# aosokin/os2d

Hardware: AMD Instinct MI355X
Metric: query-image-pairs/s (1280-px input, ResNet50, N-class) (higher is better)
Workload: dtype fftx3 (as fft; the per-bin complex GEMM on the fp16 MFMA with spectra split into fp16 hi+lo, 3 MFMAs per product, fp32 accumulate)

## Files before the change

### include/os2d_hip.h

```cpp
#ifndef OS2D_HIP_H
#define OS2D_HIP_H

#include <stddef.h>

#ifdef __cplusplus
extern "C" {
#endif

#define OS2D_ABI_VERSION 9

#define OS2D_PRECISION_F32 0
#define OS2D_PRECISION_F16X3 1
#define OS2D_PRECISION_F16X2 2

#define OS2D_PRECISION_FFT 3

#define OS2D_PRECISION_FFT32 5

#define OS2D_PRECISION_FFTX3 4

int os2d_abi_version(void);

const char* os2d_last_error(void);

size_t os2d_packed_conv_floats(int layer );
size_t os2d_packed_bias_floats(int layer );
int os2d_pack_conv(int layer, int P, const float* w, const float* b, const float* bn_weight, const float* bn_bias,
                   const float* bn_running_mean, const float* bn_running_var, float bn_eps, float* packed_w,
                   float* packed_b, void* stream);

int os2d_class_prepare(const float* src, int C, int h, int w, int normalize, float* q15, float* qp, void* stream);
size_t os2d_class_prepare_workspace_floats(int B, int C);
int os2d_class_prepare_batch(const float* const* srcs, const int* sizes, int B, int C, int normalize, float* q15,
                             float* qp, float* workspace, void* stream);

int os2d_head_workspace_bytes(int A, int B, int C, int H, int W, int P, size_t* bytes);
int os2d_head_workspace_bytes_ex(int A, int B, int C, int H, int W, int P, int precision, size_t* bytes);
int os2d_head_forward(const float* fm, const float* qp, const float* w1, const float* b1, const float* w2,
                      const float* b2, const float* w3, const float* b3, int A, int B, int C, int H, int W, int P,
                      int inverse, int stride, int rec_field, float* loc, float* cls, float* corners,
                      void* workspace, size_t workspace_bytes, void* stream);

size_t os2d_packed_conv_bytes(int layer, int precision);
int os2d_rnorm_exp(void);
int os2d_pack_conv_f16x3(int layer , int P, const float* w, const float* b, const float* bn_weight,
                         const float* bn_bias, const float* bn_running_mean, const float* bn_running_var, float bn_eps,
                         const int* weight_exp, const int* in_exp, const int* out_exp, void* packed_w, float* packed_b,
                         void* stream);

size_t os2d_class_split_bytes(int B, int C);
int os2d_class_split(const float* qp, void* qs, int B, int C, void* stream);

#define OS2D_STATUS_F16_RANGE 1
int os2d_head_forward_ex(const float* fm, const float* qp, const void* w1, const float* b1, const void* w2,
                         const float* b2, const void* w3, const float* b3, int A, int B, int C, int H, int W, int P,
                         int inverse, int stride, int rec_field, float* loc, float* cls, float* corners,
                         void* workspace, size_t workspace_bytes, void* stream, int precision, const void* qs,
                         void** stage_events, int* chunk_classes, int* status, const float* wspec, const float* twQ,
                         const float* twP);
int os2d_head_forward_ex2(const float* fm, const float* qp, const void* w1, const float* b1, const void* w2,
                          const float* b2, const void* w3, const float* b3, int A, int B, int C, int H, int W, int P,
                          int inverse, int stride, int rec_field, float* loc, float* cls, float* corners,
                          void* workspace, size_t workspace_bytes, void* stream, int precision, const void* qs,
                          void** stage_events, int* chunk_classes, int* status, const float* wspec, const float* twQ,
                          const float* twP, const void* wspec2);
void os2d_debug_set_dump(void* stream, int slot, void* dst, size_t bytes);
int os2d_prof_event_create(void** ev);
int os2d_prof_event_destroy(void* ev);
int os2d_prof_event_elapsed_ms(void* begin, void* end, float* ms);

int os2d_fm_sumsq(const float* fm, float* sumsq, int A, int C, int H, int W, void* stream);
size_t os2d_plane_floats(int H, int W);
int os2d_corr(const float* fm, const float* qp, const float* sumsq, float* corr, float* rnorm, int A, int B, int C,
              int H, int W, void* stream);
size_t os2d_corr_f16x3_workspace_bytes(int A, int C, int H, int W);
int os2d_corr_f16x3(const float* fm, const void* qs, float* corr, void* rshb, int A, int B, int C, int H, int W,
                    void* workspace, size_t workspace_bytes, void* stream);
size_t os2d_corr_f16x3_packed_workspace_bytes(int A, int B, int C, int H, int W);
int os2d_corr_f16x3_packed(const float* fm, const void* qs, float* corr, float* inv_norm, int A, int B, int C, int H, int W,
                           int form, void* workspace, size_t workspace_bytes, void* stream);
int os2d_corr_normalize(const float* corr, float* rnorm, int NB, int H, int W, void* stream);
int os2d_transform_conv(int layer, const float* in, const float* packed_w, const float* packed_b, float* out,
                        int NB, int P, int H, int W, void* stream);
size_t os2d_shb_bytes(int channels, int H, int W);
int os2d_corr_normalize_f16x3(const float* corr, void* rshb, int NB, int H, int W, void* stream);
int os2d_transform_conv_f16x3(int layer, const void* in, const void* packed_w, const float* packed_b, void* out, int NB,
                              int P, int H, int W, int terms, int* status, void* stream);
int os2d_alignment_grids(const float* params, int NB, int H, int W, int P, int inverse, float* theta, float* grids,
                         void* stream);
int os2d_sample_decode(const float* corr, const float* params, int NB, int H, int W, int P, int inverse, int stride,
                       int rec_field, float* loc, float* cls, float* corners, void* stream);

int os2d_decode_boxes(const float* loc, int NB, int H, int W, int stride, int rec_field, float img_w, float img_h,
                      float* boxes, void* stream);

int os2d_nms_workspace_bytes(int NC, int N, size_t* bytes);
int os2d_nms(const float* boxes, const int* counts, int NC, int N, float iou_threshold, unsigned char* keep,
             int* num_keep, void* workspace, size_t workspace_bytes, void* stream);

int os2d_detect_level_supported(int H, int W);
int os2d_detect_level(const float* loc, const float* cls, int B, int H, int W, int stride, int rec_field, float img_w,
                      float img_h, float scale_x, float scale_y, float score_threshold, float iou_threshold,
                      float* out_boxes, float* out_scores, int* out_index, int* out_count, void* stream);

#define OS2D_BOX_OP_SCALE 1
#define OS2D_BOX_OP_HFLIP 2
#define OS2D_BOX_OP_VFLIP 3
#define OS2D_BOX_OP_SHIFT 4
#define OS2D_BOX_MAX_OPS 6
#define OS2D_BOX_MAX_DEFAULT_OPS 12
int os2d_detect_level_ops(const float* loc, const float* cls, int B, int H, int W, int stride, int rec_field, float img_w,
                          float img_h, int op_count, const int* op_kinds, const float* op_args, float score_threshold,
                          float iou_threshold, float* out_boxes, float* out_scores, int* out_index, int* out_count,
                          void* stream);

size_t os2d_spectral_weight_bytes(int C, int Cout, int nbins);
int os2d_fft_sizes(int H, int W, int* P, int* Q, int* nbins);
int os2d_fft_tiles(int H, int W, int* tiles_y, int* tiles_x, int* tile_h, int* tile_w);
int os2d_fft_forward(const float* corr, const float* inv_norm, float* X, const float* twQ, const float* twP, int NB, int C,
                     int H, int W, void* stream);
int os2d_fft_inverse(const float* Y, const float* packed_b, void* out, const float* twQ, const float* twP, int NB, int Cout,
                     int H, int W, int* status, void* stream);
#define OS2D_SPECTRA_ROWS 0
#define OS2D_SPECTRA_QUADS 1
int os2d_fft_inverse_ex(const float* Y, const float* packed_b, void* out, const float* twQ, const float* twP, int NB, int Cout,
                        int H, int W, int* status, int layout, void* stream);
int os2d_spectral_gemm(const float* wspec, const float* X, float* Y, int NB, int C, int Cout, int nbins, void* stream);
size_t os2d_spectral_weight16_bytes(int C, int nbins);
int os2d_spectral_weights_build(const double* wfold, const double* twP64, const double* twQ64, int C, int Cout, int P, int Q,
                                int nbins, int split, void* out, void* workspace, void* stream);
float os2d_spectral_xscale(int H, int W);
int os2d_spectral_gemm_f16(const void* w16, const float* X, float* Y, int NB, int C, int Cout, int nbins, float xscale,
                           void* stream);

int os2d_dft_sizes(int H, int W, int* P, int* Q, int* nbins, int* tiles);
int os2d_dft_channel_stride(int C);
size_t os2d_dft_matrices_bytes(int P, int Q);
int os2d_dft_matrices_build(const double* twP64, const double* twQ64, int P, int Q, void* out, void* stream);
int os2d_dft_forward(const float* corr, const float* inv_norm, float* X, const void* matrices, int NB, int C, int H, int W,
                     void* stream);
int os2d_dft_inverse(const float* Y, const float* packed_b, void* out, const void* matrices, int NB, int Cout, int H, int W,
                     int* status, void* stream);
int os2d_dft_inverse_planes(const float* Y, const float* packed_b, float* out, const void* matrices, int NB, int Cout, int H, int W,
                            int* status, void* stream);
int os2d_spectral_weights_build_dft(const double* wfold, const double* twP64, const double* twQ64, int C, int Cout, int P, int Q,
                                    int nbins, void* out, void* workspace, void* stream);
int os2d_spectral_gemm_f16_quads(const void* w16, const float* X, float* Y, int NB, int C, int Cout, int nbins, float xscale,
                                 void* stream);
float os2d_dft_xscale(int H, int W);

#define OS2D_PYRAMID_MAX_LEVELS 16
int os2d_detect_pyramid_supported(int L, int N, int nms_max_batch);
int os2d_detect_pyramid_workspace_bytes(int B, int N, int passes, size_t* bytes);
int os2d_detect_pyramid(const float* const* loc, const float* const* cls, const float* const* corners, int B, int L,
                        const int* hw, int stride, int rec_field, const float* img_wh, const float* scale_xy,
                        float score_threshold, float iou_threshold, int nms_max_batch, int passes, float* out_boxes,
                        float* out_scores, int* out_index, float* out_default, float* out_corners, int* out_count,
                        int* unfinished, void* workspace, size_t workspace_bytes, void* stream);
int os2d_detect_pyramid_merged(const float* const* loc, const float* const* cls, const float* const* corners, int B, int L,
                               const int* hw, int stride, int rec_field, const float* img_wh, const float* scale_xy,
                               float score_threshold, float iou_threshold, int nms_max_batch, int passes, int G, int V,
                               const int* slot_rows, float* out_boxes, float* out_scores, int* out_index, float* out_default,
                               float* out_corners, int* out_count, int* unfinished, void* workspace, size_t workspace_bytes,
                               void* stream);

int os2d_detect_pyramid_ops(const float* const* loc, const float* const* cls, const float* const* corners, int B, int L,
                            const int* hw, int stride, int rec_field, const float* img_wh, const int* op_counts,
                            const int* op_kinds, const float* op_args, const int* default_op_counts,
                            const int* default_op_kinds, const float* default_op_args, float score_threshold, float iou_threshold,
                            int nms_max_batch, int passes, int G, int V, const int* slot_rows, float* out_boxes,
                            float* out_scores, int* out_index, float* out_default, float* out_corners, int* out_count,
                            int* unfinished, void* workspace, size_t workspace_bytes, void* stream);

#ifdef __cplusplus
}
#endif
#endif
```

### os2d_amd/_lib.py

```python
import ctypes

from . import build
from ._native import NativeLibrary, Os2dLibraryError

ABI_VERSION = 9

_c_float_p = ctypes.c_void_p
_vp = ctypes.c_void_p
_i = ctypes.c_int
_f = ctypes.c_float
_sz = ctypes.c_size_t

SIGNATURES = {
    "os2d_abi_version": (_i, []),
    "os2d_last_error": (ctypes.c_char_p, []),
    "os2d_packed_conv_floats": (_sz, [_i]),
    "os2d_packed_bias_floats": (_sz, [_i]),
    "os2d_pack_conv": (_i, [_i, _i, _vp, _vp, _vp, _vp, _vp, _vp, _f, _vp, _vp, _vp]),
    "os2d_class_prepare": (_i, [_vp, _i, _i, _i, _i, _vp, _vp, _vp]),
    "os2d_head_workspace_bytes": (_i, [_i, _i, _i, _i, _i, _i, ctypes.POINTER(_sz)]),
    "os2d_head_forward": (_i, [_vp] * 8 + [_i] * 9 + [_vp, _vp, _vp, _vp, _sz, _vp]),
    "os2d_packed_conv_bytes": (_sz, [_i, _i]),
    "os2d_pack_conv_f16x3": (_i, [_i, _i, _vp, _vp, _vp, _vp, _vp, _vp, _f, _vp, _vp, _vp, _vp, _vp, _vp]),
    "os2d_rnorm_exp": (_i, []),
    "os2d_class_prepare_batch": (_i, [_vp, _vp, _i, _i, _i, _vp, _vp, _vp, _vp]),
    "os2d_class_prepare_workspace_floats": (_sz, [_i, _i]),
    "os2d_shb_bytes": (_sz, [_i, _i, _i]),
    "os2d_corr_normalize_f16x3": (_i, [_vp, _vp, _i, _i, _i, _vp]),
    "os2d_transform_conv_f16x3": (_i, [_i, _vp, _vp, _vp, _vp, _i, _i, _i, _i, _i, _vp, _vp]),
    "os2d_alignment_grids": (_i, [_vp, _i, _i, _i, _i, _i, _vp, _vp, _vp]),
    "os2d_spectral_weight_bytes": (_sz, [_i, _i, _i]),
    "os2d_spectral_gemm": (_i, [_vp, _vp, _vp, _i, _i, _i, _i, _vp]),
    "os2d_spectral_weight16_bytes": (_sz, [_i, _i]),
    "os2d_spectral_xscale": (_f, [_i, _i]),
    "os2d_spectral_weights_build": (_i, [_vp, _vp, _vp, _i, _i, _i, _i, _i, _i, _vp, _vp, _vp]),
    "os2d_spectral_gemm_f16": (_i, [_vp, _vp, _vp, _i, _i, _i, _i, _f, _vp]),
    "os2d_debug_set_dump": (None, [_vp, _i, _vp, _sz]),
    "os2d_fft_sizes": (_i, [_i, _i, ctypes.POINTER(_i), ctypes.POINTER(_i), ctypes.POINTER(_i)]),
    "os2d_fft_tiles": (_i, [_i, _i, ctypes.POINTER(_i), ctypes.POINTER(_i), ctypes.POINTER(_i), ctypes.POINTER(_i)]),
    "os2d_fft_forward": (_i, [_vp, _vp, _vp, _vp, _vp, _i, _i, _i, _i, _vp]),
    "os2d_fft_inverse": (_i, [_vp, _vp, _vp, _vp, _vp, _i, _i, _i, _i, _vp, _vp]),
    "os2d_fft_inverse_ex": (_i, [_vp, _vp, _vp, _vp, _vp, _i, _i, _i, _i, _vp, _i, _vp]),
    "os2d_dft_sizes": (_i, [_i, _i, ctypes.POINTER(_i), ctypes.POINTER(_i), ctypes.POINTER(_i), ctypes.POINTER(_i)]),
    "os2d_dft_channel_stride": (_i, [_i]),
    "os2d_dft_matrices_bytes": (_sz, [_i, _i]),
    "os2d_dft_matrices_build": (_i, [_vp, _vp, _i, _i, _vp, _vp]),
    "os2d_dft_forward": (_i, [_vp, _vp, _vp, _vp, _i, _i, _i, _i, _vp]),
    "os2d_dft_inverse": (_i, [_vp, _vp, _vp, _vp, _i, _i, _i, _i, _vp, _vp]),
    "os2d_spectral_weights_build_dft": (_i, [_vp, _vp, _vp, _i, _i, _i, _i, _i, _vp, _vp, _vp]),
    "os2d_spectral_gemm_f16_quads": (_i, [_vp, _vp, _vp, _i, _i, _i, _i, _f, _vp]),
    "os2d_dft_xscale": (_f, [_i, _i]),
    "os2d_class_split": (_i, [_vp, _vp, _i, _i, _vp]),
    "os2d_class_split_bytes": (_sz, [_i, _i]),
    "os2d_head_forward_ex": (_i, [_vp] * 8 + [_i] * 9 + [_vp, _vp, _vp, _vp, _sz, _vp, _i, _vp,
                                  ctypes.POINTER(_vp), ctypes.POINTER(_i), _vp, _vp, _vp, _vp]),
    "os2d_head_forward_ex2": (_i, [_vp] * 8 + [_i] * 9 + [_vp, _vp, _vp, _vp, _sz, _vp, _i, _vp,
                                   ctypes.POINTER(_vp), ctypes.POINTER(_i), _vp, _vp, _vp, _vp, _vp]),
    "os2d_dft_inverse_planes": (_i, [_vp, _vp, _vp, _vp, _i, _i, _i, _i, _vp, _vp]),
    "os2d_head_workspace_bytes_ex": (_i, [_i, _i, _i, _i, _i, _i, _i, ctypes.POINTER(_sz)]),
    "os2d_prof_event_create": (_i, [ctypes.POINTER(_vp)]),
    "os2d_prof_event_destroy": (_i, [_vp]),
    "os2d_prof_event_elapsed_ms": (_i, [_vp, _vp, ctypes.POINTER(_f)]),
    "os2d_fm_sumsq": (_i, [_vp, _vp, _i, _i, _i, _i, _vp]),
    "os2d_plane_floats": (_sz, [_i, _i]),
    "os2d_corr": (_i, [_vp, _vp, _vp, _vp, _vp, _i, _i, _i, _i, _i, _vp]),
    "os2d_corr_normalize": (_i, [_vp, _vp, _i, _i, _i, _vp]),
    "os2d_corr_f16x3_workspace_bytes": (_sz, [_i, _i, _i, _i]),
    "os2d_corr_f16x3": (_i, [_vp, _vp, _vp, _vp, _i, _i, _i, _i, _i, _vp, _sz, _vp]),
    "os2d_corr_f16x3_packed_workspace_bytes": (_sz, [_i, _i, _i, _i, _i]),
    "os2d_corr_f16x3_packed": (_i, [_vp, _vp, _vp, _vp, _i, _i, _i, _i, _i, _i, _vp, _sz, _vp]),
    "os2d_transform_conv": (_i, [_i, _vp, _vp, _vp, _vp, _i, _i, _i, _i, _vp]),
    "os2d_sample_decode": (_i, [_vp, _vp, _i, _i, _i, _i, _i, _i, _i, _vp, _vp, _vp, _vp]),
    "os2d_decode_boxes": (_i, [_vp, _i, _i, _i, _i, _i, _f, _f, _vp, _vp]),
    "os2d_nms_workspace_bytes": (_i, [_i, _i, ctypes.POINTER(_sz)]),
    "os2d_nms": (_i, [_vp, _vp, _i, _i, _f, _vp, _vp, _vp, _sz, _vp]),
    "os2d_detect_level_supported": (_i, [_i, _i]),
    "os2d_detect_level": (_i, [_vp, _vp] + [_i] * 5 + [_f] * 6 + [_vp] * 5),
    "os2d_detect_level_ops": (_i, [_vp, _vp] + [_i] * 5 + [_f, _f, _i, _vp, _vp, _f, _f] + [_vp] * 5),
    "os2d_detect_pyramid_supported": (_i, [_i, _i, _i]),
    "os2d_detect_pyramid_workspace_bytes": (_i, [_i, _i, _i, ctypes.POINTER(_sz)]),
    "os2d_detect_pyramid": (_i, [_vp, _vp, _vp, _i, _i, _vp, _i, _i, _vp, _vp, _f, _f, _i, _i, _vp, _vp, _vp, _vp, _vp, _vp,
                                 _vp, _vp, _sz, _vp]),
    "os2d_detect_pyramid_merged": (_i, [_vp, _vp, _vp, _i, _i, _vp, _i, _i, _vp, _vp, _f, _f, _i, _i, _i, _i, _vp, _vp, _vp, _vp,
                                        _vp, _vp, _vp, _vp, _vp, _sz, _vp]),
    "os2d_detect_pyramid_ops": (_i, [_vp, _vp, _vp, _i, _i, _vp, _i, _i, _vp, _vp, _vp, _vp, _vp, _vp, _vp, _f, _f, _i, _i, _i, _i, _vp, _vp, _vp,
                                     _vp, _vp, _vp, _vp, _vp, _vp, _sz, _vp]),
}


LIBRARY = NativeLibrary(build.HIP, SIGNATURES, ABI_VERSION, "os2d_abi_version", "os2d_last_error", "the OS2D head")
lib_path, load, check = LIBRARY.lib_path, LIBRARY.load, LIBRARY.check


def ptr(t):
    if t is None:
        return None
    import torch
    if not (isinstance(t, torch.Tensor) and t.is_cuda and t.dtype in (torch.float32, torch.float64, torch.uint8, torch.int32, torch.int64)
            and t.is_contiguous()):
        raise ValueError("expected a contiguous device tensor, got {}".format(
            (type(t).__name__, getattr(t, "device", None), getattr(t, "dtype", None))))
    return ctypes.c_void_p(t.data_ptr())


def host_ptr(t):
    if t is None:
        return None
    if not t.is_pinned():
        raise ValueError("expected a pinned host tensor")
    return ctypes.c_void_p(t.data_ptr())


def current_stream(device):
    import torch
    return ctypes.c_void_p(torch.cuda.current_stream(device).cuda_stream)
```

### os2d_amd/csrc/abi.hip

```cpp
#include <stdio.h>

#include "../../include/os2d_hip.h"
#include "os2d_common.h"
#include "detect_common.h"
#include <atomic>
#include <mutex>
#include <random>
#include <vector>

namespace {
struct ConvShape {
  int cout, cin, ks, mt;
};
bool conv_shape(int layer, int P, ConvShape* s) {
  switch (layer) {
    case 1: *s = {128, OS2D_K, 7, 128}; return true;
    case 2: *s = {64, 128, 5, 64}; return true;
    case 3: *s = {P, 64, 5, 32}; return true;
    default: return false;
  }
}
size_t align_up(size_t x, size_t a) { return (x + a - 1) / a * a; }

int os2d_conv1_steps_padded() { return 25; }

struct Carve {
  size_t flags, sumsq, fs, corr, rpad, h1, h2, params, invn, sumfx, xspec, yspec, total;
};
Carve carve(int A, int Bc, int C, int H, int W, int P, int fft_bins = 0, int fft_tiles = 1, int xspec_channels = OS2D_K) {
  const size_t HW = (size_t)H * W, PL = os2d_plane(H, W), NB = (size_t)A * Bc;
  Carve c;
  size_t off = 0;
  auto take = [&](size_t floats) {
    size_t o = off;
    off = align_up(off + floats * sizeof(float), 256);
    return o;
  };
  c.flags = take((size_t)A + 1);
  c.sumsq = take((size_t)A * HW);
  c.fs = take((size_t)A * os2d_corr_groups(C) * 2 * HW * 4);
  c.corr = take(NB * OS2D_K * HW);
  c.rpad = take(fft_bins > 0 ? 0 : NB * (OS2D_G * 2 * 4) * PL);
  c.h1 = take(NB * 128 * PL);
  c.h2 = take(NB * 64 * PL);
  c.params = take(NB * P * HW);
  c.invn = c.sumfx = c.xspec = c.yspec = 0;
  if (fft_bins > 0) {
    c.invn = take(NB * HW);
    c.sumfx = take(NB * HW * 2);
    c.xspec = take(NB * fft_tiles * xspec_channels * (size_t)fft_bins * 2);
    c.yspec = take(NB * fft_tiles * 128 * (size_t)fft_bins * 2);
  }
  c.total = off;
  return c;
}

#ifdef OS2D_DIAG_DUMP
struct DumpEntry {
  void* stream;
  int slot;
  void* dst;
  size_t bytes;
};
std::vector<DumpEntry> g_dumps;
std::mutex g_dumps_mutex;
bool dumps_active() {
  std::lock_guard<std::mutex> lock(g_dumps_mutex);
  return !g_dumps.empty();
}
void dump_slot(void* stream, int slot, const void* src, size_t bytes) {
  std::lock_guard<std::mutex> lock(g_dumps_mutex);
  for (const DumpEntry& e : g_dumps)
    if (e.stream == stream && e.slot == slot && e.dst)
      (void)hipMemcpyAsync(e.dst, src, bytes < e.bytes ? bytes : e.bytes, hipMemcpyDeviceToDevice, static_cast<hipStream_t>(stream));
}
#else
inline bool dumps_active() { return false; }
inline void dump_slot(void*, int, const void*, size_t) {}
#endif

bool head_args_ok(int A, int B, int C, int H, int W, int P) {
  if (A < 1 || B < 1 || C < 1 || H < 1 || W < 1 || (P != 6 && P != 4)) {
    os2d_set_error("bad head shape A=%d B=%d C=%d H=%d W=%d P=%d (need A,B,C,H,W>=1, P in {6,4})", A, B, C, H,
                   W, P);
    return false;
  }
  if (W > OS2D_MAX_W) {
    os2d_set_error("feature map width %d > %d: beyond what the transform planner of the 7x7 layer tiles (images wider than %d px "
                   "at stride 16 are not supported)", W, OS2D_MAX_W, OS2D_MAX_W * 16);
    return false;
  }
  if (H > OS2D_MAX_H) {
    os2d_set_error("feature map height %d > %d: beyond what the transform planner of the 7x7 layer tiles (images taller than %d px "
                   "at stride 16 are not supported)", H, OS2D_MAX_H, OS2D_MAX_H * 16);
    return false;
  }
  return true;
}
int next_epoch() {
  static std::atomic<unsigned> counter{[] {
    std::random_device rd;
    return (unsigned)rd() | 0x100u;
  }()};
  unsigned e;
  do e = counter.fetch_add(1u, std::memory_order_relaxed) + 1u;
  while (e < 2u);
  return (int)e;
}
bool is_freq(int precision) {
  return precision == OS2D_PRECISION_FFT || precision == OS2D_PRECISION_FFTX3 || precision == OS2D_PRECISION_FFT32;
}
int freq_plan(int precision, int H, int W, int* P, int* Q, int* bins, int* tiles) {
  return precision == OS2D_PRECISION_FFTX3 ? os2d_dft_plan(H, W, P, Q, bins, tiles) : os2d_fft_plan(H, W, P, Q, bins, tiles);
}
bool direct7_width_ok(int W) {
  if (W > OS2D_MAX_W_DIRECT7) {
    os2d_set_error("feature map width %d > %d: the direct 7x7 kernels keep 3 halo rows of their input in LDS - wider maps need a "
                   "frequency-domain precision (fftx3 / fft / fft32), which tiles any width up to %d", W, OS2D_MAX_W_DIRECT7, OS2D_MAX_W);
    return false;
  }
  return true;
}
}

void os2d_debug_set_dump(void* stream, int slot, void* dst, size_t bytes) {
#ifdef OS2D_DIAG_DUMP
  std::lock_guard<std::mutex> lock(g_dumps_mutex);
  for (size_t i = 0; i < g_dumps.size(); ++i)
    if (g_dumps[i].stream == stream && g_dumps[i].slot == slot) {
      if (dst) {
        g_dumps[i].dst = dst;
        g_dumps[i].bytes = bytes;
      } else {
        g_dumps.erase(g_dumps.begin() + i);
      }
      return;
    }
  if (dst) g_dumps.push_back(DumpEntry{stream, slot, dst, bytes});
#else
  (void)stream, (void)slot, (void)dst, (void)bytes;
  os2d_set_error("os2d_debug_set_dump: this library was built without -DOS2D_DIAG_DUMP (diagnostic builds only)");
#endif
}

extern "C" {

int os2d_abi_version(void) { return OS2D_ABI_VERSION; }
const char* os2d_last_error(void) { return os2d_error_text; }

size_t os2d_packed_conv_floats(int layer) {
  ConvShape s;
  if (!conv_shape(layer, 6, &s)) return 0;
  return (size_t)((s.cin + 1) / 2) * s.ks * s.ks * 2 * s.mt;
}
size_t os2d_packed_bias_floats(int layer) {
  ConvShape s;
  if (!conv_shape(layer, 6, &s)) return 0;
  return (size_t)3 * s.mt;
}

int os2d_pack_conv(int layer, int P, const float* w, const float* b, const float* bn_weight, const float* bn_bias,
                   const float* bn_running_mean, const float* bn_running_var, float bn_eps, float* packed_w,
                   float* packed_b, void* stream) {
  ConvShape s;
  if (!conv_shape(layer, P, &s) || (layer == 3 && P != 6 && P != 4)) {
    os2d_set_error("os2d_pack_conv: bad layer %d / P %d", layer, P);
    return -1;
  }
  if (!w || !b || !packed_w || !packed_b) {
    os2d_set_error("os2d_pack_conv: null pointer");
    return -1;
  }
  const bool has_bn = bn_weight || bn_bias || bn_running_mean || bn_running_var;
  if (has_bn && !(bn_weight && bn_bias && bn_running_mean && bn_running_var)) {
    os2d_set_error("os2d_pack_conv: BatchNorm needs all four of weight/bias/running_mean/running_var");
    return -1;
  }
  return os2d_launch_pack_conv(w, b, bn_weight, bn_bias, bn_running_mean, bn_running_var, bn_eps, s.cout, s.cin, s.ks,
                               s.mt, packed_w, packed_b, os2d_stream(stream));
}

int os2d_class_prepare(const float* src, int C, int h, int w, int normalize, float* q15, float* qp, void* stream) {
  if (!src || !q15 || !qp || C < 1 || h < 1 || w < 1) {
    os2d_set_error("os2d_class_prepare: bad arguments (C=%d h=%d w=%d)", C, h, w);
    return -1;
  }
  return os2d_launch_class_prepare(src, C, h, w, normalize, q15, qp, os2d_stream(stream));
}

size_t os2d_class_prepare_workspace_floats(int B, int C) {
  if (B < 1 || C < 1) return 0;
  return (size_t)os2d_class_prepare_partial_floats(B, C);
}

int os2d_class_prepare_batch(const float* const* srcs, const int* sizes, int B, int C, int normalize, float* q15,
                             float* qp, float* workspace, void* stream) {
  if (!srcs || !sizes || !q15 || !qp || !workspace || B < 1 || C < 1 || B > 65535) {
    os2d_set_error("os2d_class_prepare_batch: bad arguments (B=%d C=%d; at most 65535 classes per call)", B, C);
    return -1;
  }
  return os2d_launch_class_prepare_batch(srcs, sizes, B, C, normalize, q15, qp, workspace, os2d_stream(stream));
}

size_t os2d_plane_floats(int H, int W) { return (size_t)os2d_plane(H, W); }

size_t os2d_shb_bytes(int channels, int H, int W) {
  if (channels < 1 || H < 1 || W < 1) return 0;
  return (size_t)((channels + 7) / 8) * 2 * os2d_plane(H, W) * 16;
}

int os2d_head_workspace_bytes(int A, int B, int C, int H, int W, int P, size_t* bytes) {
  if (!bytes) {
    os2d_set_error("os2d_head_workspace_bytes: null output");
    return -1;
  }
  if (!head_args_ok(A, B, C, H, W, P)) return -1;
  *bytes = carve(A, B, C, H, W, P).total;
  return 0;
}

int os2d_head_workspace_bytes_ex(int A, int B, int C, int H, int W, int P, int precision, size_t* bytes) {
  if (!bytes) {
    os2d_set_error("os2d_head_workspace_bytes_ex: null output");
    return -1;
  }
  if (!head_args_ok(A, B, C, H, W, P)) return -1;
  int bins = 0, tiles[6] = {1, 1, 0, 0, 0, 0};
  if (is_freq(precision) && !freq_plan(precision, H, W, nullptr, nullptr, &bins, tiles)) {
    os2d_set_error("os2d_head_workspace_bytes_ex: no transform plan for a %dx%d map", H, W);
    return -3;
  }
  *bytes = carve(A, B, C, H, W, P, bins, tiles[0] * tiles[1], precision == OS2D_PRECISION_FFTX3 ? OS2D_XSPEC_CPAD : OS2D_K).total;
  return 0;
}

int os2d_fm_sumsq(const float* fm, float* sumsq, int A, int C, int H, int W, void* stream) {
  if (!fm || !sumsq || A < 1 || C < 1 || H < 1 || W < 1) {
    os2d_set_error("os2d_fm_sumsq: bad arguments");
    return -1;
  }
  return os2d_launch_fm_sumsq(fm, sumsq, A, C, H * W, os2d_stream(stream));
}

int os2d_corr(const float* fm, const float* qp, const float* sumsq, float* corr, float* rnorm, int A, int B, int C,
              int H, int W, void* stream) {
  if (!fm || !qp || !sumsq || !corr || !rnorm) {
    os2d_set_error("os2d_corr: null pointer");
    return -1;
  }
  if (!head_args_ok(A, B, C, H, W, 6)) return -1;
  int rc = os2d_launch_border_zero(rnorm, A * B * OS2D_KP, H, W, os2d_stream(stream));
  if (rc) return rc;
  return os2d_launch_corr(fm, qp, sumsq, corr, rnorm, nullptr, A, B, C, H, W, 0, os2d_stream(stream));
}

size_t os2d_corr_f16x3_workspace_bytes(int A, int C, int H, int W) {
  if (A < 1 || C < 1 || H < 1 || W < 1) return 0;
  return align_up((size_t)A * H * W * sizeof(float), 256) + (size_t)A * os2d_corr_groups(C) * 2 * H * W * 16;
}

int os2d_corr_f16x3(const float* fm, const void* qs, float* corr, void* rshb, int A, int B, int C, int H, int W,
                    void* workspace, size_t workspace_bytes, void* stream) {
  if (!fm || !qs || !corr || !rshb || !workspace) {
    os2d_set_error("os2d_corr_f16x3: null pointer");
    return -1;
  }
  if (!head_args_ok(A, B, C, H, W, 6)) return -1;
  if (workspace_bytes < os2d_corr_f16x3_workspace_bytes(A, C, H, W) || (reinterpret_cast<uintptr_t>(workspace) & 255)) {
    os2d_set_error("os2d_corr_f16x3: workspace too small or not 256-byte aligned");
    return -2;
  }
  float* sumsq = static_cast<float*>(workspace);
  void* fs = static_cast<char*>(workspace) + align_up((size_t)A * H * W * sizeof(float), 256);
  int rc = os2d_launch_fm_sumsq(fm, sumsq, A, C, H * W, os2d_stream(stream));
  if (!rc) rc = os2d_launch_split_fm(fm, sumsq, fs, A, C, H * W, nullptr, 0, Os2dRangeFlag{nullptr, 0}, os2d_stream(stream));
  if (!rc) rc = os2d_launch_border_zero_shb(rshb, A * B, H, W, os2d_stream(stream));
  if (!rc) rc = os2d_launch_corr_f16x3(fs, qs, corr, rshb, nullptr, nullptr, 0, A, B, C, H, W, os2d_stream(stream));
  return rc;
}

size_t os2d_corr_f16x3_packed_workspace_bytes(int A, int B, int C, int H, int W) {
  if (A < 1 || B < 1 || C < 1 || H < 1 || W < 1) return 0;
  return align_up(os2d_corr_f16x3_workspace_bytes(A, C, H, W), 256) + (size_t)A * B * H * W * sizeof(unsigned long long);
}

int os2d_corr_f16x3_packed(const float* fm, const void* qs, float* corr, float* inv_norm, int A, int B, int C, int H, int W,
                           int form, void* workspace, size_t workspace_bytes, void* stream) {
  if (!fm || !qs || !corr || !inv_norm || !workspace) {
    os2d_set_error("os2d_corr_f16x3_packed: null pointer");
    return -1;
  }
  if (!head_args_ok(A, B, C, H, W, 6)) return -1;
  if (workspace_bytes < os2d_corr_f16x3_packed_workspace_bytes(A, B, C, H, W) || (reinterpret_cast<uintptr_t>(workspace) & 255)) {
    os2d_set_error("os2d_corr_f16x3_packed: workspace too small or not 256-byte aligned");
    return -2;
  }
  float* sumsq = static_cast<float*>(workspace);
  void* fs = static_cast<char*>(workspace) + align_up((size_t)A * H * W * sizeof(float), 256);
  void* sumfx = static_cast<char*>(workspace) + align_up(os2d_corr_f16x3_workspace_bytes(A, C, H, W), 256);
  int rc = os2d_launch_fm_sumsq(fm, sumsq, A, C, H * W, os2d_stream(stream));
  if (!rc) rc = os2d_launch_split_fm(fm, sumsq, fs, A, C, H * W, nullptr, 0, Os2dRangeFlag{nullptr, 0}, os2d_stream(stream));
  if (form < -1 || form > 7 || (form >= 0 && (form & 3) > 1)) {
    os2d_set_error("os2d_corr_f16x3_packed: form %d (0 padded | 1 packed | -1 the head's choice; + 4: no half tiles at the tail)", form);
    return -1;
  }
  const bool packed = form < 0 ? os2d_corr_f16x3_use_packed(A, B, H, W) != 0 : (form & 1) != 0;
  if (!rc && packed) rc = os2d_launch_corr_sums_clear(sumfx, A, B, H, W, os2d_stream(stream));
  if (!rc) rc = os2d_launch_corr_f16x3(fs, qs, corr, nullptr, inv_norm, packed ? sumfx : nullptr, (form >= 0 && (form & 4)) ? 2 : 0, A, B, C, H, W, os2d_stream(stream));
  return rc;
}

int os2d_corr_normalize(const float* corr, float* rnorm, int NB, int H, int W, void* stream) {
  if (!corr || !rnorm || NB < 1 || H < 1 || W < 1) {
    os2d_set_error("os2d_corr_normalize: bad arguments");
    return -1;
  }
  return os2d_launch_corr_normalize(corr, rnorm, NB, H, W, os2d_stream(stream));
}

int os2d_transform_conv(int layer, const float* in, const float* packed_w, const float* packed_b, float* out, int NB,
                        int P, int H, int W, void* stream) {
  if (!in || !packed_w || !packed_b || !out || NB < 1 || H < 1 || W < 1 || (layer == 3 && P != 6 && P != 4)) {
    os2d_set_error("os2d_transform_conv: bad arguments (layer=%d NB=%d P=%d)", layer, NB, P);
    return -1;
  }
  return os2d_launch_conv(layer, in, packed_w, packed_b, out, NB, P, H, W, os2d_stream(stream));
}

int os2d_sample_decode(const float* corr, const float* params, int NB, int H, int W, int P, int inverse, int stride,
                       int rec_field, float* loc, float* cls, float* corners, void* stream) {
  if (!corr || !params || !loc || !cls || !corners || NB < 1 || H < 1 || W < 1 || (P != 6 && P != 4)) {
    os2d_set_error("os2d_sample_decode: bad arguments");
    return -1;
  }
  return os2d_launch_sample_decode(corr, params, NB, H, W, P, inverse, stride, rec_field, NB, NB, 0, loc, cls,
                                   corners, nullptr, 0, nullptr, os2d_stream(stream));
}

int os2d_decode_boxes(const float* loc, int NB, int H, int W, int stride, int rec_field, float img_w, float img_h,
                      float* boxes, void* stream) {
  if (!loc || !boxes || NB < 1 || H < 1 || W < 1) {
    os2d_set_error("os2d_decode_boxes: bad arguments");
    return -1;
  }
  return os2d_launch_decode_boxes(loc, NB, H, W, stride, rec_field, img_w, img_h, boxes, os2d_stream(stream));
}

int os2d_detect_level_supported(int H, int W) { return os2d_detect_level_lds_bytes(H, W) != 0 ? 1 : 0; }

int os2d_detect_level(const float* loc, const float* cls, int B, int H, int W, int stride, int rec_field, float img_w,
                      float img_h, float scale_x, float scale_y, float score_threshold, float iou_threshold,
                      float* out_boxes, float* out_scores, int* out_index, int* out_count, void* stream) {
  if (!loc || !cls || !out_boxes || !out_scores || !out_index || !out_count || B < 1 || H < 1 || W < 1 || stride < 1 ||
      rec_field < 1) {
    os2d_set_error("os2d_detect_level: bad arguments");
    return -1;
  }
  return os2d_launch_detect_level(loc, cls, B, H, W, stride, rec_field, img_w, img_h, os2d_box_ops_scale<OS2D_BOX_MAX_OPS>(scale_x, scale_y),
                                  score_threshold, iou_threshold, out_boxes, out_scores, out_index, out_count, os2d_stream(stream));
}

int os2d_detect_level_ops(const float* loc, const float* cls, int B, int H, int W, int stride, int rec_field, float img_w,
                          float img_h, int op_count, const int* op_kinds, const float* op_args, float score_threshold,
                          float iou_threshold, float* out_boxes, float* out_scores, int* out_index, int* out_count,
                          void* stream) {
  if (!loc || !cls || !out_boxes || !out_scores || !out_index || !out_count || B < 1 || H < 1 || W < 1 || stride < 1 ||
      rec_field < 1) {
    os2d_set_error("os2d_detect_level_ops: bad arguments");
    return -1;
  }
  Os2dBoxOps ops;
  if (!os2d_box_ops_from(op_kinds, op_args, op_count, &ops)) {
    os2d_set_error("os2d_detect_level_ops: bad transform chain (at most %d ops of kind 1..4)", OS2D_BOX_MAX_OPS);
    return -1;
  }
  return os2d_launch_detect_level(loc, cls, B, H, W, stride, rec_field, img_w, img_h, ops, score_threshold, iou_threshold,
                                  out_boxes, out_scores, out_index, out_count, os2d_stream(stream));
}

int os2d_nms_workspace_bytes(int NC, int N, size_t* bytes) {
  if (!bytes || NC < 1 || N < 1) {
    os2d_set_error("os2d_nms_workspace_bytes: bad arguments");
    return -1;
  }
  *bytes = (size_t)NC * N * 4 * sizeof(float);
  return 0;
}

int os2d_nms(const float* boxes, const int* counts, int NC, int N, float iou_threshold, unsigned char* keep,
             int* num_keep, void* workspace, size_t workspace_bytes, void* stream) {
  if (!boxes || !counts || !keep || !num_keep || !workspace || NC < 1 || N < 1) {
    os2d_set_error("os2d_nms: bad arguments");
    return -1;
  }
  if ((reinterpret_cast<uintptr_t>(boxes) & 15) || (reinterpret_cast<uintptr_t>(workspace) & 15)) {
    os2d_set_error("os2d_nms: boxes and workspace must be 16-byte aligned");
    return -1;
  }
  if (workspace_bytes < (size_t)NC * N * 4 * sizeof(float)) {
    os2d_set_error("os2d_nms: workspace too small");
    return -2;
  }
  return os2d_launch_nms(boxes, counts, NC, N, iou_threshold, keep, num_keep, workspace, os2d_stream(stream));
}

int os2d_head_forward_ex2(const float* fm, const float* qp, const void* w1, const float* b1, const void* w2,
                          const float* b2, const void* w3, const float* b3, int A, int B, int C, int H, int W, int P,
                          int inverse, int stride, int rec_field, float* loc, float* cls, float* corners,
                          void* workspace, size_t workspace_bytes, void* stream, int precision, const void* qs,
                          void** stage_events, int* chunk_classes, int* status, const float* wspec, const float* twQ,
                          const float* twP, const void* wspec2) {
  if (!fm || !qp || !w1 || !b1 || !w2 || !b2 || !w3 || !b3 || !loc || !cls || !corners || !workspace) {
    os2d_set_error("os2d_head_forward: null pointer");
    return -1;
  }
  if (precision != OS2D_PRECISION_F32 && precision != OS2D_PRECISION_F16X3 && precision != OS2D_PRECISION_F16X2 &&
      precision != OS2D_PRECISION_FFT && precision != OS2D_PRECISION_FFTX3 && precision != OS2D_PRECISION_FFT32) {
    os2d_set_error("os2d_head_forward: unknown precision %d", precision);
    return -1;
  }
  int fft_bins = 0, tiles[6] = {1, 1, 0, 0, 0, 0};
  const bool dft = precision == OS2D_PRECISION_FFTX3;
  if (is_freq(precision)) {
    if (!wspec || !twQ || (!dft && !twP)) {
      os2d_set_error("os2d_head_forward: the frequency-domain modes need the weight spectra and the transform tables "
                     "(fft / fft32: twQ, twP; fftx3: the matrices of os2d_dft_matrices_build as twQ)");
      return -1;
    }
    if (!freq_plan(precision, H, W, nullptr, nullptr, &fft_bins, tiles)) {
      os2d_set_error("os2d_head_forward: no transform plan for a %dx%d map", H, W);
      return -3;
    }
  } else if (!direct7_width_ok(W)) {
    return -1;
  }
  const int fft_T = tiles[0] * tiles[1], xch = dft ? OS2D_XSPEC_CPAD : OS2D_K;
  static const bool conv2_freq_env = [] {
    const char* e = getenv("OS2D_CONV2_FREQ");
    return !(e && e[0] == '0');
  }();
  const bool conv2_freq = dft && wspec2 && conv2_freq_env;
  const bool fp32_ops = precision == OS2D_PRECISION_F32 || precision == OS2D_PRECISION_FFT32;
  if (!fp32_ops && !qs) {
    os2d_set_error("os2d_head_forward: precision f16x3 / f16x2 needs the split class operand (os2d_class_split)");
    return -1;
  }
  if (!head_args_ok(A, B, C, H, W, P)) return -1;
  if (stride < 1 || rec_field < 1) {
    os2d_set_error("os2d_head_forward: bad stride/rec_field %d/%d", stride, rec_field);
    return -1;
  }
  if (reinterpret_cast<uintptr_t>(workspace) & 255) {
    os2d_set_error("os2d_head_forward: workspace must be 256-byte aligned");
    return -1;
  }
  const size_t one = carve(A, 1, C, H, W, P, fft_bins, fft_T, xch).total;
  if (workspace_bytes < one) {
    os2d_set_error("os2d_head_forward: workspace too small (%zu B, need >= %zu B for one class)", workspace_bytes, one);
    return -2;
  }
  int Bc = B;
  while (Bc > 1 && carve(A, Bc, C, H, W, P, fft_bins, fft_T, xch).total > workspace_bytes) {
    const size_t two = carve(A, 2, C, H, W, P, fft_bins, fft_T, xch).total;
    const size_t per = two - one;
    int guess = per ? (int)((workspace_bytes - one) / per) + 1 : 1;
    if (guess >= Bc) guess = Bc - 1;
    if (guess < 1) guess = 1;
    Bc = guess;
  }
  hipStream_t st = os2d_stream(stream);
  char* ws = static_cast<char*>(workspace);
  const Carve c = carve(A, Bc, C, H, W, P, fft_bins, fft_T, xch);
  float* invn = fft_bins ? reinterpret_cast<float*>(ws + c.invn) : nullptr;
  void* sumfx = (fft_bins && !fp32_ops && os2d_corr_f16x3_use_packed(A, Bc, H, W)) ? ws + c.sumfx : nullptr;
  float* xspec = fft_bins ? reinterpret_cast<float*>(ws + c.xspec) : nullptr;
  float* yspec = fft_bins ? reinterpret_cast<float*>(ws + c.yspec) : nullptr;
  float* sumsq = reinterpret_cast<float*>(ws + c.sumsq);
  void* fsplit = ws + c.fs;
  float* corr = reinterpret_cast<float*>(ws + c.corr);
  float* rpad = reinterpret_cast<float*>(ws + c.rpad);
  float* h1 = reinterpret_cast<float*>(ws + c.h1);
  float* h2 = reinterpret_cast<float*>(ws + c.h2);
  float* params = reinterpret_cast<float*>(ws + c.params);
  int* flags = reinterpret_cast<int*>(ws + c.flags);
  const int epoch = next_epoch();
  const Os2dRangeFlag per_image = {fp32_ops ? nullptr : flags, epoch}, whole_call = {fp32_ops ? nullptr : flags + A, epoch};

  if (chunk_classes) *chunk_classes = Bc;
  auto mark = [&](int b0, int idx) {
    if (stage_events && b0 == 0 && stage_events[idx]) (void)hipEventRecord(reinterpret_cast<hipEvent_t>(stage_events[idx]), st);
  };
  int rc = os2d_launch_fm_sumsq(fm, sumsq, A, C, H * W, st);
  if (rc) return rc;
  if (!fp32_ops && (rc = os2d_launch_split_fm(fm, sumsq, fsplit, A, C, H * W, sumfx, sumfx ? (size_t)A * Bc * H * W : 0, per_image, st))) return rc;
  for (int b0 = 0; b0 < B; b0 += Bc) {
    const int bc = (B - b0 < Bc) ? (B - b0) : Bc;
    const int NB = A * bc;
    const bool f16 = !fp32_ops;
    const int terms1 = precision == OS2D_PRECISION_F16X2 ? 2 : 3;
    mark(b0, 0);
    if (f16) {
      if (!fft_bins && (rc = os2d_launch_border_zero_shb(rpad, NB, H, W, st))) return rc;
    } else if (!fft_bins) {
      if ((rc = os2d_launch_border_zero(rpad, NB * OS2D_KP, H, W, st))) return rc;
    }
    if (f16) {
      const char* qsb = static_cast<const char*>(qs) + (size_t)b0 * os2d_corr_groups(C) * 2 * 256 * 16;
      if ((rc = os2d_launch_corr_f16x3(fsplit, qsb, corr, fft_bins ? nullptr : rpad, invn, sumfx, 1, A, bc, C, H, W, st))) return rc;
    } else {
      if ((rc = os2d_launch_corr(fm, qp + (size_t)b0 * C * OS2D_QROWS, sumsq, corr, fft_bins ? nullptr : rpad, invn, A, bc, C, H, W,
                                 0, st)))
        return rc;
    }
    mark(b0, 1);
    mark(b0, 2);
    if (fft_bins) {
      bool inv_borders = false;
      if (f16) {
        static const bool borders_in_inverse = [] {
          const char* e = getenv("OS2D_BORDERS_IN_INVERSE");
          return !(e && e[0] == '0');
        }();
        inv_borders = dft && borders_in_inverse;
        const int planes = (inv_borders || conv2_freq) ? 0 : NB * 16 * 2;
        if ((planes || sumfx) &&
            (rc = os2d_launch_border_zero_shb_planes_norms(h1, planes, H, W, sumfx, invn, (size_t)NB * H * W, st)))
          return rc;
      } else if ((rc = os2d_launch_border_zero(h1, NB * 128, H, W, st))) {
        return rc;
      }
      mark(b0, 10);
      const int layout = precision == OS2D_PRECISION_FFTX3 ? OS2D_SPECTRA_QUADS : OS2D_SPECTRA_ROWS;
      if (dft) {
        const void* mats = twQ;
        if ((rc = os2d_launch_dft_forward(corr, invn, xspec, mats, NB, OS2D_K, xch, H, W, st))) return rc;
        mark(b0, 11);
        if ((rc = os2d_launch_spectral_gemm_f16(wspec, xspec, yspec, NB * fft_T, OS2D_K, 128, fft_bins,
                                                os2d_spectral_xscale_for(tiles[4], tiles[5]), 1, xch, st)))
          return rc;
        mark(b0, 12);
        if ((rc = os2d_launch_dft_inverse(yspec, b1, 128, h1, mats, NB, 128, H, W, whole_call,
                                          conv2_freq ? OS2D_DFT_OUT_PLANES : inv_borders ? OS2D_DFT_OUT_SHB_BORDERS : OS2D_DFT_OUT_SHB, st)))
          return rc;
      } else {
        if ((rc = os2d_launch_fft_forward(corr, invn, xspec, twQ, twP, NB, OS2D_K, H, W, st))) return rc;
        mark(b0, 11);
        if ((rc = os2d_launch_spectral_gemm(wspec, xspec, yspec, NB * fft_T, OS2D_K, 128, fft_bins, st))) return rc;
        mark(b0, 12);
        if ((rc = os2d_launch_fft_inverse(yspec, b1, 128, h1, twQ, twP, NB, 128, H, W, whole_call, layout, f16 ? 0 : 1, st))) return rc;
      }
    } else if (f16) {
      if ((rc = os2d_launch_conv_f16x3(1, rpad, w1, b1, whole_call, h1, NB, P, H, W, terms1, st))) return rc;
    } else {
      if ((rc = os2d_launch_conv(1, rpad, static_cast<const float*>(w1), b1, h1, NB, P, H, W, st))) return rc;
    }
    mark(b0, 3);
    mark(b0, 4);
    if (dumps_active() && b0 == 0) {
      const size_t PLb = os2d_plane(H, W);
      dump_slot(stream, 0, corr, (size_t)NB * OS2D_K * H * W * 4);
      if (fft_bins) {
        dump_slot(stream, 1, invn, (size_t)NB * H * W * 4);
        dump_slot(stream, 2, xspec, (size_t)NB * fft_T * OS2D_K * fft_bins * 8);
        dump_slot(stream, 3, yspec, (size_t)NB * fft_T * 128 * fft_bins * 8);
      }
      dump_slot(stream, 4, h1, (size_t)NB * 128 * (conv2_freq ? (size_t)H * W : PLb) * 4);
    }
    if (conv2_freq) {
      if ((rc = os2d_launch_dft_forward(h1, nullptr, xspec, twQ, NB, 128, 128, H, W, st))) return rc;
      if ((rc = os2d_launch_spectral_gemm_f16(wspec2, xspec, yspec, NB * fft_T, 128, 64, fft_bins,
                                              os2d_spectral_xscale_for(tiles[4], tiles[5]), 1, 128, st)))
        return rc;
      if ((rc = os2d_launch_dft_inverse(yspec, b2, 64, h2, twQ, NB, 64, H, W, whole_call, OS2D_DFT_OUT_SHB_BORDERS, st))) return rc;
    } else if (f16) {
      if ((rc = os2d_launch_conv_f16x3(2, h1, w2, b2, whole_call, h2, NB, P, H, W, 3, st))) return rc;
    } else {
      if ((rc = os2d_launch_conv(2, h1, static_cast<const float*>(w2), b2, h2, NB, P, H, W, st))) return rc;
    }
    mark(b0, 5);
    mark(b0, 6);
    if (dumps_active() && b0 == 0) dump_slot(stream, 5, h2, (size_t)NB * 64 * os2d_plane(H, W) * 4);
    static const bool fused_tail_env = [] {
      const char* e = getenv("OS2D_FUSED_TAIL");
      return !(e && e[0] == '0');
    }();
    const bool fused_tail = f16 && fused_tail_env && !dumps_active();
    if (fused_tail) {
      if ((rc = os2d_launch_conv3_sample_decode(h2, w3, b3, corr, NB, H, W, P, inverse, stride, rec_field, bc, B, b0, loc, cls, corners,
                                                flags, epoch, status, st)))
        return rc;
      mark(b0, 7);
      mark(b0, 8);
      mark(b0, 9);
      continue;
    }
    if (f16) {
      if ((rc = os2d_launch_conv_f16x3(3, h2, w3, b3, whole_call, params, NB, P, H, W, 3, st))) return rc;
    } else {
      if ((rc = os2d_launch_conv(3, h2, static_cast<const float*>(w3), b3, params, NB, P, H, W, st))) return rc;
    }
    mark(b0, 7);
    mark(b0, 8);
    if (dumps_active() && b0 == 0) dump_slot(stream, 6, params, (size_t)NB * P * H * W * 4);
    if ((rc = os2d_launch_sample_decode(corr, params, NB, H, W, P, inverse, stride, rec_field, bc, B, b0, loc, cls,
                                        corners, fp32_ops ? nullptr : flags, epoch, status, st)))
      return rc;
    mark(b0, 9);
  }
  return 0;
}

int os2d_head_forward_ex(const float* fm, const float* qp, const void* w1, const float* b1, const void* w2,
                         const float* b2, const void* w3, const float* b3, int A, int B, int C, int H, int W, int P,
                         int inverse, int stride, int rec_field, float* loc, float* cls, float* corners,
                         void* workspace, size_t workspace_bytes, void* stream, int precision, const void* qs,
                         void** stage_events, int* chunk_classes, int* status, const float* wspec, const float* twQ,
                         const float* twP) {
  return os2d_head_forward_ex2(fm, qp, w1, b1, w2, b2, w3, b3, A, B, C, H, W, P, inverse, stride, rec_field, loc, cls, corners, workspace,
                               workspace_bytes, stream, precision, qs, stage_events, chunk_classes, status, wspec, twQ, twP, nullptr);
}

int os2d_head_forward(const float* fm, const float* qp, const float* w1, const float* b1, const float* w2,
                      const float* b2, const float* w3, const float* b3, int A, int B, int C, int H, int W, int P,
                      int inverse, int stride, int rec_field, float* loc, float* cls, float* corners, void* workspace,
                      size_t workspace_bytes, void* stream) {
  return os2d_head_forward_ex(fm, qp, w1, b1, w2, b2, w3, b3, A, B, C, H, W, P, inverse, stride, rec_field, loc, cls,
                              corners, workspace, workspace_bytes, stream, OS2D_PRECISION_F32, nullptr, nullptr, nullptr,
                              nullptr, nullptr, nullptr, nullptr);
}

size_t os2d_class_split_bytes(int B, int C) {
  if (B < 1 || C < 1) return 0;
  return (size_t)B * os2d_corr_groups(C) * 2 * 256 * 16;
}

int os2d_class_split(const float* qp, void* qs, int B, int C, void* stream) {
  if (!qp || !qs || B < 1 || C < 1) {
    os2d_set_error("os2d_class_split: bad arguments");
    return -1;
  }
  return os2d_launch_split_qp(qp, qs, B, C, os2d_stream(stream));
}

size_t os2d_packed_conv_bytes(int layer, int precision) {
  if (precision == OS2D_PRECISION_F32) return os2d_packed_conv_floats(layer) * sizeof(float);
  if (precision != OS2D_PRECISION_F16X3 && precision != OS2D_PRECISION_F16X2) return 0;
  if (layer == 1) return (size_t)OS2D_G * os2d_conv1_steps_padded() * 4 * 128 * 16;
  if (layer == 2) return (size_t)16 * 14 * 4 * 64 * 16;
  if (layer == 3) return (size_t)8 * 14 * 4 * 32 * 16;
  return 0;
}

int os2d_pack_conv_f16x3(int layer, int P, const float* w, const float* b, const float* bn_weight, const float* bn_bias,
                         const float* bn_running_mean, const float* bn_running_var, float bn_eps, const int* weight_exp,
                         const int* in_exp, const int* out_exp, void* packed_w, float* packed_b, void* stream) {
  const bool has_bn = bn_weight || bn_bias || bn_running_mean || bn_running_var;
  if (layer < 1 || layer > 3 || !w || !b || !packed_w || !packed_b || !weight_exp || !in_exp ||
      (layer != 3 && !out_exp) || (has_bn && !(bn_weight && bn_bias && bn_running_mean && bn_running_var)) ||
      (layer == 3 && P != 6 && P != 4)) {
    os2d_set_error("os2d_pack_conv_f16x3: bad arguments (layer %d, P %d)", layer, P);
    return -1;
  }
  if (layer == 1)
    return os2d_launch_pack_conv_f16(w, b, bn_weight, bn_bias, bn_running_mean, bn_running_var, bn_eps, 128, OS2D_K, 7,
                                     128, os2d_conv1_steps_padded(), weight_exp, in_exp, out_exp, packed_w, packed_b,
                                     os2d_stream(stream));
  if (layer == 2)
    return os2d_launch_pack_conv_f16(w, b, bn_weight, bn_bias, bn_running_mean, bn_running_var, bn_eps, 64, 128, 5, 64,
                                     14, weight_exp, in_exp, out_exp, packed_w, packed_b, os2d_stream(stream));
  return os2d_launch_pack_conv_f16(w, b, bn_weight, bn_bias, bn_running_mean, bn_running_var, bn_eps, P, 64, 5, 32, 14,
                                   weight_exp, in_exp, nullptr, packed_w, packed_b, os2d_stream(stream));
}

int os2d_rnorm_exp(void) { return OS2D_RNORM_EXP; }

int os2d_corr_normalize_f16x3(const float* corr, void* rshb, int NB, int H, int W, void* stream) {
  if (!corr || !rshb || NB < 1 || H < 1 || W < 1) {
    os2d_set_error("os2d_corr_normalize_f16x3: bad arguments");
    return -1;
  }
  return os2d_launch_corr_normalize_shb(corr, rshb, NB, H, W, os2d_stream(stream));
}

int os2d_transform_conv_f16x3(int layer, const void* in, const void* packed_w, const float* packed_b, void* out, int NB,
                              int P, int H, int W, int terms, int* status, void* stream) {
  if (!in || !packed_w || !packed_b || !out || NB < 1 || H < 1 || W < 1 || layer < 1 || layer > 3 ||
      (layer == 3 && P != 6 && P != 4) || (terms != 3 && !(terms == 2 && layer == 1))) {
    os2d_set_error("os2d_transform_conv_f16x3: bad arguments (layer=%d NB=%d P=%d terms=%d)", layer, NB, P, terms);
    return -1;
  }
  if (W > (layer == 1 ? OS2D_MAX_W_DIRECT7 : OS2D_MAX_W)) {
    os2d_set_error("os2d_transform_conv_f16x3: feature map width %d > %d", W, layer == 1 ? OS2D_MAX_W_DIRECT7 : OS2D_MAX_W);
    return -1;
  }
  return os2d_launch_conv_f16x3(layer, in, packed_w, packed_b, Os2dRangeFlag{status, OS2D_STATUS_F16_RANGE}, out, NB, P, H, W, terms, os2d_stream(stream));
}

int os2d_fft_sizes(int H, int W, int* P, int* Q, int* nbins) {
  if (!P || !Q || !nbins) {
    os2d_set_error("os2d_fft_sizes: null output");
    return -1;
  }
  if (!os2d_fft_plan(H, W, P, Q, nbins, nullptr)) {
    os2d_set_error("os2d_fft_sizes: no transform plan for a %dx%d map", H, W);
    return -3;
  }
  return 0;
}

int os2d_fft_tiles(int H, int W, int* tiles_y, int* tiles_x, int* tile_h, int* tile_w) {
  int t[6];
  if (!tiles_y || !tiles_x || !tile_h || !tile_w) {
    os2d_set_error("os2d_fft_tiles: null output");
    return -1;
  }
  if (!os2d_fft_plan(H, W, nullptr, nullptr, nullptr, t)) {
    os2d_set_error("os2d_fft_tiles: no transform plan for a %dx%d map", H, W);
    return -3;
  }
  *tiles_y = t[0];
  *tiles_x = t[1];
  *tile_h = t[2];
  *tile_w = t[3];
  return 0;
}

int os2d_fft_forward(const float* corr, const float* inv_norm, float* X, const float* twQ, const float* twP, int NB, int C,
                     int H, int W, void* stream) {
  if (!corr || !inv_norm || !X || !twQ || !twP || NB < 1 || C < 1 || H < 1 || W < 1) {
    os2d_set_error("os2d_fft_forward: bad arguments");
    return -1;
  }
  return os2d_launch_fft_forward(corr, inv_norm, X, twQ, twP, NB, C, H, W, os2d_stream(stream));
}

int os2d_fft_inverse_ex(const float* Y, const float* packed_b, void* out, const float* twQ, const float* twP, int NB, int Cout,
                        int H, int W, int* status, int layout, void* stream) {
  if (!Y || !packed_b || !out || !twQ || !twP || NB < 1 || Cout != 128 || H < 1 || W < 1 ||
      (layout != OS2D_SPECTRA_ROWS && layout != OS2D_SPECTRA_QUADS)) {
    os2d_set_error("os2d_fft_inverse: bad arguments (Cout must be 128: the 7x7 layer)");
    return -1;
  }
  int rc = os2d_launch_border_zero_shb_planes(out, NB * (Cout / 8) * 2, H, W, os2d_stream(stream));
  if (rc) return rc;
  return os2d_launch_fft_inverse(Y, packed_b, 128, out, twQ, twP, NB, Cout, H, W, Os2dRangeFlag{status, OS2D_STATUS_F16_RANGE}, layout, 0, os2d_stream(stream));
}

int os2d_fft_inverse(const float* Y, const float* packed_b, void* out, const float* twQ, const float* twP, int NB, int Cout,
                     int H, int W, int* status, void* stream) {
  return os2d_fft_inverse_ex(Y, packed_b, out, twQ, twP, NB, Cout, H, W, status, OS2D_SPECTRA_ROWS, stream);
}

size_t os2d_spectral_weight_bytes(int C, int Cout, int nbins) {
  if (C < 1 || Cout < 1 || Cout > 128 || nbins < 8 || (nbins & 7)) return 0;
  return os2d_spectral_weight_floats(C, Cout, nbins) * sizeof(float);
}

int os2d_spectral_gemm(const float* wspec, const float* X, float* Y, int NB, int C, int Cout, int nbins, void* stream) {
  if (!wspec || !X || !Y || NB < 1 || C < 1 || Cout < 1 || Cout > 128 || nbins < 8 || (nbins & 7)) {
    os2d_set_error("os2d_spectral_gemm: bad arguments (NB=%d C=%d Cout=%d nbins=%d; nbins must be a multiple of 8)", NB, C,
                   Cout, nbins);
    return -1;
  }
  if ((reinterpret_cast<uintptr_t>(wspec) | reinterpret_cast<uintptr_t>(X) | reinterpret_cast<uintptr_t>(Y)) & 15) {
    os2d_set_error("os2d_spectral_gemm: buffers must be 16-byte aligned");
    return -1;
  }
  return os2d_launch_spectral_gemm(wspec, X, Y, NB, C, Cout, nbins, os2d_stream(stream));
}

int os2d_spectral_weights_build(const double* wfold, const double* twP64, const double* twQ64, int C, int Cout, int P, int Q,
                                int nbins, int split, void* out, void* workspace, void* stream) {
  if (!wfold || !twP64 || !twQ64 || !out || (split && !workspace) || C < 1 || Cout < 1 || Cout > 128 || nbins < 8 || (nbins & 7)) {
    os2d_set_error("os2d_spectral_weights_build: bad arguments (C=%d Cout=%d nbins=%d)", C, Cout, nbins);
    return -1;
  }
  if ((reinterpret_cast<uintptr_t>(out) & 15) || (reinterpret_cast<uintptr_t>(workspace) & 7)) {
    os2d_set_error("os2d_spectral_weights_build: out must be 16-byte, workspace 8-byte aligned");
    return -1;
  }
  return os2d_launch_spectra_pack(wfold, twP64, twQ64, C, Cout, P, Q, nbins, split, 0, out, workspace, os2d_stream(stream));
}

size_t os2d_spectral_weight16_bytes(int C, int nbins) {
  if (C < 1 || nbins < 8 || (nbins & 7)) return 0;
  return os2d_spectral_weight16_size(C, nbins);
}

float os2d_spectral_xscale(int H, int W) {
  int t[6];
  if (H < 1 || W < 1 || !os2d_fft_plan(H, W, nullptr, nullptr, nullptr, t)) return 0.f;
  return os2d_spectral_xscale_for(t[4], t[5]);
}

int os2d_spectral_gemm_f16(const void* w16, const float* X, float* Y, int NB, int C, int Cout, int nbins, float xscale,
                           void* stream) {
  if (!w16 || !X || !Y || NB < 1 || C < 1 || Cout < 1 || Cout > 128 || nbins < 8 || (nbins & 7) || !(xscale > 0.f)) {
    os2d_set_error("os2d_spectral_gemm_f16: bad arguments (NB=%d C=%d Cout=%d nbins=%d; nbins must be a multiple of 8)", NB, C,
                   Cout, nbins);
    return -1;
  }
  if ((reinterpret_cast<uintptr_t>(w16) | reinterpret_cast<uintptr_t>(X) | reinterpret_cast<uintptr_t>(Y)) & 15) {
    os2d_set_error("os2d_spectral_gemm_f16: buffers must be 16-byte aligned");
    return -1;
  }
  return os2d_launch_spectral_gemm_f16(w16, X, Y, NB, C, Cout, nbins, xscale, 0, 0, os2d_stream(stream));
}

int os2d_dft_sizes(int H, int W, int* P, int* Q, int* nbins, int* tiles) {
  if (!P || !Q || !nbins) {
    os2d_set_error("os2d_dft_sizes: null output");
    return -1;
  }
  if (!os2d_dft_plan(H, W, P, Q, nbins, tiles)) {
    os2d_set_error("os2d_dft_sizes: no transform plan for a %dx%d map", H, W);
    return -3;
  }
  return 0;
}

int os2d_dft_channel_stride(int C) { return C == OS2D_K ? OS2D_XSPEC_CPAD : (C + 7) / 8 * 8; }

size_t os2d_dft_matrices_bytes(int P, int Q) {
  if (P < 4 || (P & 3) || Q < 2 || (Q & 1)) return 0;
  return os2d_dft_matrices_size(P, Q);
}

int os2d_dft_matrices_build(const double* twP64, const double* twQ64, int P, int Q, void* out, void* stream) {
  if (!twP64 || !twQ64 || !out || (reinterpret_cast<uintptr_t>(out) & 15)) {
    os2d_set_error("os2d_dft_matrices_build: bad arguments (out must be 16-byte aligned)");
    return -1;
  }
  return os2d_launch_dft_matrices(twP64, twQ64, P, Q, out, os2d_stream(stream));
}

int os2d_dft_forward(const float* corr, const float* inv_norm, float* X, const void* matrices, int NB, int C, int H, int W,
                     void* stream) {
  if (!corr || !X || !matrices || NB < 1 || C < 1 || H < 1 || W < 1) {
    os2d_set_error("os2d_dft_forward: bad arguments");
    return -1;
  }
  return os2d_launch_dft_forward(corr, inv_norm, X, matrices, NB, C, os2d_dft_channel_stride(C), H, W, os2d_stream(stream));
}

int os2d_dft_inverse(const float* Y, const float* packed_b, void* out, const void* matrices, int NB, int Cout, int H, int W,
                     int* status, void* stream) {
  if (!Y || !packed_b || !out || !matrices || NB < 1 || (Cout != 128 && Cout != 64) || H < 1 || W < 1) {
    os2d_set_error("os2d_dft_inverse: bad arguments (Cout must be 128 or 64: the 7x7 layer / the 5x5 layer 128 -> 64)");
    return -1;
  }
  return os2d_launch_dft_inverse(Y, packed_b, Cout, out, matrices, NB, Cout, H, W, Os2dRangeFlag{status, OS2D_STATUS_F16_RANGE},
                                 OS2D_DFT_OUT_SHB_BORDERS, os2d_stream(stream));
}

int os2d_dft_inverse_planes(const float* Y, const float* packed_b, float* out, const void* matrices, int NB, int Cout, int H, int W,
                            int* status, void* stream) {
  if (!Y || !packed_b || !out || !matrices || NB < 1 || (Cout != 128 && Cout != 64) || H < 1 || W < 1) {
    os2d_set_error("os2d_dft_inverse_planes: bad arguments (Cout must be 128 or 64)");
    return -1;
  }
  return os2d_launch_dft_inverse(Y, packed_b, Cout, out, matrices, NB, Cout, H, W, Os2dRangeFlag{status, OS2D_STATUS_F16_RANGE},
                                 OS2D_DFT_OUT_PLANES, os2d_stream(stream));
}

int os2d_spectral_weights_build_dft(const double* wfold, const double* twP64, const double* twQ64, int C, int Cout, int P, int Q,
                                    int nbins, void* out, void* workspace, void* stream) {
  if (!wfold || !twP64 || !twQ64 || !out || !workspace || C < 1 || Cout < 1 || Cout > 128 || nbins < 8 || (nbins & 7) || (P & 3)) {
    os2d_set_error("os2d_spectral_weights_build_dft: bad arguments (C=%d Cout=%d P=%d nbins=%d)", C, Cout, P, nbins);
    return -1;
  }
  if ((reinterpret_cast<uintptr_t>(out) & 15) || (reinterpret_cast<uintptr_t>(workspace) & 7)) {
    os2d_set_error("os2d_spectral_weights_build_dft: out must be 16-byte, workspace 8-byte aligned");
    return -1;
  }
  return os2d_launch_spectra_pack(wfold, twP64, twQ64, C, Cout, P, Q, nbins, 1, 1, out, workspace, os2d_stream(stream));
}

int os2d_spectral_gemm_f16_quads(const void* w16, const float* X, float* Y, int NB, int C, int Cout, int nbins, float xscale,
                                 void* stream) {
  if (!w16 || !X || !Y || NB < 1 || C < 1 || Cout < 1 || Cout > 128 || nbins < 8 || (nbins & 7) || !(xscale > 0.f)) {
    os2d_set_error("os2d_spectral_gemm_f16_quads: bad arguments (NB=%d C=%d Cout=%d nbins=%d)", NB, C, Cout, nbins);
    return -1;
  }
  if ((reinterpret_cast<uintptr_t>(w16) | reinterpret_cast<uintptr_t>(X) | reinterpret_cast<uintptr_t>(Y)) & 15) {
    os2d_set_error("os2d_spectral_gemm_f16_quads: buffers must be 16-byte aligned");
    return -1;
  }
  return os2d_launch_spectral_gemm_f16(w16, X, Y, NB, C, Cout, nbins, xscale, 1, os2d_dft_channel_stride(C), os2d_stream(stream));
}

float os2d_dft_xscale(int H, int W) {
  int t[6];
  if (H < 1 || W < 1 || !os2d_dft_plan(H, W, nullptr, nullptr, nullptr, t)) return 0.f;
  return os2d_spectral_xscale_for(t[4], t[5]);
}

int os2d_alignment_grids(const float* params, int NB, int H, int W, int P, int inverse, float* theta, float* grids,
                         void* stream) {
  if (!params || (!theta && !grids) || NB < 1 || H < 1 || W < 1 || (P != 6 && P != 4)) {
    os2d_set_error("os2d_alignment_grids: bad arguments");
    return -1;
  }
  return os2d_launch_alignment_grids(params, NB, H, W, P, inverse, theta, grids, os2d_stream(stream));
}

int os2d_prof_event_create(void** ev) {
  hipEvent_t e;
  hipError_t rc = hipEventCreate(&e);
  if (rc != hipSuccess || !ev) {
    os2d_set_error("hipEventCreate: %s", hipGetErrorString(rc));
    return -4;
  }
  *ev = e;
  return 0;
}
int os2d_prof_event_destroy(void* ev) { return hipEventDestroy(reinterpret_cast<hipEvent_t>(ev)) == hipSuccess ? 0 : -4; }
int os2d_prof_event_elapsed_ms(void* a, void* b, float* ms) {
  hipError_t rc = hipEventElapsedTime(ms, reinterpret_cast<hipEvent_t>(a), reinterpret_cast<hipEvent_t>(b));
  if (rc != hipSuccess) {
    os2d_set_error("hipEventElapsedTime: %s", hipGetErrorString(rc));
    return -4;
  }
  return 0;
}

}
```

### os2d_amd/csrc/dft_mfma.h

```cpp
#pragma once

#ifndef DFT_DEV
#error "the includer defines DFT_DEV, DFT_TID, DFT_BID, DFT_GRID, DFT_LDS, DFT_BARRIER, DFT_MFMA, DFT_SHFL_XOR, DFT_SHFL_XOR_U32, DFT_BALLOT, DFT_FLAG, DFT_FLAG_SET, DFT_RAISE, DFT_UNIFORM"
#endif

#ifndef DFT_HD
#define DFT_HD static inline
#endif
#ifndef DFT_MEMBER
#define DFT_MEMBER inline
#endif
#ifndef DFT_LANDED
#define DFT_LANDED(X)
#endif
#ifndef DFT_FWD_PREFETCH_AFTER
#define DFT_FWD_PREFETCH_AFTER 2
#endif
#ifndef DFT_INV_PREFETCH_AFTER
#define DFT_INV_PREFETCH_AFTER 2
#endif
#ifndef DFT_PIPE_REGA
#define DFT_PIPE_REGA 1
#endif
#ifndef DFT_PIPE_LDS
#define DFT_PIPE_LDS 1
#endif
#ifndef DFT_SCHED_FENCE
#define DFT_SCHED_FENCE()
#endif
#ifndef DFT_STREAM_STORE
#define DFT_STREAM_STORE(P, V) (*(P) = (V))
#endif
#ifndef DFT_STAMP
#define DFT_STAMP(K)
#define DFT_STAMP_BEGIN()
#define DFT_STAMP_END(BASE)
#endif

#include "tile_common.h"

namespace os2d_dft {

typedef float f32x4u __attribute__((ext_vector_type(4), aligned(4)));

constexpr int DFT_THR = 512, DFT_WAVES = 8;
constexpr int DFT_G = 4;
constexpr int DFT_MAXP = 64;
constexpr int DFT_MAXV = 48;
constexpr int DFT_MAXWK = 96;
constexpr int DFT_KREG = 8;
constexpr int DFT_OUT_SHB = 0, DFT_OUT_SHB_BORDERS = 1, DFT_OUT_PLANES = 2;

struct DftPlan {
  int H, W;
  int P, Q, V, NBINS;
  int T, TY, TX, TH, TW;
  int oy, ox;
  int LH, LW;
  int RH;
  int Pp;
  int Wk;
  int N1;
  int M2;
  int Mx;
  int N2;
  int MA;
  int MB;
  int KB;
  int NBo;
  int G;
  int eT;
  int fast;
  unsigned inv_cg, inv_t, inv_tx, inv_c4, inv_v, inv_pq, inv_og, inv_kg, inv_pp;
  int lds_const, lds_union, lds_total;
};

DFT_HD int dft_round_up(int x, int m) { return (x + m - 1) / m * m; }
DFT_HD unsigned dft_magic(unsigned d) { return d > 1 ? (unsigned)(((1ull << 32) + d - 1) / d) : 0u; }

DFT_HD int dft_units_fqt(int P, int Q) { return (dft_round_up(Q, 16) / 8) * 2 * dft_round_up(Q + 2, 32); }
constexpr int DFT_R2_P = 64, DFT_R2_MATU = 8 * 2 * 64, DFT_R2_TWU = 16;
constexpr int DFT_R2_LDS_TW = 512;
DFT_HD bool dft_radix2(int P) { return P == DFT_R2_P; }
DFT_HD int dft_units_fp2(int P, int Q) {
  return dft_radix2(P) ? DFT_R2_MATU + DFT_R2_TWU : (2 * dft_round_up(P, 8) / 8) * 2 * dft_round_up(2 * P, 32);
}
DFT_HD int dft_units_e2(int P, int Q) { return (2 * dft_round_up(P, 8) / 8) * 2 * dft_round_up(2 * P, 32); }
DFT_HD int dft_units_gq(int P, int Q) { return (dft_round_up(Q + 2, 16) / 8) * 2 * dft_round_up(Q, 32); }
DFT_HD size_t dft_matrices_units(int P, int Q) {
  return (size_t)dft_units_fqt(P, Q) + dft_units_fp2(P, Q) + dft_units_e2(P, Q) + dft_units_gq(P, Q);
}

static inline bool dft_plan_transform(int LH, int LW, int RH, int ncols, int minP, int minQ, int G, DftPlan* pl) {
  pl->G = G;
  pl->P = dft_round_up(minP, 4);
  if (pl->P == 60) pl->P = DFT_R2_P;
  pl->Q = dft_round_up(minQ, 2);
  pl->V = pl->Q / 2 + 1;
  pl->NBINS = dft_round_up(pl->P * pl->V, 8);
  pl->LH = LH;
  pl->LW = LW;
  pl->RH = RH;
  pl->Pp = dft_round_up(pl->P, 8);
  pl->Wk = dft_round_up(LW, 16);
  pl->N1 = dft_round_up(2 * pl->V, 32);
  pl->M2 = dft_round_up(2 * pl->P, 32);
  pl->Mx = dft_round_up(G * pl->Pp, 32);
  pl->N2 = dft_round_up(G * pl->V, 32);
  pl->MA = dft_round_up(2 * RH, 32);
  pl->MB = G * (pl->MA / 2);
  pl->KB = dft_round_up(2 * pl->V, 16);
  pl->NBo = dft_round_up(ncols, 32);
  int e = 0;
  while ((1 << e) < pl->P) ++e;
  pl->eT = e + 1;
  if (pl->P > DFT_MAXP || pl->V > DFT_MAXV || pl->Wk > DFT_MAXWK || LH > pl->P || LW > pl->Q || RH > pl->P) return false;
  const int fqt = (pl->Wk / 8) * 2 * pl->N1 * 16, gq = (pl->KB / 8) * 2 * pl->NBo * 16;
  const int x = (pl->Wk / 8) * 2 * (pl->Mx + 1) * 16, r2 = (2 * pl->Pp / 8) * 2 * (pl->N2 + 1) * 16;
  const int xs = pl->V * (pl->P * 8 * G + 16);
  const int y2 = r2, tt = (pl->KB / 8) * 2 * (pl->MB + 1) * 16;
  int u = x;
  if (r2 > u) u = r2;
  if (xs > u) u = xs;
  if (y2 > u) u = y2;
  if (tt > u) u = tt;
  if (G == 8) {
    if (dft_radix2(pl->P)) return false;
    const int fp2 = (2 * pl->Pp / 8) * 2 * pl->M2 * 16;
    const int ca = fqt + fp2, cb = gq + fp2;
    pl->lds_const = ca > cb ? ca : cb;
    pl->lds_union = dft_round_up(u, 256);
    pl->lds_total = pl->lds_const + pl->lds_union + 1024;
    const int t1 = (pl->Mx / 32) * (pl->N1 / 32), t2 = (pl->M2 / 32) * (pl->N2 / 32), tA = (pl->MA / 32) * (pl->N2 / 32),
              tB = (pl->MB / 32) * (pl->NBo / 32);
    const int npos = pl->Pp * (pl->Wk / 4), nitem = G * pl->V * (pl->Pp / 8);
    return pl->lds_total <= 160 * 1024 && t1 <= 24 && t2 <= 24 && tA <= 24 && tB <= 24 && npos <= 2 * DFT_THR && nitem <= 3 * DFT_THR;
  }
  pl->lds_const = fqt > gq ? fqt : gq;
  pl->lds_union = dft_round_up(u, 256);
  pl->lds_total = pl->lds_const + pl->lds_union + 1024;
  return pl->lds_total <= 160 * 1024;
}

static inline void dft_set_tiles(DftPlan* pl, int H, int W, int TY, int TX, int TH, int TW) {
  pl->H = H;
  pl->W = W;
  pl->TY = TY;
  pl->TX = TX;
  pl->T = TY * TX;
  pl->TH = TH;
  pl->TW = TW;
  pl->oy = TY > 1 ? 3 : 0;
  pl->ox = TX > 1 ? 3 : 0;
  pl->fast = (pl->T == 1 && (W & 3) == 0) ? 1 : 0;
  pl->inv_t = dft_magic((unsigned)pl->T);
  pl->inv_tx = dft_magic((unsigned)TX);
  pl->inv_c4 = dft_magic((unsigned)(pl->Wk / 4));
  pl->inv_v = dft_magic((unsigned)pl->V);
  pl->inv_pq = dft_magic((unsigned)(pl->P / 4 * pl->G * 2));
  pl->inv_kg = dft_magic((unsigned)(pl->Pp / 8));
  pl->inv_pp = dft_magic((unsigned)pl->Pp);
}

struct DftSize {
  int P, Q;
};
static const DftSize DFT_CANONICAL[6] = {{36, 46}, {44, 54}, {48, 62}, {52, 68}, {56, 70}, {64, 84}};

static inline bool dft_make_plan_policy(int H, int W, int canonical, DftPlan* out, int G = DFT_G) {
  bool found = false;
  long best = 0;
  for (int TY = 1; TY <= 48; ++TY)
    for (int TX = 1; TX <= 48; ++TX) {
      const int TH = (H + TY - 1) / TY, TW = (W + TX - 1) / TX;
      if ((TY > 1 && (TY - 1) * TH >= H) || (TX > 1 && (TX - 1) * TW >= W)) continue;
      const int LH = TY > 1 ? TH + 6 : H, LW = TX > 1 ? TW + 6 : W;
      const int minP = TY > 1 ? TH + 6 : H + 3, minQ = TX > 1 ? TW + 6 : W + 3;
      if (minP > DFT_MAXP || minQ > 2 * (DFT_MAXV - 1)) continue;
      for (int k = 0; k < (canonical ? 6 : 1); ++k) {
        if (canonical && (DFT_CANONICAL[k].P < minP || DFT_CANONICAL[k].Q < minQ)) continue;
        DftPlan c = {};
        if (!dft_plan_transform(LH, LW, TY > 1 ? TH + 3 : H, TX > 1 ? TW + 3 : W, canonical ? DFT_CANONICAL[k].P : minP,
                                canonical ? DFT_CANONICAL[k].Q : minQ, G, &c))
          continue;
        dft_set_tiles(&c, H, W, TY, TX, TH, TW);
        const long cost = (long)c.T * c.NBINS;
        if (!found || cost < best) {
          found = true;
          best = cost;
          *out = c;
        }
      }
    }
  return found;
}

#ifndef OS2D_HOST_EMU
static inline int dft_size_policy() {
  static const int policy = [] {
    const char* e = getenv("OS2D_DFT_SIZES");
    return (e && (e[0] == 'e' || e[0] == '0')) ? 0 : 1;
  }();
  return policy;
}
#else
static inline int dft_size_policy() { return emu_dft_policy; }
#endif
static inline bool dft_make_plan(int H, int W, DftPlan* out) { return dft_make_plan_policy(H, W, dft_size_policy(), out); }
static inline bool dft_plan_g8(const DftPlan& base, DftPlan* out) {
  DftPlan c = {};
  if (!dft_plan_transform(base.LH, base.LW, base.RH, base.TX > 1 ? base.TW + 3 : base.W, base.P, base.Q, 8, &c)) return false;
  dft_set_tiles(&c, base.H, base.W, base.TY, base.TX, base.TH, base.TW);
  *out = c;
  return true;
}

constexpr int DFT_PBLK = 64;
DFT_HD size_t dft_spectra_pair0(int pr, int NBT, int NQ, int cstride, size_t* qstride) {
  const int pb = pr / DFT_PBLK, pl = pr - pb * DFT_PBLK;
  const int nbl = NBT - pb * DFT_PBLK < DFT_PBLK ? NBT - pb * DFT_PBLK : DFT_PBLK;
  *qstride = (size_t)nbl * cstride * 8;
  return ((size_t)pb * DFT_PBLK * NQ + pl) * cstride * 8;
}

DFT_DEV int dft_div(int x, unsigned magic) { return magic ? (int)(((unsigned long long)(unsigned)x * magic) >> 32) : x; }

DFT_DEV void dft_split4(float a, float b, float c, float d, u32x2* hi, u32x2* lo) {
  const f32x4 x = {a, b, c, d};
  const half4 h = __builtin_convertvector(x, half4);
  *hi = __builtin_bit_cast(u32x2, h);
#ifdef DFT_SPLIT_LO_PAIR
  u32x2 l;
  l[0] = DFT_SPLIT_LO_PAIR(a, b, (*hi)[0]);
  l[1] = DFT_SPLIT_LO_PAIR(c, d, (*hi)[1]);
  *lo = l;
#else
  const half4 l = __builtin_convertvector(x - __builtin_convertvector(h, f32x4), half4);
  *lo = __builtin_bit_cast(u32x2, l);
#endif
}

DFT_DEV half8 dft_frag(const u32x4* p) { return __builtin_bit_cast(half8, *p); }

DFT_DEV f32x16 dft_mma3(half8 ah, half8 al, half8 bh, half8 bl, f32x16 acc) {
  acc = DFT_MFMA(ah, bl, acc);
  acc = DFT_MFMA(al, bh, acc);
  acc = DFT_MFMA(ah, bh, acc);
  return acc;
}

template <int NT, int KS>
DFT_DEV void dft_product_rega(f32x16* acc, const half8* ah, const half8* al, int ksn, const u32x4* B, int bstride, int nt0,
                              int ntstep, int l31, int hw) {
  constexpr int KR = KS ? KS : DFT_KREG;
  half8 bh[2][NT], bl[2][NT];
#define DFT_REGA_READ(KSTEP, SET)                                                                                          \
  _Pragma("unroll") for (int j = 0; j < NT; ++j) {                                                                         \
    bh[SET][j] = dft_frag(B + (size_t)((2 * (KSTEP) + hw) * 2 + 0) * bstride + (nt0 + ntstep * j) * 32 + l31);             \
    bl[SET][j] = dft_frag(B + (size_t)((2 * (KSTEP) + hw) * 2 + 1) * bstride + (nt0 + ntstep * j) * 32 + l31);             \
  }
  if (DFT_PIPE_REGA) DFT_REGA_READ(0, 0)
#pragma unroll
  for (int ks = 0; ks < KR; ++ks) {
    if (KS || ks < ksn) {
      if (DFT_PIPE_REGA) {
        if (ks + 1 < KR && (KS || ks + 1 < ksn)) DFT_REGA_READ(ks + 1, (ks + 1) & 1)
        DFT_SCHED_FENCE();
      } else {
        DFT_REGA_READ(ks, ks & 1)
      }
#pragma unroll
      for (int j = 0; j < NT; ++j) acc[j] = dft_mma3(ah[ks], al[ks], bh[ks & 1][j], bl[ks & 1][j], acc[j]);
      if (DFT_PIPE_REGA) DFT_SCHED_FENCE();
    }
  }
#undef DFT_REGA_READ
}

template <int KS>
DFT_DEV void dft_product_rega_any(f32x16* acc, int ntiles, const half8* ah, const half8* al, int ksn, const u32x4* B, int bstride,
                                  int nt0, int ntstep, int l31, int hw) {
  if (ntiles == 3) dft_product_rega<3, KS>(acc, ah, al, ksn, B, bstride, nt0, ntstep, l31, hw);
  else if (ntiles == 2) dft_product_rega<2, KS>(acc, ah, al, ksn, B, bstride, nt0, ntstep, l31, hw);
  else if (ntiles == 1) dft_product_rega<1, KS>(acc, ah, al, ksn, B, bstride, nt0, ntstep, l31, hw);
}

template <int NT, bool SHARE, int NW, int PIPE_MODE>
DFT_DEV void dft_product_lds(f32x16* acc, int ks0, int ks1, const u32x4* A, int astride, const u32x4* B, int bstride, int t0, int mtn,
                             int l31, int hw) {
  constexpr int NA = SHARE ? 1 : NT;
  int tm[NT], tn[NT];
#pragma unroll
  for (int j = 0; j < NT; ++j) {
    const int t = t0 + NW * j;
    tn[j] = t / mtn;
    tm[j] = t - tn[j] * mtn;
  }
  half8 ah[2][NA], al[2][NA], bh[2][NT], bl[2][NT];
#define DFT_LDS_READ(KSTEP, SET)                                                                                           \
  {                                                                                                                        \
    const int kc_ = (KSTEP) < ks1 ? (KSTEP) : ks1 - 1;                                                                     \
    _Pragma("unroll") for (int j = 0; j < NA; ++j) {                                                                       \
      ah[SET][j] = dft_frag(A + (size_t)((2 * kc_ + hw) * 2 + 0) * astride + tm[j] * 32 + l31);                            \
      al[SET][j] = dft_frag(A + (size_t)((2 * kc_ + hw) * 2 + 1) * astride + tm[j] * 32 + l31);                            \
    }                                                                                                                      \
    _Pragma("unroll") for (int j = 0; j < NT; ++j) {                                                                       \
      bh[SET][j] = dft_frag(B + (size_t)((2 * kc_ + hw) * 2 + 0) * bstride + tn[j] * 32 + l31);                            \
      bl[SET][j] = dft_frag(B + (size_t)((2 * kc_ + hw) * 2 + 1) * bstride + tn[j] * 32 + l31);                            \
    }                                                                                                                      \
  }
#define DFT_LDS_MMA(SET)                                                                                                   \
  DFT_SCHED_FENCE();                                                                                                       \
  _Pragma("unroll") for (int j = 0; j < NT; ++j)                                                                           \
    acc[j] = dft_mma3(ah[SET][SHARE ? 0 : j], al[SET][SHARE ? 0 : j], bh[SET][j], bl[SET][j], acc[j]);                    \
  DFT_SCHED_FENCE();
  if (ks0 >= ks1) return;
  constexpr bool PIPE = PIPE_MODE == 2 || (PIPE_MODE == 1 && SHARE);
  if (!PIPE) {
    for (int ks = ks0; ks < ks1; ++ks) {
      DFT_LDS_READ(ks, 0)
      _Pragma("unroll") for (int j = 0; j < NT; ++j)
        acc[j] = dft_mma3(ah[0][SHARE ? 0 : j], al[0][SHARE ? 0 : j], bh[0][j], bl[0][j], acc[j]);
    }
    return;
  }
  DFT_LDS_READ(ks0, 0)
  int ks = ks0;
  for (; ks + 1 < ks1; ks += 2) {
    DFT_LDS_READ(ks + 1, 1)
    DFT_LDS_MMA(0)
    DFT_LDS_READ(ks + 2, 0)
    DFT_LDS_MMA(1)
  }
  if (ks < ks1) {
    DFT_LDS_MMA(0)
  }
#undef DFT_LDS_READ
#undef DFT_LDS_MMA
}

template <int NW, int PIPE_MODE>
DFT_DEV void dft_product_lds_any(f32x16* acc, int ntiles, int ks0, int ks1, const u32x4* A, int astride, const u32x4* B, int bstride,
                                 int t0, int mtn, int l31, int hw) {
  const bool share = mtn == NW;
  if (ntiles == 3) {
    if (share) dft_product_lds<3, true, NW, PIPE_MODE>(acc, ks0, ks1, A, astride, B, bstride, t0, mtn, l31, hw);
    else dft_product_lds<3, false, NW, PIPE_MODE>(acc, ks0, ks1, A, astride, B, bstride, t0, mtn, l31, hw);
  } else if (ntiles == 2) {
    if (share) dft_product_lds<2, true, NW, PIPE_MODE>(acc, ks0, ks1, A, astride, B, bstride, t0, mtn, l31, hw);
    else dft_product_lds<2, false, NW, PIPE_MODE>(acc, ks0, ks1, A, astride, B, bstride, t0, mtn, l31, hw);
  } else if (ntiles == 1) {
    dft_product_lds<1, true, NW, PIPE_MODE>(acc, ks0, ks1, A, astride, B, bstride, t0, mtn, l31, hw);
  }
}

DFT_DEV void dft_matrix_unit(int which, int unit, int P, int Q, const double* twP, const double* twQ, u32x4* out) {
  const int V = Q / 2 + 1;
  const bool r2 = which == 1 && dft_radix2(P);
  if (r2 && unit >= DFT_R2_MATU) {
    const int u = 2 * (unit - DFT_R2_MATU);
    u32x4 o;
    for (int t = 0; t < 4; ++t) o[t] = __builtin_bit_cast(unsigned, (float)twP[2 * u + t]);
    *out = o;
    return;
  }
  const int tws = r2 ? 2 : 1;
  if (r2) P /= 2;
  const int Pp = dft_round_up(P, 8);
  int cols, kidx, hl, col;
  double vals[8];
  if (which == 0) cols = dft_round_up(2 * V, 32);
  else if (which == 1 || which == 2) cols = dft_round_up(2 * P, 32);
  else cols = dft_round_up(Q, 32);
  col = unit % cols;
  hl = (unit / cols) & 1;
  kidx = unit / (2 * cols);
  for (int t = 0; t < 8; ++t) {
    const int k = kidx * 8 + t;
    double x = 0.0;
    if (which == 0) {
      const int v = col >> 1, ri = col & 1;
      if (k < Q && v < V) x = twQ[2 * (int)(((long long)v * k) % Q) + ri] * 16384.0;
    } else if (which == 1) {
      const int ri = k / Pp, h = k - ri * Pp, u = col >> 1, ro = col & 1;
      if (h < P && u < P && ri < 2) {
        const int a = (int)(((long long)u * h) % P) * tws;
        const double c = twP[2 * a], s = -twP[2 * a + 1];
        x = (ro == 0 ? (ri == 0 ? c : s) : (ri == 0 ? -s : c)) * 16384.0;
      }
    } else if (which == 2) {
      const int ri = k / Pp, u = k - ri * Pp, h = col >> 1, ro = col & 1;
      if (u < P && h < P && ri < 2) {
        const int a = (int)(((long long)u * h) % P);
        const double c = twP[2 * a], s = -twP[2 * a + 1];
        x = (ro == 0 ? (ri == 0 ? c : -s) : (ri == 0 ? s : c)) * 16384.0;
      }
    } else {
      const int v = k >> 1, ri = k & 1;
      if (v < V && col < Q) {
        const double a = (v == 0 || 2 * v == Q) ? 1.0 : 2.0;
        x = a * twQ[2 * (int)(((long long)v * col) % Q) + ri] * 8192.0;
      }
    }
    vals[t] = x;
  }
  unsigned w[4];
  for (int t = 0; t < 4; ++t) {
    unsigned short b[2];
    for (int e = 0; e < 2; ++e) {
      const double x = vals[2 * t + e];
      const _Float16 h = (_Float16)x;
      const _Float16 r = hl == 0 ? h : (_Float16)(x - (double)h);
      b[e] = __builtin_bit_cast(unsigned short, r);
    }
    w[t] = (unsigned)b[0] | ((unsigned)b[1] << 16);
  }
  u32x4 o;
  o[0] = w[0];
  o[1] = w[1];
  o[2] = w[2];
  o[3] = w[3];
  *out = o;
}

template <bool TILED, bool FAST, int G, int NW, int KS2 = 0>
DFT_DEV void dft_forward_body(const float* corr,
                              const float* invn,
                              float* X,
                              const u32x4* FqT, const u32x4* Fp2, const DftPlan& pl, int C, int Cpad, int NBT, int iters) {
  constexpr int THR = NW * 64;
  constexpr bool ALDS = G == 8;
  constexpr bool R2 = !ALDS && KS2 == 8;
  unsigned char* smem = DFT_LDS;
  const int tid = DFT_TID, lane = tid & 63, l31 = lane & 31, hw = lane >> 5;
  const int wv = DFT_UNIFORM(tid >> 6);
  const int P = pl.P, V = pl.V, Pp = pl.Pp, Wk = pl.Wk, N1 = pl.N1, Mx = pl.Mx, N2 = pl.N2, LH = pl.LH, LW = pl.LW, W = pl.W, H = pl.H;
  const int MxS = Mx + 1, N2S = N2 + 1;
  const int CG = (C + G - 1) / G, HW = H * W;
  const bool unit_norm = invn == nullptr;
  u32x4* ldsF = reinterpret_cast<u32x4*>(smem);
  u32x4* ldsU = reinterpret_cast<u32x4*>(smem + pl.lds_const);
  unsigned char* ldsUb = smem + pl.lds_const;
  const int nF = (Wk / 8) * 2 * N1;
  for (int i = tid; i < nF; i += THR) ldsF[i] = FqT[i];
  const unsigned char* ldsTw = smem + pl.lds_const + pl.lds_union + DFT_R2_LDS_TW;
  if (R2 && tid < DFT_R2_TWU) reinterpret_cast<u32x4*>(smem + pl.lds_const + pl.lds_union + DFT_R2_LDS_TW)[tid] = Fp2[DFT_R2_MATU + tid];
  u32x4* ldsP = ldsF + nF;
  if (ALDS)
    for (int i = tid; i < (2 * Pp / 8) * 2 * pl.M2; i += THR) ldsP[i] = Fp2[i];

  const int mt1n = Mx / 32, nt1n = N1 / 32, nt2n = N2 / 32, mt2n = pl.M2 / 32;
  const int ks1n = Wk / 16, ks2n = 2 * Pp / 16;
  const int mt2 = wv & 3;
  constexpr int KR2 = R2 ? 4 : KS2 ? KS2 : DFT_KREG;
  half8 fp2h[KR2], fp2l[KR2];
  if (R2) {
#pragma unroll
    for (int ks = 0; ks < KR2; ++ks) {
      fp2h[ks] = dft_frag(Fp2 + ((size_t)((2 * ks + hw) * 2 + 0)) * 64 + (mt2 & 1) * 32 + l31);
      fp2l[ks] = dft_frag(Fp2 + ((size_t)((2 * ks + hw) * 2 + 1)) * 64 + (mt2 & 1) * 32 + l31);
    }
  } else if (!ALDS) {
#pragma unroll
    for (int ks = 0; ks < KR2; ++ks) {
      const int kc = ks < ks2n ? ks : 0, mc = mt2 < mt2n ? mt2 : 0;
      fp2h[ks] = dft_frag(Fp2 + ((size_t)((2 * kc + hw) * 2 + 0)) * pl.M2 + mc * 32 + l31);
      fp2l[ks] = dft_frag(Fp2 + ((size_t)((2 * kc + hw) * 2 + 1)) * pl.M2 + mc * 32 + l31);
    }
  }
  if (!ALDS) {
#pragma unroll
    for (int ks = 0; ks < KR2; ++ks) {
      DFT_LANDED(fp2h[ks]);
      DFT_LANDED(fp2l[ks]);
    }
  }

  constexpr int NSLOT = ALDS ? 2 : 3 * 512 / THR;
  const int npos = Pp * (Wk / 4);
  f32x4 pc[NSLOT][G], pn[NSLOT];
#define DFT_FWD_ITER(IT)                                                                                     \
  const int pr_ = dft_div((IT), pl.inv_cg), cg_ = (IT)-pr_ * CG;                                             \
  const int nb_ = TILED ? dft_div(pr_, pl.inv_t) : pr_, tile_ = TILED ? pr_ - nb_ * pl.T : 0;               \
  const int ty_ = TILED ? dft_div(tile_, pl.inv_tx) : 0, tx_ = TILED ? tile_ - ty_ * pl.TX : 0;             \
  const int Y0 = TILED ? ty_ * pl.TH - pl.oy : 0, X0 = TILED ? tx_ * pl.TW - pl.ox : 0;                     \
  const int c0_ = cg_ * G;
#define DFT_FWD_POS(TID, S)                                                                                  \
  const int i_ = (TID) + (S)*THR;                                                                        \
  const int r_ = dft_div(i_, pl.inv_c4), c4_ = i_ - r_ * (Wk / 4);                                          \
  const int y_ = Y0 + r_, x_ = X0 + 4 * c4_;
#define DFT_FWD_PREFETCH(IT, TID) DFT_FWD_PREFETCH_SLOTS(IT, TID, 0, NSLOT)
#define DFT_FWD_PREFETCH_SLOTS(IT, TID, S0, S1)                                                              \
  {                                                                                                          \
    DFT_FWD_ITER(IT)                                                                                         \
     \
    const float* nrm_ = invn ? invn + (size_t)nb_ * HW : corr + ((size_t)nb_ * C + (c0_ < C ? c0_ : C - 1)) * HW; \
    _Pragma("unroll") for (int s = (S0); s < (S1); ++s) {                                                    \
      DFT_FWD_POS(TID, s)                                                                                    \
      if (FAST) {                                                                                            \
        const bool ok = i_ < npos && r_ < LH && 4 * c4_ < LW;                                                \
        const int off = ok ? y_ * W + x_ : 0;                                                                \
        pn[s] = *reinterpret_cast<const f32x4*>(nrm_ + off);                                                \
        _Pragma("unroll") for (int g = 0; g < G; ++g) {                                                  \
          const int c = c0_ + g < C ? c0_ + g : C - 1;                                                       \
          pc[s][g] = *reinterpret_cast<const f32x4*>(corr + ((size_t)nb_ * C + c) * HW + off);              \
        }                                                                                                    \
      } else {                                                                                               \
                                                                           \
        const bool rok = i_ < npos && r_ < LH && y_ >= 0 && y_ < H;                                          \
        const int off0 = y_ * W + x_;                                                                        \
        const bool vec = rok && off0 >= 0 && off0 + 3 < HW;                                                  \
        const int offv = vec ? off0 : 0;                                                                     \
        pn[s] = *reinterpret_cast<const f32x4u*>(nrm_ + offv);                                               \
        _Pragma("unroll") for (int g = 0; g < G; ++g) {                                                      \
          const int c = c0_ + g < C ? c0_ + g : C - 1;                                                       \
          pc[s][g] = *reinterpret_cast<const f32x4u*>(corr + ((size_t)nb_ * C + c) * HW + offv);             \
        }                                                                                                    \
        if (rok && !vec) {                                                                                   \
          _Pragma("unroll") for (int e = 0; e < 4; ++e) {                                                    \
            const bool ok = 4 * c4_ + e < LW && x_ + e >= 0 && x_ + e < W;                                   \
            const int off = ok ? y_ * W + x_ + e : 0;                                                        \
            pn[s][e] = nrm_[off];                                                                            \
            _Pragma("unroll") for (int g = 0; g < G; ++g) {                                                  \
              const int c = c0_ + g < C ? c0_ + g : C - 1;                                                   \
              pc[s][g][e] = corr[((size_t)nb_ * C + c) * HW + off];                                          \
            }                                                                                                \
          }                                                                                                  \
        }                                                                                                    \
      }                                                                                                      \
    }                                                                                                        \
  }
  const int first = (DFT_GRID & 7) == 0 ? (DFT_BID & 7) * (DFT_GRID >> 3) + (DFT_BID >> 3) : DFT_BID;
  if (first < iters) DFT_FWD_PREFETCH(first, tid)
  DFT_BARRIER();

  DFT_STAMP_BEGIN()
  for (int it = first; it < iters; it += DFT_GRID) {
    int tl = tid;
#ifndef OS2D_HOST_EMU
    asm volatile("" : "+v"(tl));
#endif
    const int lane = tl & 63, l31 = lane & 31, hw = lane >> 5;
    DFT_FWD_ITER(it)
    {
#pragma unroll
      for (int s = 0; s < NSLOT; ++s) {
        DFT_FWD_POS(tl, s)
        if (i_ < npos) {
          float nsc[4];
#pragma unroll
          for (int e = 0; e < 4; ++e) {
            const bool ok = FAST ? (r_ < LH && 4 * c4_ < LW) : (r_ < LH && y_ >= 0 && y_ < H && 4 * c4_ + e < LW && x_ + e >= 0 && x_ + e < W);
            nsc[e] = ok ? (unit_norm ? 32768.0f : pn[s][e] * 32768.0f) : 0.f;
          }
#pragma unroll
          for (int g = 0; g < G; ++g) {
            u32x2 hi = {0u, 0u}, lo = {0u, 0u};
            if (c0_ + g < C)
              dft_split4(fmaxf(pc[s][g][0], 0.f) * nsc[0], fmaxf(pc[s][g][1], 0.f) * nsc[1], fmaxf(pc[s][g][2], 0.f) * nsc[2],
                         fmaxf(pc[s][g][3], 0.f) * nsc[3], &hi, &lo);
            const int m = g * Pp + (R2 ? (r_ & 1) * 32 + (r_ >> 1) : r_);
            unsigned char* dst = ldsUb + ((size_t)((c4_ >> 1) * 2) * MxS + m) * 16 + (c4_ & 1) * 8;
            *reinterpret_cast<u32x2*>(dst) = hi;
            *reinterpret_cast<u32x2*>(dst + (size_t)MxS * 16) = lo;
          }
        }
      }
      for (int i = tid; i < (Mx - G * Pp) * (Wk / 8) * 2; i += THR) {
        const int m = G * Pp + i % (Mx - G * Pp), kh = i / (Mx - G * Pp);
        ldsU[(size_t)kh * MxS + m] = u32x4{0u, 0u, 0u, 0u};
      }
    }
    DFT_BARRIER();
    DFT_STAMP(0)

    f32x16 acc[3];
    int tm[3], tn[3];
    int nt1w = 0;
#pragma unroll
    for (int j = 0; j < 3; ++j) {
      const int t = wv + NW * j;
      const bool mine = t < mt1n * nt1n;
      tn[j] = mine ? t / mt1n : 0;
      tm[j] = mine ? t - tn[j] * mt1n : -1;
      nt1w += mine ? 1 : 0;
#pragma unroll
      for (int r = 0; r < 16; ++r) acc[j][r] = 0.f;
    }
    dft_product_lds_any<NW, DFT_PIPE_LDS ? 2 : 0>(acc, nt1w, 0, ks1n, ldsU, MxS, ldsF, N1, wv, mt1n, l31, hw);
    DFT_BARRIER();
    DFT_STAMP(1)

#pragma unroll
    for (int j = 0; j < 3; ++j) {
      if (tm[j] < 0) continue;
      const int n = tn[j] * 32 + l31, v = n >> 1, ri = n & 1;
#pragma unroll
      for (int q = 0; q < 4; ++q) {
        const int mb = tm[j] * 32 + 8 * q;
        const int img = dft_div(mb, pl.inv_pp), h0 = mb - img * Pp + 4 * hw;
        if (v < V && img < G) {
          u32x2 hi, lo;
          const float sc = 1.0f / 2097152.0f;
          dft_split4(acc[j][4 * q] * sc, acc[j][4 * q + 1] * sc, acc[j][4 * q + 2] * sc, acc[j][4 * q + 3] * sc, &hi, &lo);
          const int kg = R2 ? (h0 >> 5) * 8 + ri * 4 + ((h0 & 31) >> 3) : ri * (Pp / 8) + (h0 >> 3);
          unsigned char* dst = ldsUb + ((size_t)(kg * 2) * N2S + img * V + v) * 16 + (h0 & 4) * 2;
          *reinterpret_cast<u32x2*>(dst) = hi;
          *reinterpret_cast<u32x2*>(dst + (size_t)N2S * 16) = lo;
        }
      }
    }
    DFT_BARRIER();
    DFT_STAMP(2)

    f32x16 xc[3];
    int un[3], um[3];
    int nt2w = 0;
#pragma unroll
    for (int j = 0; j < 3; ++j) {
      const int t = wv + NW * j;
      const int nt = ALDS ? t / mt2n : (wv >> 2) + (NW / 4) * j;
      const bool mine = ALDS ? t < mt2n * nt2n : (nt < nt2n && mt2 < mt2n);
      un[j] = mine ? nt : -1;
      um[j] = ALDS ? t - nt * mt2n : mt2;
      nt2w += mine ? 1 : 0;
#pragma unroll
      for (int r = 0; r < 16; ++r) xc[j][r] = 0.f;
    }
    const int itn = it + DFT_GRID < iters ? it + DFT_GRID : it;
    {
      if (ALDS) {
        dft_product_lds_any<NW, DFT_PIPE_LDS ? 2 : 0>(xc, nt2w, 0, ks2n, ldsP, pl.M2, ldsU, N2S, wv, mt2n, l31, hw);
        DFT_FWD_PREFETCH_SLOTS(itn, tl, 0, NSLOT)
      } else if (!R2 && (DFT_FWD_PREFETCH_AFTER == 1 || (DFT_FWD_PREFETCH_AFTER == 2 && KS2 > 0 && KS2 <= 6))) {
        dft_product_rega_any<KS2>(xc, nt2w, fp2h, fp2l, ks2n, ldsU, N2S, wv >> 2, NW / 4, l31, hw);
        DFT_FWD_PREFETCH_SLOTS(itn, tl, 0, NSLOT)
      } else if (R2) {
        DFT_FWD_PREFETCH_SLOTS(itn, tl, 0, NSLOT)
        dft_product_rega_any<4>(xc, nt2w, fp2h, fp2l, 4, ldsU + (size_t)(mt2 >> 1) * 16 * N2S, N2S, wv >> 2, NW / 4, l31, hw);
      } else {
        DFT_FWD_PREFETCH_SLOTS(itn, tl, 0, NSLOT)
        dft_product_rega_any<KS2>(xc, nt2w, fp2h, fp2l, ks2n, ldsU, N2S, wv >> 2, NW / 4, l31, hw);
      }
    }
    DFT_BARRIER();
    DFT_STAMP(3)

    const int XS = P * 8 * G + 16;
#pragma unroll
    for (int j = 0; j < 3; ++j) {
      if (un[j] < 0) continue;
      const int n2 = un[j] * 32 + l31;
      const int img = dft_div(n2, pl.inv_v), v = n2 - img * V;
#pragma unroll
      for (int q = 0; q < 4; ++q) {
        const int u0 = (um[j] * 32 + 8 * q + 4 * hw) >> 1;
        if (img < G && u0 < P) {
          const float sc = 1.0f / 4194304.0f;
          f32x4 o;
          o[0] = xc[j][4 * q] * sc;
          o[1] = xc[j][4 * q + 1] * sc;
          o[2] = xc[j][4 * q + 2] * sc;
          o[3] = xc[j][4 * q + 3] * sc;
          *reinterpret_cast<f32x4*>(ldsUb + (size_t)v * XS + (u0 >> 2) * (G * 32) + img * 32 + (u0 & 3) * 8) = o;
        }
      }
    }
    DFT_BARRIER();
    DFT_STAMP(4)

    {
      const int per_v = (P / 4) * (G * 2), npieces = V * per_v;
      size_t qstride;
      float* dstbase = X + dft_spectra_pair0(pr_, NBT, pl.NBINS / 4, Cpad, &qstride) + (size_t)c0_ * 8;
      if (R2) {
        constexpr int per_h = (DFT_R2_P / 8) * (G * 2);
        for (int i = tl; i < V * per_h; i += THR) {
          const int v = i / per_h, rem = i - v * per_h;
          const int uq = rem / (2 * G), jj = rem - uq * (2 * G);
          const unsigned char* src = ldsUb + (size_t)v * XS + uq * (G * 32) + jj * 16;
          const f32x4 e = *reinterpret_cast<const f32x4*>(src);
          const f32x4 o = *reinterpret_cast<const f32x4*>(src + (DFT_R2_P / 8) * (G * 32));
          const f32x4 w = *reinterpret_cast<const f32x4*>(ldsTw + (4 * uq + 2 * (jj & 1)) * 8);
          f32x4 t;
          t[0] = w[0] * o[0] - w[1] * o[1];
          t[1] = w[0] * o[1] + w[1] * o[0];
          t[2] = w[2] * o[2] - w[3] * o[3];
          t[3] = w[2] * o[3] + w[3] * o[2];
          float* dst = dstbase + (size_t)(v * (P / 4) + uq) * qstride + jj * 4;
          DFT_STREAM_STORE(reinterpret_cast<f32x4*>(dst), e + t);
          DFT_STREAM_STORE(reinterpret_cast<f32x4*>(dst + (size_t)(DFT_R2_P / 8) * qstride), e - t);
        }
      } else
      for (int i = tl; i < npieces; i += THR) {
        const int v = dft_div(i, pl.inv_pq), rem = i - v * per_v;
        const int uq = rem / (2 * G), jj = rem - uq * (2 * G);
        const f32x4 val = *reinterpret_cast<const f32x4*>(ldsUb + (size_t)v * XS + uq * (G * 32) + jj * 16);
        DFT_STREAM_STORE(reinterpret_cast<f32x4*>(dstbase + (size_t)(v * (P / 4) + uq) * qstride + jj * 4), val);
      }
      const int qpad0 = (P * V) / 4, qpad1 = pl.NBINS / 4;
      for (int i = tl; i < (qpad1 - qpad0) * 2 * G; i += THR)
        *reinterpret_cast<f32x4*>(dstbase + (size_t)(qpad0 + i / (2 * G)) * qstride + (i % (2 * G)) * 4) = f32x4{0.f, 0.f, 0.f, 0.f};
    }
    DFT_BARRIER();
    DFT_STAMP(5)
  }
  DFT_STAMP_END(0)
#undef DFT_FWD_ITER
#undef DFT_FWD_POS
#undef DFT_FWD_PREFETCH
#undef DFT_FWD_PREFETCH_SLOTS
}

template <bool TILED, int KSA = 0, int G = DFT_G>
DFT_DEV void dft_inverse_body(const float* Y,
                              const float* bp,
                              int MTP, unsigned char* out,
                              const u32x4* E2, const u32x4* Gq, const DftPlan& pl, int Cout, int NBT, int PLANE, int Ws,
                              int BASE, int iters, DFT_FLAG bad_flag, int zero_borders) {
  unsigned char* smem = DFT_LDS;
  const int tid = DFT_TID, lane = tid & 63, l31 = lane & 31, hw = lane >> 5;
  const int wv = DFT_UNIFORM(tid >> 6);
  const int P = pl.P, V = pl.V, Pp = pl.Pp, N2 = pl.N2, MB = pl.MB, KB = pl.KB, NBo = pl.NBo, H = pl.H, W = pl.W;
  const int N2S = N2 + 1, MBS = MB + 1;
  const int OG = Cout / G;
  constexpr bool ALDS = G == 8;
  constexpr int LG = G == 8 ? 3 : 2;
  u32x4* ldsG = reinterpret_cast<u32x4*>(smem);
  u32x4* ldsU = reinterpret_cast<u32x4*>(smem + pl.lds_const);
  unsigned char* ldsUb = smem + pl.lds_const;
  float* smaxw = reinterpret_cast<float*>(smem + pl.lds_const + pl.lds_union);
  const int nG = (KB / 8) * 2 * NBo, NQ = dft_round_up(pl.Q, 32);
  for (int i = tid; i < nG; i += DFT_THR) {
    const int kh = i / NBo, n = i - kh * NBo;
    ldsG[i] = Gq[(size_t)kh * NQ + n];
  }
  const int MAfull = dft_round_up(2 * P, 32);
  u32x4* ldsE = ldsG + nG;
  if (ALDS)
    for (int i = tid; i < (2 * Pp / 8) * 2 * MAfull; i += DFT_THR) ldsE[i] = E2[i];

  const int mtAn = pl.MA / 32, ntAn = N2 / 32, ksAn = 2 * Pp / 16;
  const int mtBn = MB / 32, ntBn = NBo / 32, ksBn = KB / 16;
  const int mtA = wv & 3;
  constexpr int KRA = KSA ? KSA : DFT_KREG;
  half8 e2h[KRA], e2l[KRA];
  if (!ALDS) {
#pragma unroll
    for (int ks = 0; ks < KRA; ++ks) {
      const int kc = ks < ksAn ? ks : 0, mc = mtA < mtAn ? mtA : 0;
      e2h[ks] = dft_frag(E2 + ((size_t)((2 * kc + hw) * 2 + 0)) * MAfull + mc * 32 + l31);
      e2l[ks] = dft_frag(E2 + ((size_t)((2 * kc + hw) * 2 + 1)) * MAfull + mc * 32 + l31);
    }
#pragma unroll
    for (int ks = 0; ks < KRA; ++ks) {
      DFT_LANDED(e2h[ks]);
      DFT_LANDED(e2l[ks]);
    }
  }

  constexpr int NITEM = 3;
  const int uoct = Pp / 8, nitem = G * V * uoct;
  f32x4 py[NITEM][4];
#define DFT_INV_PREFETCH(IT, TID) DFT_INV_PREFETCH_ITEMS(IT, TID, 0, NITEM)
#define DFT_INV_PREFETCH_ITEMS(IT, TID, S0, S1)                                             \
  {                                                                                         \
    const int pr_ = dft_div((IT), pl.inv_og), og_ = (IT)-pr_ * OG;                          \
    size_t qstride;                                                                         \
    const float* src_ = Y + dft_spectra_pair0(pr_, NBT, pl.NBINS / 4, Cout, &qstride) + (size_t)og_ * G * 8; \
    _Pragma("unroll") for (int s = (S0); s < (S1); ++s) {                                   \
      const int e_ = (TID) + s * DFT_THR;                                                   \
      const int ec_ = e_ < nitem ? e_ : 0;                                                  \
      const int pimg_ = ec_ & (G - 1), prest_ = ec_ >> LG;                                  \
      const int pv_ = dft_div(prest_, pl.inv_kg), puo_ = prest_ - pv_ * (Pp / 8);           \
      const int q0_ = pv_ * (P / 4) + 2 * puo_;                                             \
      const bool ptwo_ = 8 * puo_ + 4 < P;                                                  \
      const float* p0_ = src_ + (size_t)q0_ * qstride + pimg_ * 8;                          \
      const float* p1_ = src_ + (size_t)(ptwo_ ? q0_ + 1 : q0_) * qstride + pimg_ * 8;      \
      py[s][0] = *reinterpret_cast<const f32x4*>(p0_);                                     \
      py[s][1] = *reinterpret_cast<const f32x4*>(p0_ + 4);                                 \
      py[s][2] = *reinterpret_cast<const f32x4*>(p1_);                                     \
      py[s][3] = *reinterpret_cast<const f32x4*>(p1_ + 4);                                 \
    }                                                                                       \
  }
#define DFT_INV_ITEM(E)                                                                     \
  const int img_ = (E) & (G - 1), rest_ = (E) >> LG;                                        \
  const int v_ = dft_div(rest_, pl.inv_kg), uo_ = rest_ - v_ * uoct;                        \
  const bool two_ = 8 * uo_ + 4 < P;
#define DFT_INV_MAXIMA(TID)                                                                 \
  {                                                                                         \
    float m = 0.f;                                                                          \
    _Pragma("unroll") for (int s = 0; s < NITEM; ++s)                                       \
      if ((TID) + s * DFT_THR < nitem) {                                                    \
        DFT_INV_ITEM((TID) + s * DFT_THR)                                                   \
        (void)img_;                                                                         \
        (void)v_;                                                                           \
        (void)uo_;                                                                          \
        _Pragma("unroll") for (int k = 0; k < 4; ++k)                                       \
          if (k < 2 || two_) {                                                              \
            _Pragma("unroll") for (int e = 0; e < 4; ++e) m = fmaxf(m, fabsf(py[s][k][e])); \
          }                                                                                 \
      }                                                                                     \
    if (G == 4) m = fmaxf(m, DFT_SHFL_XOR(m, 4));                                           \
    m = fmaxf(m, DFT_SHFL_XOR(m, 8));                                                       \
    m = fmaxf(m, DFT_SHFL_XOR(m, 16));                                                      \
    m = fmaxf(m, DFT_SHFL_XOR(m, 32));                                                      \
    if (lane < G) smaxw[wv * G + lane] = m;                                                 \
  }
  bool bad = false;
  const int first = (DFT_GRID & 7) == 0 ? (DFT_BID & 7) * (DFT_GRID >> 3) + (DFT_BID >> 3) : DFT_BID;
  if (first < iters) {
    DFT_INV_PREFETCH(first, tid)
    DFT_INV_MAXIMA(tid)
  }
  DFT_BARRIER();

  DFT_STAMP_BEGIN()
  for (int it = first; it < iters; it += DFT_GRID) {
    int tl = tid;
#ifndef OS2D_HOST_EMU
    asm volatile("" : "+v"(tl));
#endif
    const int lane = tl & 63, l31 = lane & 31, hw = lane >> 5;
    const int pr = dft_div(it, pl.inv_og), og = it - pr * OG;
    const int nb = TILED ? dft_div(pr, pl.inv_t) : pr, tile = TILED ? pr - nb * pl.T : 0;
    const int ty = TILED ? dft_div(tile, pl.inv_tx) : 0, tx = TILED ? tile - ty * pl.TX : 0;
    const int y0 = TILED ? ty * pl.TH : 0, x0 = TILED ? tx * pl.TW : 0, oy = TILED ? pl.oy : 0, ox = TILED ? pl.ox : 0;
    const int TH_ = TILED ? pl.TH : H, TW_ = TILED ? pl.TW : W;
    const int o0 = og * G;

    DFT_STAMP(0)
    float simg = 1.f, cinv[4] = {0.f, 0.f, 0.f, 0.f};
    {
#pragma unroll
      for (int g = 0; g < G; ++g) {
        float m = 0.f;
#pragma unroll
        for (int w = 0; w < DFT_WAVES; ++w) m = fmaxf(m, smaxw[w * G + g]);
        int E = (int)((__builtin_bit_cast(unsigned, m) >> 23) & 0xffu) - 127;
        if (!(m > 0.f) || E < -100) E = -100;
        if (E > 100) E = 100;
        const float s = __builtin_bit_cast(float, (unsigned)(13 - E + 127) << 23);
        const float sinv = __builtin_bit_cast(float, (unsigned)(E - 13 + 127) << 23);
        if (g == (tl & (G - 1))) simg = s;
        const float ci = sinv * __builtin_bit_cast(float, (unsigned)(pl.eT - 13 + 127) << 23) / (float)(P * pl.Q);
        if (G == 4 || (g >> 2) == hw) cinv[g & 3] = ci;
      }
    }
#pragma unroll
    for (int s = 0; s < NITEM; ++s) {
      const int e = tl + s * DFT_THR;
      if (e < nitem) {
        DFT_INV_ITEM(e)
        const int img = img_, v = v_, uo = uo_;
        const bool two = two_;
        float re[8], im[8];
#pragma unroll
        for (int k = 0; k < 4; ++k) {
          const bool ok = k < 2 || two;
          re[2 * k] = ok ? py[s][k][0] * simg : 0.f;
          im[2 * k] = ok ? py[s][k][1] * simg : 0.f;
          re[2 * k + 1] = ok ? py[s][k][2] * simg : 0.f;
          im[2 * k + 1] = ok ? py[s][k][3] * simg : 0.f;
        }
        u32x2 h0, l0, h1, l1;
        u32x4 t;
        const size_t n = (size_t)img * V + v;
        dft_split4(re[0], re[1], re[2], re[3], &h0, &l0);
        dft_split4(re[4], re[5], re[6], re[7], &h1, &l1);
        t[0] = h0[0], t[1] = h0[1], t[2] = h1[0], t[3] = h1[1];
        ldsU[(size_t)((uo)*2 + 0) * N2S + n] = t;
        t[0] = l0[0], t[1] = l0[1], t[2] = l1[0], t[3] = l1[1];
        ldsU[(size_t)((uo)*2 + 1) * N2S + n] = t;
        dft_split4(im[0], im[1], im[2], im[3], &h0, &l0);
        dft_split4(im[4], im[5], im[6], im[7], &h1, &l1);
        t[0] = h0[0], t[1] = h0[1], t[2] = h1[0], t[3] = h1[1];
        ldsU[(size_t)((uoct + uo) * 2 + 0) * N2S + n] = t;
        t[0] = l0[0], t[1] = l0[1], t[2] = l1[0], t[3] = l1[1];
        ldsU[(size_t)((uoct + uo) * 2 + 1) * N2S + n] = t;
      }
    }
    DFT_BARRIER();
    DFT_STAMP(1)

    f32x16 ta[3];
    int an[3], am[3];
    int ntaw = 0;
#pragma unroll
    for (int j = 0; j < 3; ++j) {
      const int t = wv + DFT_WAVES * j;
      const int nt = ALDS ? t / mtAn : (wv >> 2) + 2 * j;
      const bool mine = ALDS ? t < mtAn * ntAn : (nt < ntAn && mtA < mtAn);
      an[j] = mine ? nt : -1;
      am[j] = ALDS ? t - nt * mtAn : mtA;
      ntaw += mine ? 1 : 0;
#pragma unroll
      for (int r = 0; r < 16; ++r) ta[j][r] = 0.f;
    }
    const int itn = it + DFT_GRID < iters ? it + DFT_GRID : it;
    {
      if (ALDS) {
        dft_product_lds_any<DFT_WAVES, DFT_PIPE_LDS ? 1 : 0>(ta, ntaw, 0, ksAn, ldsE, MAfull, ldsU, N2S, wv, mtAn, l31, hw);
        DFT_INV_PREFETCH_ITEMS(itn, tl, 0, NITEM)
      } else if (DFT_INV_PREFETCH_AFTER == 1 || (DFT_INV_PREFETCH_AFTER == 2 && KSA > 0 && KSA <= 6)) {
        dft_product_rega_any<KSA>(ta, ntaw, e2h, e2l, ksAn, ldsU, N2S, wv >> 2, 2, l31, hw);
        DFT_INV_PREFETCH_ITEMS(itn, tl, 0, NITEM)
      } else {
        DFT_INV_PREFETCH_ITEMS(itn, tl, 0, NITEM)
        dft_product_rega_any<KSA>(ta, ntaw, e2h, e2l, ksAn, ldsU, N2S, wv >> 2, 2, l31, hw);
      }
    }
    DFT_BARRIER();
    DFT_STAMP(2)

    {
      const float sc = __builtin_bit_cast(float, (unsigned)(127 - 14 - pl.eT) << 23);
#pragma unroll
      for (int j = 0; j < 3; ++j) {
        if (an[j] < 0) continue;
        const int n = an[j] * 32 + l31;
        const int img = dft_div(n, pl.inv_v), v = n - img * V;
        if (img >= G) continue;
#pragma unroll
        for (int q = 0; q < 4; ++q) {
          const int h0 = (am[j] * 32 + 8 * q + 4 * hw) >> 1;
          u32x2 hi, lo;
          dft_split4(ta[j][4 * q] * sc, ta[j][4 * q + 1] * sc, ta[j][4 * q + 2] * sc, ta[j][4 * q + 3] * sc, &hi, &lo);
          unsigned char* d0 = ldsUb + ((size_t)((v >> 2) * 2) * MBS + (size_t)h0 * G + img) * 16 + (v & 3) * 4;
          *reinterpret_cast<unsigned*>(d0) = hi[0];
          *reinterpret_cast<unsigned*>(d0 + (size_t)MBS * 16) = lo[0];
          *reinterpret_cast<unsigned*>(d0 + G * 16) = hi[1];
          *reinterpret_cast<unsigned*>(d0 + G * 16 + (size_t)MBS * 16) = lo[1];
        }
      }
      for (int v = V; v < KB / 2; ++v)
        for (int m = tl; m < MB; m += DFT_THR) {
          unsigned char* d0 = ldsUb + ((size_t)((v >> 2) * 2) * MBS + m) * 16 + (v & 3) * 4;
          *reinterpret_cast<unsigned*>(d0) = 0u;
          *reinterpret_cast<unsigned*>(d0 + (size_t)MBS * 16) = 0u;
        }
    }
    DFT_BARRIER();
    DFT_STAMP(3)

    f32x16 yc[3];
    int bm[3], bn[3];
    int ntbw = 0;
#pragma unroll
    for (int j = 0; j < 3; ++j) {
      const int t = wv + DFT_WAVES * j;
      const bool mine = t < mtBn * ntBn;
      bn[j] = mine ? t / mtBn : 0;
      bm[j] = mine ? t - bn[j] * mtBn : -1;
      ntbw += mine ? 1 : 0;
#pragma unroll
      for (int r = 0; r < 16; ++r) yc[j][r] = 0.f;
    }
    dft_product_lds_any<DFT_WAVES, DFT_PIPE_LDS ? 1 : 0>(yc, ntbw, 0, ksBn, ldsU, MBS, ldsG, NBo, wv, mtBn, l31, hw);
    DFT_INV_MAXIMA(tl)
    DFT_STAMP(4)

    {
      const bool planes = zero_borders == DFT_OUT_PLANES;
      float bias[4], osc[4];
#pragma unroll
      for (int g = 0; g < 4; ++g) {
        bias[g] = bp[o0 + (G == 8 ? 4 * hw : 0) + g];
        osc[g] = bp[2 * MTP + o0 + (G == 8 ? 4 * hw : 0) + g];
      }
      const int grp = o0 >> 3, slot = o0 & 7;
      unsigned char* hi_unit = out + (((size_t)nb * ((Cout + 7) >> 3) + grp) * 2 + 0) * (size_t)PLANE * 16 + slot * 2;
      unsigned char* lo_unit = out + (((size_t)nb * ((Cout + 7) >> 3) + grp) * 2 + 1) * (size_t)PLANE * 16 + slot * 2;
      if (zero_borders == DFT_OUT_SHB_BORDERS && (!TILED || tile == 0)) {
        const int rows = H * (Ws - W), tail0 = BASE + H * Ws, npad = BASE + rows + (PLANE - tail0);
        for (int k = tl; k < npad; k += DFT_THR) {
          int cell;
          if (k < BASE) cell = k;
          else if (k < BASE + rows) {
            const int jj = k - BASE, hr = jj / (Ws - W);
            cell = BASE + hr * Ws + W + (jj - hr * (Ws - W));
          } else cell = tail0 + (k - BASE - rows);
          if (G == 8) {
            *reinterpret_cast<u32x4*>(hi_unit + (size_t)cell * 16) = u32x4{0u, 0u, 0u, 0u};
            *reinterpret_cast<u32x4*>(lo_unit + (size_t)cell * 16) = u32x4{0u, 0u, 0u, 0u};
          } else {
            *reinterpret_cast<u32x2*>(hi_unit + (size_t)cell * 16) = u32x2{0u, 0u};
            *reinterpret_cast<u32x2*>(lo_unit + (size_t)cell * 16) = u32x2{0u, 0u};
          }
        }
      }
#pragma unroll
      for (int j = 0; j < 3; ++j) {
        if (bm[j] < 0) continue;
        const int wwin = bn[j] * 32 + l31, tw = wwin - ox;
#pragma unroll
        for (int q = 0; q < 4; ++q) {
          const int hwin = G == 8 ? bm[j] * 4 + q : (bm[j] * 32 + 8 * q + 4 * hw) >> 2, th = hwin - oy;
          const int h = y0 + th, w = x0 + tw;
          const bool inside = th >= 0 && th < TH_ && tw >= 0 && tw < TW_ && h < H && w < W;
          if (G == 8 || inside) {
            float t[4];
#pragma unroll
            for (int g = 0; g < 4; ++g) {
              const float pre = yc[j][4 * q + g] * cinv[g] + bias[g];
              t[g] = fmaxf(pre, 0.f) * osc[g];
              if (inside && (!(fabsf(t[g]) <= 65504.f) || pre != pre)) bad = true;
            }
            if (planes) {
              if (inside) {
                float* dst = reinterpret_cast<float*>(out) + ((size_t)nb * Cout + o0 + (G == 8 ? 4 * hw : 0)) * ((size_t)H * W) + (size_t)h * W + w;
#pragma unroll
                for (int g = 0; g < 4; ++g) dst[(size_t)g * H * W] = t[g] * (1.0f / 32768.0f);
              }
              continue;
            }
            u32x2 hi, lo;
            dft_split4(t[0], t[1], t[2], t[3], &hi, &lo);
            const size_t off = ((size_t)BASE + (size_t)h * Ws + w) * 16;
            if (G == 8) {
              const u32x2 send = hw ? hi : lo, keep = hw ? lo : hi;
              u32x2 recv;
              recv[0] = DFT_SHFL_XOR_U32(send[0], 32);
              recv[1] = DFT_SHFL_XOR_U32(send[1], 32);
              const u32x4 unit = hw ? u32x4{recv[0], recv[1], keep[0], keep[1]} : u32x4{keep[0], keep[1], recv[0], recv[1]};
              if (inside) *reinterpret_cast<u32x4*>((hw ? lo_unit : hi_unit) + off) = unit;
            } else {
              *reinterpret_cast<u32x2*>(hi_unit + off) = hi;
              *reinterpret_cast<u32x2*>(lo_unit + off) = lo;
            }
          }
        }
      }
    }
    DFT_BARRIER();
    DFT_STAMP(5)
  }
  DFT_STAMP_END(8)
  if (DFT_FLAG_SET(bad_flag) && DFT_BALLOT(bad) != 0ull) {
    if ((tid & 63) == 0) DFT_RAISE(bad_flag);
  }
#undef DFT_INV_MAXIMA
#undef DFT_INV_ITEM
#undef DFT_INV_PREFETCH
#undef DFT_INV_PREFETCH_ITEMS
}

}
```

### os2d_amd/csrc/dft_mfma.hip

```cpp
#include "tile_common.h"
#include <map>
#include <mutex>
#include <utility>

extern __shared__ __attribute__((aligned(16))) unsigned char os2d_dft_smem[];

#define DFT_DEV __device__ __forceinline__
#define DFT_HD __host__ __device__ static inline
#define DFT_MEMBER __device__ __forceinline__
#define DFT_TID ((int)threadIdx.x)
#define DFT_BID ((int)blockIdx.x)
#define DFT_GRID ((int)gridDim.x)
#define DFT_LDS os2d_dft_smem
#define DFT_BARRIER() asm volatile("s_waitcnt lgkmcnt(0)\n\ts_barrier" ::: "memory")
#define DFT_MFMA(a, b, c) __builtin_amdgcn_mfma_f32_32x32x16_f16(a, b, c, 0, 0, 0)
#define DFT_SHFL_XOR(v, m) __shfl_xor(v, m, 64)
#define DFT_SHFL_XOR_U32(v, m) ((unsigned)__shfl_xor((int)(v), m, 64))
#define DFT_BALLOT(p) __builtin_amdgcn_ballot_w64(p)
#define DFT_UNIFORM(x) __builtin_amdgcn_readfirstlane(x)
#define DFT_SCHED_FENCE() __builtin_amdgcn_sched_barrier(0)
#define DFT_LANDED(X) asm volatile("" : "+v"(X))
#define DFT_SPLIT_LO_PAIR(a, b, hi) os2d_split_lo_pair(a, b, hi)
#define DFT_STREAM_STORE(P, V) os2d_stream_store(P, V)
#define DFT_FLAG Os2dRangeFlag
#define DFT_FLAG_SET(f) ((f).word != nullptr)
#define DFT_RAISE(f) os2d_raise(f)
#ifdef OS2D_DIAG_DFT_STAMPS
__device__ unsigned long long os2d_dft_stamps[16];
#define DFT_STAMP_BEGIN() unsigned long long st_acc_[6] = {0, 0, 0, 0, 0, 0}, st_n_ = 0, st_last_ = wall_clock64();
#define DFT_STAMP(K)                                   \
  {                                                    \
    const unsigned long long t_ = wall_clock64();      \
    st_acc_[K] += t_ - st_last_;                       \
    st_last_ = t_;                                     \
    if ((K) == 5) ++st_n_;                             \
  }
#define DFT_STAMP_END(BASE)                                                                   \
  if (threadIdx.x == 0) {                                                                     \
    for (int k_ = 0; k_ < 6; ++k_) atomicAdd(&os2d_dft_stamps[(BASE) + k_], st_acc_[k_]);     \
    atomicAdd(&os2d_dft_stamps[(BASE) + 6], st_n_);                                           \
  }
#endif
#include "dft_mfma.h"

namespace {

using namespace os2d_dft;

template <bool TILED, bool FAST, int G, int NW, int KS>
__global__ __launch_bounds__(NW * 64, 8 / NW) void dft_forward_kernel(const float* __restrict__ corr, const float* __restrict__ invn,
                                                                      float* __restrict__ X, const u32x4* __restrict__ FqT,
                                                                      const u32x4* __restrict__ Fp2, DftPlan pl, int C, int Cpad, int NBT,
                                                                      int iters) {
  dft_forward_body<TILED, FAST, G, NW, KS>(corr, invn, X, FqT, Fp2, pl, C, Cpad, NBT, iters);
}

template <bool TILED, int KS, int G>
__global__ __launch_bounds__(DFT_THR, 1) void dft_inverse_kernel(const float* __restrict__ Y, const float* __restrict__ bp, int MTP,
                                                                 unsigned char* __restrict__ out, const u32x4* __restrict__ E2,
                                                                 const u32x4* __restrict__ Gq, DftPlan pl, int Cout, int NBT, int PLANE,
                                                                 int Ws, int BASE, int iters, Os2dRangeFlag status, int zero_borders) {
  dft_inverse_body<TILED, KS, G>(Y, bp, MTP, out, E2, Gq, pl, Cout, NBT, PLANE, Ws, BASE, iters, status, zero_borders);
}

typedef void (*dft_forward_fn)(const float*, const float*, float*, const u32x4*, const u32x4*, DftPlan, int, int, int, int);
typedef void (*dft_inverse_fn)(const float*, const float*, int, unsigned char*, const u32x4*, const u32x4*, DftPlan, int, int, int, int, int,
                               int, Os2dRangeFlag, int);
template <int G, int NW, int KS>
dft_forward_fn dft_forward_variant(const DftPlan& pl) {
  return pl.T > 1 ? dft_forward_kernel<true, false, G, NW, KS> : (pl.fast ? dft_forward_kernel<false, true, G, NW, KS> : dft_forward_kernel<false, false, G, NW, KS>);
}
template <int G, int NW>
dft_forward_fn dft_forward_pick(const DftPlan& pl) {
  if constexpr (G == 8) {
    return dft_forward_variant<G, NW, 0>(pl);
  } else {
    switch (2 * pl.Pp / 16) {
      case 5: return dft_forward_variant<G, NW, 5>(pl);
      case 6: return dft_forward_variant<G, NW, 6>(pl);
      case 7: return dft_forward_variant<G, NW, 7>(pl);
      case 8: return dft_forward_variant<G, NW, 8>(pl);
      default: return dft_forward_variant<G, NW, 0>(pl);
    }
  }
}
template <int KS, int G = DFT_G>
dft_inverse_fn dft_inverse_variant(const DftPlan& pl) {
  return pl.T > 1 ? dft_inverse_kernel<true, KS, G> : dft_inverse_kernel<false, KS, G>;
}
dft_inverse_fn dft_inverse_pick(const DftPlan& pl) {
  if (pl.G == 8) return dft_inverse_variant<0, 8>(pl);
  switch (2 * pl.Pp / 16) {
    case 5: return dft_inverse_variant<5>(pl);
    case 6: return dft_inverse_variant<6>(pl);
    case 7: return dft_inverse_variant<7>(pl);
    case 8: return dft_inverse_variant<8>(pl);
    default: return dft_inverse_variant<0>(pl);
  }
}

__global__ __launch_bounds__(256) void dft_matrices_kernel(const double* __restrict__ twP, const double* __restrict__ twQ, int P, int Q,
                                                           u32x4* __restrict__ out) {
  const int n0 = dft_units_fqt(P, Q), n1 = n0 + dft_units_fp2(P, Q), n2 = n1 + dft_units_e2(P, Q), n3 = n2 + dft_units_gq(P, Q);
  const int i = blockIdx.x * 256 + threadIdx.x;
  if (i >= n3) return;
  const int which = i < n0 ? 0 : i < n1 ? 1 : i < n2 ? 2 : 3;
  const int base = which == 0 ? 0 : which == 1 ? n0 : which == 2 ? n1 : n2;
  dft_matrix_unit(which, i - base, P, Q, twP, twQ, out + i);
}

bool dft_plan_cached(int H, int W, DftPlan* out, bool g8 = true) {
  static const bool g8_enabled = [] {
    const char* e = getenv("OS2D_DFT_G8");
    return !(e && e[0] == '0');
  }();
  struct Entry {
    bool ok, ok8;
    DftPlan pl, pl8;
  };
  static std::mutex mu;
  static std::map<std::pair<int, int>, Entry> cache;
  {
    std::lock_guard<std::mutex> lock(mu);
    auto it = cache.find({H, W});
    if (it != cache.end()) {
      if (it->second.ok) *out = (g8 && g8_enabled && it->second.ok8) ? it->second.pl8 : it->second.pl;
      return it->second.ok;
    }
  }
  Entry e = {};
  e.ok = dft_make_plan(H, W, &e.pl);
  e.ok8 = e.ok && dft_plan_g8(e.pl, &e.pl8);
  if (e.ok) *out = (g8 && g8_enabled && e.ok8) ? e.pl8 : e.pl;
  std::lock_guard<std::mutex> lock(mu);
  if (cache.size() >= 4096) cache.clear();
  cache[{H, W}] = e;
  return e.ok;
}

int dft_grid(int iters, int per_cu = 1) {
  int g = iters < 256 * per_cu ? iters : 256 * per_cu;
  return os2d_round_up(g, 8);
}

}

int os2d_dft_plan(int H, int W, int* P, int* Q, int* nbins, int* tiles) {
  DftPlan pl;
  if (H < 1 || W < 1 || !dft_plan_cached(H, W, &pl)) return 0;
  if (P) *P = pl.P;
  if (Q) *Q = pl.Q;
  if (nbins) *nbins = pl.NBINS;
  if (tiles) {
    tiles[0] = pl.TY;
    tiles[1] = pl.TX;
    tiles[2] = pl.TH;
    tiles[3] = pl.TW;
    tiles[4] = pl.LH;
    tiles[5] = pl.LW;
  }
  return 1;
}

size_t os2d_dft_matrices_size(int P, int Q) { return dft_matrices_units(P, Q) * 16; }

int os2d_launch_dft_matrices(const double* twP64, const double* twQ64, int P, int Q, void* out, hipStream_t stream) {
  if (P < 4 || (P & 3) || P > DFT_MAXP || Q < 2 || (Q & 1) || Q / 2 + 1 > DFT_MAXV) {
    os2d_set_error("dft_matrices: transform %d x %d is outside the kernels' range (P %% 4 == 0, P <= %d, Q even, Q/2 + 1 <= %d)", P, Q,
                   DFT_MAXP, DFT_MAXV);
    return -3;
  }
  const int n = (int)dft_matrices_units(P, Q);
  hipLaunchKernelGGL(dft_matrices_kernel, dim3((n + 255) / 256), dim3(256), 0, stream, twP64, twQ64, P, Q, static_cast<u32x4*>(out));
  return os2d_launched("dft_matrices");
}

int os2d_launch_dft_forward(const float* corr, const float* inv, float* X, const void* matrices, int NB, int C, int Cpad, int H, int W,
                            hipStream_t stream) {
  DftPlan pl;
  if (!dft_plan_cached(H, W, &pl)) {
    os2d_set_error("dft_forward: no transform plan for a %dx%d map", H, W);
    return -3;
  }
  if (pl.G == 8 && Cpad < dft_round_up(C, 8)) dft_plan_cached(H, W, &pl, false);
  const int G = pl.G;
  if (Cpad < dft_round_up(C, G)) {
    os2d_set_error("dft_forward: channel stride %d < %d", Cpad, dft_round_up(C, G));
    return -1;
  }
  if (G == 4 && pl.Pp == 64 && !dft_radix2(pl.P)) {
    os2d_set_error("dft_forward: a plan of 8 k-steps with %d rows (the radix-2 kernel takes 64)", pl.P);
    return -3;
  }
  const int CG = (C + G - 1) / G, NBT = NB * pl.T, iters = NBT * CG;
  pl.inv_cg = dft_magic((unsigned)CG);
  const u32x4* FqT = static_cast<const u32x4*>(matrices);
  const u32x4* Fp2 = FqT + dft_units_fqt(pl.P, pl.Q);
  auto kern = G == 8 ? dft_forward_pick<8, 8>(pl) : dft_forward_pick<4, 8>(pl);
  if (int rc = os2d_set_dynamic_lds(kern, pl.lds_total, "dft_forward")) return rc;
  hipLaunchKernelGGL(kern, dim3(dft_grid(iters)), dim3(DFT_THR), pl.lds_total, stream, corr, inv, X, FqT, Fp2, pl,
                     C, Cpad, NBT, iters);
  return os2d_launched("dft_forward");
}

int os2d_launch_dft_inverse(const float* Y, const float* bp, int MTP, void* out, const void* matrices, int NB, int Cout, int H, int W,
                            Os2dRangeFlag status, int zero_borders, hipStream_t stream) {
  DftPlan pl;
  if (!dft_plan_cached(H, W, &pl)) {
    os2d_set_error("dft_inverse: no transform plan for a %dx%d map", H, W);
    return -3;
  }
  if (Cout % 8) {
    os2d_set_error("dft_inverse: Cout %d must be a multiple of 8", Cout);
    return -1;
  }
  const int OG = Cout / pl.G, NBT = NB * pl.T, iters = NBT * OG;
  pl.inv_og = dft_magic((unsigned)OG);
  const u32x4* E2 = static_cast<const u32x4*>(matrices) + dft_units_fqt(pl.P, pl.Q) + dft_units_fp2(pl.P, pl.Q);
  const u32x4* Gq = E2 + dft_units_e2(pl.P, pl.Q);
  auto kern = dft_inverse_pick(pl);
  if (int rc = os2d_set_dynamic_lds(kern, pl.lds_total, "dft_inverse")) return rc;
  hipLaunchKernelGGL(kern, dim3(dft_grid(iters)), dim3(DFT_THR), pl.lds_total, stream, Y, bp, MTP, static_cast<unsigned char*>(out), E2, Gq,
                     pl, Cout, NBT, os2d_plane(H, W), os2d_ws(W), os2d_base(W), iters, status, zero_borders);
  return os2d_launched("dft_inverse");
}

extern "C" int os2d_debug_dft_stamps(unsigned long long* out16, int reset) {
#ifdef OS2D_DIAG_DFT_STAMPS
  if (out16 && hipMemcpyFromSymbol(out16, HIP_SYMBOL(os2d_dft_stamps), 16 * sizeof(unsigned long long)) != hipSuccess) return -4;
  if (reset) {
    unsigned long long z[16] = {0};
    if (hipMemcpyToSymbol(HIP_SYMBOL(os2d_dft_stamps), z, sizeof(z)) != hipSuccess) return -4;
  }
  return 0;
#else
  (void)out16, (void)reset;
  os2d_set_error("os2d_debug_dft_stamps: this library was built without -DOS2D_DIAG_DFT_STAMPS");
  return -1;
#endif
}
```

### os2d_amd/csrc/os2d_common.h

```cpp
#pragma once
#include <hip/hip_runtime.h>
#include <stdint.h>

#include "../csrc_shared/abi_common.h"

#define OS2D_PAD 3
#define OS2D_T 15
#define OS2D_K 225
#define OS2D_KP 226
#define OS2D_QROWS 256
#define OS2D_MAX_W_DIRECT7 209
#define OS2D_MAX_W_LINEAR5 316
#define OS2D_MAX_W 3600
#define OS2D_MAX_H 2784
#define OS2D_XSPEC_CPAD 232
#define OS2D_G 29
#define OS2D_RNORM_EXP 12
#define OS2D_STATUS_F16_RANGE 1

struct Os2dRangeFlag {
  int* word;
  int value;
};
#ifdef __HIPCC__
__device__ __forceinline__ void os2d_raise(Os2dRangeFlag f) {
  __hip_atomic_store(f.word, f.value, __ATOMIC_RELAXED, __HIP_MEMORY_SCOPE_SYSTEM);
}
#endif

typedef float f32x16 __attribute__((ext_vector_type(16)));
typedef float f32x4 __attribute__((ext_vector_type(4)));

static inline __host__ __device__ int os2d_round_up(int x, int m) { return ((x + m - 1) / m) * m; }
static inline __host__ __device__ int os2d_ws(int W) { return W + OS2D_PAD; }
static inline __host__ __device__ int os2d_base(int W) { return os2d_round_up(OS2D_PAD * os2d_ws(W) + OS2D_PAD, 4); }
static inline __host__ __device__ int os2d_plane(int H, int W) {
  return os2d_round_up(os2d_base(W) + (H + OS2D_PAD) * os2d_ws(W) + OS2D_PAD, 64);
}
__device__ __forceinline__ void os2d_corr_norm_finalize_one(unsigned long long* __restrict__ sumfx, float* __restrict__ invn, size_t i) {
  const unsigned long long v = sumfx[i];
  sumfx[i] = 0ull;
  const float s = (v >> 62) ? __builtin_nanf("") : (float)((double)v * 5.6843418860808015e-14);
  invn[i] = 1.0f / (sqrtf(s) + 1e-6f);
}
template <class T>
__device__ __forceinline__ void os2d_stream_store(T* p, const T& v) {
  __builtin_nontemporal_store(v, p);
}
__device__ __forceinline__ unsigned os2d_split_lo_pair(float x0, float x1, unsigned hi) {
  unsigned lo;
  asm("v_fma_mixlo_f16 %0, %1, 1.0, -%3 op_sel_hi:[0,0,1]\n\t"
      "v_fma_mixhi_f16 %0, %2, 1.0, -%3 op_sel:[0,0,1] op_sel_hi:[0,0,1]"
      : "=&v"(lo)
      : "v"(x0), "v"(x1), "v"(hi));
  return lo;
}
__device__ __forceinline__ float os2d_relu(float v) { return v < 0.f ? 0.f : v; }
static inline __host__ __device__ bool os2d_interior(int n, int H, int W) {
  const int r = n - os2d_base(W);
  return r >= 0 && r < H * os2d_ws(W) && (r % os2d_ws(W)) < W;
}

int os2d_launch_fm_sumsq(const float* fm, float* sumsq, int A, int C, int HW, hipStream_t stream);
int os2d_launch_border_zero(float* rpad, int planes_total, int H, int W, hipStream_t stream);
int os2d_launch_corr_normalize(const float* corr, float* rpad, int NB, int H, int W, hipStream_t stream);
int os2d_launch_class_prepare(const float* src, int C, int h, int w, int normalize, float* q15, float* qp, hipStream_t stream);
int os2d_launch_pack_conv(const float* w, const float* b, const float* bn_w, const float* bn_b,
                          const float* bn_mean, const float* bn_var, float bn_eps, int Cout, int Cin, int KS,
                          int MT, float* wp, float* bp, hipStream_t stream);
int os2d_launch_border_zero_shb(void* rnorm, int NB, int H, int W, hipStream_t stream);
int os2d_launch_border_zero_shb_planes(void* buf, int planes, int H, int W, hipStream_t stream);
int os2d_launch_border_zero_shb_planes_norms(void* buf, int planes, int H, int W, void* sumfx, float* invn, size_t n, hipStream_t stream);
int os2d_launch_pack_conv_f16(const float* w, const float* b, const float* bn_w, const float* bn_b, const float* bn_mean,
                              const float* bn_var, float bn_eps, int Cout, int Cin, int KS, int MT, int steps_padded,
                              const int* wexp, const int* in_exp, const int* out_exp, void* wp, float* bp,
                              hipStream_t stream);
int os2d_class_prepare_partial_floats(int B, int C);
int os2d_launch_class_prepare_batch(const float* const* srcs, const int* sizes, int B, int C, int normalize, float* q15,
                                    float* qp, float* partial, hipStream_t stream);
int os2d_launch_corr_normalize_shb(const float* corr, void* rshb, int NB, int H, int W, hipStream_t stream);
int os2d_launch_corr(const float* fm, const float* qp, const float* sumsq, float* corr, void* rnorm ,
                     float* invn ,
                     int A, int B, int C, int H, int W, int shb, hipStream_t stream);
int os2d_launch_conv3_f16x3(const void* in, const void* wp, const float* bp, void* out, int NB, int P, int H, int W,
                            hipStream_t stream);
int os2d_launch_conv3_sample_decode(const void* in, const void* wp, const float* bp, const float* corr, int NB, int H, int W, int P,
                                    int inverse, int stride, int rec_field, int Bc, int Btot, int b0, float* loc, float* cls, float* corners,
                                    const int* flags, int epoch, int* host_status, hipStream_t stream);
int os2d_launch_conv_f16x3(int layer, const void* in, const void* wp, const float* bp, Os2dRangeFlag status, void* out, int NB,
                           int P, int H, int W, int terms, hipStream_t stream);
int os2d_launch_conv(int layer, const float* in, const float* wp, const float* bp, float* out,
                     int NB, int P, int H, int W, hipStream_t stream);
int os2d_launch_sample_decode(const float* corr, const float* params, int NB, int H, int W, int P, int inverse,
                              int stride, int rec_field, int Bc, int Btot, int b0, float* loc, float* cls,
                              float* corners, const int* flags , int epoch,
                              int* host_status , hipStream_t stream);
int os2d_launch_decode_boxes(const float* loc, int NB, int H, int W, int stride, int rec_field, float img_w,
                             float img_h, float* boxes, hipStream_t stream);
int os2d_launch_alignment_grids(const float* params, int NB, int H, int W, int P, int inverse, float* theta,
                                float* grids, hipStream_t stream);
int os2d_launch_nms(const float* boxes, const int* counts, int NC, int N, float thr, unsigned char* keep, int* num_keep,
                    void* workspace, hipStream_t stream);
int os2d_fft_plan(int H, int W, int* P, int* Q, int* nbins, int* tiles );
int os2d_launch_fft_forward(const float* corr, const float* inv, float* X, const float* twQ, const float* twP, int NB, int C,
                            int H, int W, hipStream_t stream);
int os2d_launch_fft_inverse(const float* Y, const float* bp, int MTP, void* out, const float* twQ, const float* twP, int NB,
                            int Cout, int H, int W, Os2dRangeFlag status, int layout ,
                            int out_fp32 ,
                            hipStream_t stream);
int os2d_launch_spectra_pack(const double* wfold, const double* twP64, const double* twQ64, int C, int Cout, int P, int Q,
                             int NBINS, int split, int u_fastest ,
                             void* out, void* workspace, hipStream_t stream);
size_t os2d_spectral_weight_floats(int C, int Cout, int NBINS);
int os2d_launch_spectral_gemm(const float* wspec, const float* X, float* Y, int NB, int C, int Cout, int NBINS,
                              hipStream_t stream);
size_t os2d_spectral_weight16_size(int C, int NBINS);
float os2d_spectral_xscale_for(int H, int W);
int os2d_launch_spectral_gemm_f16(const void* w16, const float* X, float* Y, int NB, int C, int Cout, int NBINS, float xscale,
                                  int x_quads , int Cpad,
                                  hipStream_t stream);
int os2d_dft_plan(int H, int W, int* P, int* Q, int* nbins, int* tiles );
size_t os2d_dft_matrices_size(int P, int Q);
int os2d_launch_dft_matrices(const double* twP64, const double* twQ64, int P, int Q, void* out, hipStream_t stream);
int os2d_launch_dft_forward(const float* corr, const float* inv, float* X, const void* matrices, int NB, int C, int Cpad, int H, int W,
                            hipStream_t stream);
enum { OS2D_DFT_OUT_SHB = 0, OS2D_DFT_OUT_SHB_BORDERS = 1, OS2D_DFT_OUT_PLANES = 2 };
int os2d_launch_dft_inverse(const float* Y, const float* bp, int MTP, void* out, const void* matrices, int NB, int Cout, int H, int W,
                            Os2dRangeFlag status, int form, hipStream_t stream);
int os2d_corr_groups(int C);
int os2d_launch_split_fm(const float* fm, const float* sumsq, void* fs, int A, int C, int HW, void* clear, size_t clear_words,
                         Os2dRangeFlag status, hipStream_t stream);
int os2d_launch_split_qp(const float* qp, void* qs, int B, int C, hipStream_t stream);
int os2d_launch_corr_f16x3(const void* fs, const void* qs, float* corr, void* rshb, float* invn, void* sumfx, int flags, int A,
                           int B, int C, int H, int W, hipStream_t stream);
int os2d_corr_f16x3_use_packed(int A, int B, int H, int W);
int os2d_launch_corr_sums_clear(void* sumfx, int A, int B, int H, int W, hipStream_t stream);
```

Baseline: 46240.

## Fuse conv1 inverse DFT with conv2 forward DFT in one kernel

Adds a fused kernel path that takes the conv1 output spectra, does the inverse DFT with bias and activation, and immediately runs the forward DFT for conv2 in LDS. It writes conv2 input spectra directly instead of storing spatial planes to global memory and reading them back. The path is on by default when the plan fits (untiled, group size, LDS budget) and can be disabled via OS2D_CONV2_FUSE=0. It costs more LDS per block, which may lower occupancy, and it adds a separate code path inside the forward kernel.

```diff
diff --git a/include/os2d_hip.h b/include/os2d_hip.h
--- a/include/os2d_hip.h
+++ b/include/os2d_hip.h
@@ -133,6 +133,7 @@
 int os2d_spectral_gemm_f16(const void* w16, const float* X, float* Y, int NB, int C, int Cout, int nbins, float xscale,
                            void* stream);
 
+#define OS2D_NO_FUSED_PLAN 1
 int os2d_dft_sizes(int H, int W, int* P, int* Q, int* nbins, int* tiles);
 int os2d_dft_channel_stride(int C);
 size_t os2d_dft_matrices_bytes(int P, int Q);
@@ -143,6 +144,8 @@
                      int* status, void* stream);
 int os2d_dft_inverse_planes(const float* Y, const float* packed_b, float* out, const void* matrices, int NB, int Cout, int H, int W,
                             int* status, void* stream);
+int os2d_dft_inverse_forward(const float* Y, const float* packed_b, float* X2, const void* matrices, int NB, int Cout, int H, int W,
+                             int* status, void* stream);
 int os2d_spectral_weights_build_dft(const double* wfold, const double* twP64, const double* twQ64, int C, int Cout, int P, int Q,
                                     int nbins, void* out, void* workspace, void* stream);
 int os2d_spectral_gemm_f16_quads(const void* w16, const float* X, float* Y, int NB, int C, int Cout, int nbins, float xscale,
diff --git a/os2d_amd/_lib.py b/os2d_amd/_lib.py
--- a/os2d_amd/_lib.py
+++ b/os2d_amd/_lib.py
@@ -57,6 +57,7 @@
     "os2d_head_forward_ex2": (_i, [_vp] * 8 + [_i] * 9 + [_vp, _vp, _vp, _vp, _sz, _vp, _i, _vp,
                                    ctypes.POINTER(_vp), ctypes.POINTER(_i), _vp, _vp, _vp, _vp, _vp]),
     "os2d_dft_inverse_planes": (_i, [_vp, _vp, _vp, _vp, _i, _i, _i, _i, _vp, _vp]),
+    "os2d_dft_inverse_forward": (_i, [_vp, _vp, _vp, _vp, _i, _i, _i, _i, _vp, _vp]),
     "os2d_head_workspace_bytes_ex": (_i, [_i, _i, _i, _i, _i, _i, _i, ctypes.POINTER(_sz)]),
     "os2d_prof_event_create": (_i, [ctypes.POINTER(_vp)]),
     "os2d_prof_event_destroy": (_i, [_vp]),
diff --git a/os2d_amd/csrc/abi.hip b/os2d_amd/csrc/abi.hip
--- a/os2d_amd/csrc/abi.hip
+++ b/os2d_amd/csrc/abi.hip
@@ -440,6 +440,11 @@
     return !(e && e[0] == '0');
   }();
   const bool conv2_freq = dft && wspec2 && conv2_freq_env;
+  static const bool conv2_fuse_env = [] {
+    const char* e = getenv("OS2D_CONV2_FUSE");
+    return !(e && e[0] == '0');
+  }();
+  const bool conv2_fused = conv2_freq && conv2_fuse_env && !dumps_active() && os2d_dft_has_fused_plan(H, W);
   const bool fp32_ops = precision == OS2D_PRECISION_F32 || precision == OS2D_PRECISION_FFT32;
   if (!fp32_ops && !qs) {
     os2d_set_error("os2d_head_forward: precision f16x3 / f16x2 needs the split class operand (os2d_class_split)");
@@ -539,9 +544,17 @@
                                                 os2d_spectral_xscale_for(tiles[4], tiles[5]), 1, xch, st)))
           return rc;
         mark(b0, 12);
-        if ((rc = os2d_launch_dft_inverse(yspec, b1, 128, h1, mats, NB, 128, H, W, whole_call,
-                                          conv2_freq ? OS2D_DFT_OUT_PLANES : inv_borders ? OS2D_DFT_OUT_SHB_BORDERS : OS2D_DFT_OUT_SHB, st)))
+        if (conv2_fused) {
+          mark(b0, 3);
+          mark(b0, 4);
+          if ((rc = os2d_launch_dft_inverse_forward(yspec, b1, 128, xspec, mats, NB, 128, 128, H, W, whole_call, st))) {
+            if (rc > 0) os2d_set_error("os2d_head_forward: the fused transform refused the plan of a %dx%d map", H, W);
+            return rc > 0 ? -3 : rc;
+          }
+        } else if ((rc = os2d_launch_dft_inverse(yspec, b1, 128, h1, mats, NB, 128, H, W, whole_call,
+                                                 conv2_freq ? OS2D_DFT_OUT_PLANES : inv_borders ? OS2D_DFT_OUT_SHB_BORDERS : OS2D_DFT_OUT_SHB, st))) {
           return rc;
+        }
       } else {
         if ((rc = os2d_launch_fft_forward(corr, invn, xspec, twQ, twP, NB, OS2D_K, H, W, st))) return rc;
         mark(b0, 11);
@@ -554,8 +567,10 @@
     } else {
       if ((rc = os2d_launch_conv(1, rpad, static_cast<const float*>(w1), b1, h1, NB, P, H, W, st))) return rc;
     }
-    mark(b0, 3);
-    mark(b0, 4);
+    if (!conv2_fused) {
+      mark(b0, 3);
+      mark(b0, 4);
+    }
     if (dumps_active() && b0 == 0) {
       const size_t PLb = os2d_plane(H, W);
       dump_slot(stream, 0, corr, (size_t)NB * OS2D_K * H * W * 4);
@@ -567,7 +582,7 @@
       dump_slot(stream, 4, h1, (size_t)NB * 128 * (conv2_freq ? (size_t)H * W : PLb) * 4);
     }
     if (conv2_freq) {
-      if ((rc = os2d_launch_dft_forward(h1, nullptr, xspec, twQ, NB, 128, 128, H, W, st))) return rc;
+      if (!conv2_fused && (rc = os2d_launch_dft_forward(h1, nullptr, xspec, twQ, NB, 128, 128, H, W, st))) return rc;
       if ((rc = os2d_launch_spectral_gemm_f16(wspec2, xspec, yspec, NB * fft_T, 128, 64, fft_bins,
                                               os2d_spectral_xscale_for(tiles[4], tiles[5]), 1, 128, st)))
         return rc;
@@ -855,12 +870,22 @@
 
 int os2d_dft_inverse_planes(const float* Y, const float* packed_b, float* out, const void* matrices, int NB, int Cout, int H, int W,
                             int* status, void* stream) {
-  if (!Y || !packed_b || !out || !matrices || NB < 1 || (Cout != 128 && Cout != 64) || H < 1 || W < 1) {
-    os2d_set_error("os2d_dft_inverse_planes: bad arguments (Cout must be 128 or 64)");
+  if (!Y || !packed_b || !out || !matrices || NB < 1 || Cout < 8 || Cout > 128 || (Cout & 7) || H < 1 || W < 1) {
+    os2d_set_error("os2d_dft_inverse_planes: bad arguments (Cout: a multiple of 8 up to 128)");
     return -1;
   }
   return os2d_launch_dft_inverse(Y, packed_b, Cout, out, matrices, NB, Cout, H, W, Os2dRangeFlag{status, OS2D_STATUS_F16_RANGE},
                                  OS2D_DFT_OUT_PLANES, os2d_stream(stream));
+}
+
+int os2d_dft_inverse_forward(const float* Y, const float* packed_b, float* X2, const void* matrices, int NB, int Cout, int H, int W,
+                             int* status, void* stream) {
+  if (!Y || !packed_b || !X2 || !matrices || NB < 1 || Cout < 8 || Cout > 128 || (Cout & 7) || H < 1 || W < 1) {
+    os2d_set_error("os2d_dft_inverse_forward: bad arguments (Cout: a multiple of 8 up to 128)");
+    return -1;
+  }
+  return os2d_launch_dft_inverse_forward(Y, packed_b, Cout, X2, matrices, NB, Cout, os2d_dft_channel_stride(Cout), H, W,
+                                         Os2dRangeFlag{status, OS2D_STATUS_F16_RANGE}, os2d_stream(stream));
 }
 
 int os2d_spectral_weights_build_dft(const double* wfold, const double* twP64, const double* twQ64, int C, int Cout, int P, int Q,
diff --git a/os2d_amd/csrc/dft_mfma.h b/os2d_amd/csrc/dft_mfma.h
--- a/os2d_amd/csrc/dft_mfma.h
+++ b/os2d_amd/csrc/dft_mfma.h
@@ -35,6 +35,7 @@
 #define DFT_STAMP(K)
 #define DFT_STAMP_BEGIN()
 #define DFT_STAMP_END(BASE)
+#define DFT_STAMP_END_FUSED()
 #endif
 
 #include "tile_common.h"
@@ -73,9 +74,13 @@
   int fast;
   unsigned inv_cg, inv_t, inv_tx, inv_c4, inv_v, inv_pq, inv_og, inv_kg, inv_pp;
   int lds_const, lds_union, lds_total;
+  int lds_fused;
+  int fused;
+  DFT_FLAG fused_flag;
 };
 
 DFT_HD int dft_round_up(int x, int m) { return (x + m - 1) / m * m; }
+DFT_HD int dft_fused_gq_cols(int W) { return dft_round_up(W, 16); }
 DFT_HD unsigned dft_magic(unsigned d) { return d > 1 ? (unsigned)(((1ull << 32) + d - 1) / d) : 0u; }
 
 DFT_HD int dft_units_fqt(int P, int Q) { return (dft_round_up(Q, 16) / 8) * 2 * dft_round_up(Q + 2, 32); }
@@ -139,6 +144,8 @@
   pl->lds_const = fqt > gq ? fqt : gq;
   pl->lds_union = dft_round_up(u, 256);
   pl->lds_total = pl->lds_const + pl->lds_union + 1024;
+  const int fused = fqt + (pl->KB / 8) * 2 * dft_fused_gq_cols(ncols) * 16 + pl->lds_union + 1024;
+  pl->lds_fused = fused <= 160 * 1024 ? fused : 0;
   return pl->lds_total <= 160 * 1024;
 }
 
@@ -153,6 +160,7 @@
   pl->oy = TY > 1 ? 3 : 0;
   pl->ox = TX > 1 ? 3 : 0;
   pl->fast = (pl->T == 1 && (W & 3) == 0) ? 1 : 0;
+  if (pl->T != 1) pl->lds_fused = 0;
   pl->inv_t = dft_magic((unsigned)pl->T);
   pl->inv_tx = dft_magic((unsigned)TX);
   pl->inv_c4 = dft_magic((unsigned)(pl->Wk / 4));
@@ -421,6 +429,125 @@
   o[2] = w[2];
   o[3] = w[3];
   *out = o;
+}
+
+
+template <int NW, int PIPE>
+DFT_DEV void dft_step_lds(f32x16* acc, int* tm, int* tn, int ks1n, const u32x4* ldsU, int MxS, const u32x4* ldsF, int N1, int wv,
+                           int mt1n, int nt1n, int l31, int hw) {
+  int nt1w = 0;
+#pragma unroll
+  for (int j = 0; j < 3; ++j) {
+    const int t = wv + NW * j;
+    const bool mine = t < mt1n * nt1n;
+    tn[j] = mine ? t / mt1n : 0;
+    tm[j] = mine ? t - tn[j] * mt1n : -1;
+    nt1w += mine ? 1 : 0;
+#pragma unroll
+    for (int r = 0; r < 16; ++r) acc[j][r] = 0.f;
+  }
+  dft_product_lds_any<NW, PIPE>(acc, nt1w, 0, ks1n, ldsU, MxS, ldsF, N1, wv, mt1n, l31, hw);
+}
+
+template <bool R2, int G>
+DFT_DEV void dft_fwd_write_r(const f32x16* acc, const int* tm, const int* tn, const DftPlan& pl, unsigned char* ldsUb, int V, int Pp,
+                             int N2S, int l31, int hw) {
+#pragma unroll
+  for (int j = 0; j < 3; ++j) {
+    if (tm[j] < 0) continue;
+    const int n = tn[j] * 32 + l31, v = n >> 1, ri = n & 1;
+#pragma unroll
+    for (int q = 0; q < 4; ++q) {
+      const int mb = tm[j] * 32 + 8 * q;
+      const int img = dft_div(mb, pl.inv_pp), h0 = mb - img * Pp + 4 * hw;
+      if (v < V && img < G) {
+        u32x2 hi, lo;
+        const float sc = 1.0f / 2097152.0f;
+        dft_split4(acc[j][4 * q] * sc, acc[j][4 * q + 1] * sc, acc[j][4 * q + 2] * sc, acc[j][4 * q + 3] * sc, &hi, &lo);
+        const int kg = R2 ? (h0 >> 5) * 8 + ri * 4 + ((h0 & 31) >> 3) : ri * (Pp / 8) + (h0 >> 3);
+        unsigned char* dst = ldsUb + ((size_t)(kg * 2) * N2S + img * V + v) * 16 + (h0 & 4) * 2;
+        *reinterpret_cast<u32x2*>(dst) = hi;
+        *reinterpret_cast<u32x2*>(dst + (size_t)N2S * 16) = lo;
+      }
+    }
+  }
+}
+
+template <bool ALDS, int NW>
+DFT_DEV int dft_step_rega_tiles(f32x16* xc, int* un, int* um, int wv, int mt2, int mt2n, int nt2n) {
+  int nt2w = 0;
+#pragma unroll
+  for (int j = 0; j < 3; ++j) {
+    const int t = wv + NW * j;
+    const int nt = ALDS ? t / mt2n : (wv >> 2) + (NW / 4) * j;
+    const bool mine = ALDS ? t < mt2n * nt2n : (nt < nt2n && mt2 < mt2n);
+    un[j] = mine ? nt : -1;
+    um[j] = ALDS ? t - nt * mt2n : mt2;
+    nt2w += mine ? 1 : 0;
+#pragma unroll
+    for (int r = 0; r < 16; ++r) xc[j][r] = 0.f;
+  }
+  return nt2w;
+}
+
+template <int G>
+DFT_DEV void dft_fwd_stage(const f32x16* xc, const int* un, const int* um, const DftPlan& pl, unsigned char* ldsUb, int P, int V, int XS,
+                           int l31, int hw) {
+#pragma unroll
+  for (int j = 0; j < 3; ++j) {
+    if (un[j] < 0) continue;
+    const int n2 = un[j] * 32 + l31;
+    const int img = dft_div(n2, pl.inv_v), v = n2 - img * V;
+#pragma unroll
+    for (int q = 0; q < 4; ++q) {
+      const int u0 = (um[j] * 32 + 8 * q + 4 * hw) >> 1;
+      if (img < G && u0 < P) {
+        const float sc = 1.0f / 4194304.0f;
+        f32x4 o;
+        o[0] = xc[j][4 * q] * sc;
+        o[1] = xc[j][4 * q + 1] * sc;
+        o[2] = xc[j][4 * q + 2] * sc;
+        o[3] = xc[j][4 * q + 3] * sc;
+        *reinterpret_cast<f32x4*>(ldsUb + (size_t)v * XS + (u0 >> 2) * (G * 32) + img * 32 + (u0 & 3) * 8) = o;
+      }
+    }
+  }
+}
+
+template <bool R2, int G, int THR>
+DFT_DEV void dft_fwd_store(float* X, const DftPlan& pl, const unsigned char* ldsUb, const unsigned char* ldsTw, int pr, int c0, int NBT,
+                           int Cpad, int P, int V, int XS, int tl) {
+  const int per_v = (P / 4) * (G * 2), npieces = V * per_v;
+  size_t qstride;
+  float* dstbase = X + dft_spectra_pair0(pr, NBT, pl.NBINS / 4, Cpad, &qstride) + (size_t)c0 * 8;
+  if (R2) {
+    constexpr int per_h = (DFT_R2_P / 8) * (G * 2);
+    for (int i = tl; i < V * per_h; i += THR) {
+      const int v = i / per_h, rem = i - v * per_h;
+      const int uq = rem / (2 * G), jj = rem - uq * (2 * G);
+      const unsigned char* src = ldsUb + (size_t)v * XS + uq * (G * 32) + jj * 16;
+      const f32x4 e = *reinterpret_cast<const f32x4*>(src);
+      const f32x4 o = *reinterpret_cast<const f32x4*>(src + (DFT_R2_P / 8) * (G * 32));
+      const f32x4 w = *reinterpret_cast<const f32x4*>(ldsTw + (4 * uq + 2 * (jj & 1)) * 8);
+      f32x4 t;
+      t[0] = w[0] * o[0] - w[1] * o[1];
+      t[1] = w[0] * o[1] + w[1] * o[0];
+      t[2] = w[2] * o[2] - w[3] * o[3];
+      t[3] = w[2] * o[3] + w[3] * o[2];
+      float* dst = dstbase + (size_t)(v * (P / 4) + uq) * qstride + jj * 4;
+      DFT_STREAM_STORE(reinterpret_cast<f32x4*>(dst), e + t);
+      DFT_STREAM_STORE(reinterpret_cast<f32x4*>(dst + (size_t)(DFT_R2_P / 8) * qstride), e - t);
+    }
+  } else
+  for (int i = tl; i < npieces; i += THR) {
+    const int v = dft_div(i, pl.inv_pq), rem = i - v * per_v;
+    const int uq = rem / (2 * G), jj = rem - uq * (2 * G);
+    const f32x4 val = *reinterpret_cast<const f32x4*>(ldsUb + (size_t)v * XS + uq * (G * 32) + jj * 16);
+    DFT_STREAM_STORE(reinterpret_cast<f32x4*>(dstbase + (size_t)(v * (P / 4) + uq) * qstride + jj * 4), val);
+  }
+  const int qpad0 = (P * V) / 4, qpad1 = pl.NBINS / 4;
+  for (int i = tl; i < (qpad1 - qpad0) * 2 * G; i += THR)
+    *reinterpret_cast<f32x4*>(dstbase + (size_t)(qpad0 + i / (2 * G)) * qstride + (i % (2 * G)) * 4) = f32x4{0.f, 0.f, 0.f, 0.f};
 }
 
 template <bool TILED, bool FAST, int G, int NW, int KS2 = 0>
@@ -576,57 +703,17 @@
 
     f32x16 acc[3];
     int tm[3], tn[3];
-    int nt1w = 0;
-#pragma unroll
-    for (int j = 0; j < 3; ++j) {
-      const int t = wv + NW * j;
-      const bool mine = t < mt1n * nt1n;
-      tn[j] = mine ? t / mt1n : 0;
-      tm[j] = mine ? t - tn[j] * mt1n : -1;
-      nt1w += mine ? 1 : 0;
-#pragma unroll
-      for (int r = 0; r < 16; ++r) acc[j][r] = 0.f;
-    }
-    dft_product_lds_any<NW, DFT_PIPE_LDS ? 2 : 0>(acc, nt1w, 0, ks1n, ldsU, MxS, ldsF, N1, wv, mt1n, l31, hw);
+    dft_step_lds<NW, DFT_PIPE_LDS ? 2 : 0>(acc, tm, tn, ks1n, ldsU, MxS, ldsF, N1, wv, mt1n, nt1n, l31, hw);
     DFT_BARRIER();
     DFT_STAMP(1)
 
-#pragma unroll
-    for (int j = 0; j < 3; ++j) {
-      if (tm[j] < 0) continue;
-      const int n = tn[j] * 32 + l31, v = n >> 1, ri = n & 1;
-#pragma unroll
-      for (int q = 0; q < 4; ++q) {
-        const int mb = tm[j] * 32 + 8 * q;
-        const int img = dft_div(mb, pl.inv_pp), h0 = mb - img * Pp + 4 * hw;
-        if (v < V && img < G) {
-          u32x2 hi, lo;
-          const float sc = 1.0f / 2097152.0f;
-          dft_split4(acc[j][4 * q] * sc, acc[j][4 * q + 1] * sc, acc[j][4 * q + 2] * sc, acc[j][4 * q + 3] * sc, &hi, &lo);
-          const int kg = R2 ? (h0 >> 5) * 8 + ri * 4 + ((h0 & 31) >> 3) : ri * (Pp / 8) + (h0 >> 3);
-          unsigned char* dst = ldsUb + ((size_t)(kg * 2) * N2S + img * V + v) * 16 + (h0 & 4) * 2;
-          *reinterpret_cast<u32x2*>(dst) = hi;
-          *reinterpret_cast<u32x2*>(dst + (size_t)N2S * 16) = lo;
-        }
-      }
-    }
+    dft_fwd_write_r<R2, G>(acc, tm, tn, pl, ldsUb, V, Pp, N2S, l31, hw);
     DFT_BARRIER();
     DFT_STAMP(2)
 
     f32x16 xc[3];
     int un[3], um[3];
-    int nt2w = 0;
-#pragma unroll
-    for (int j = 0; j < 3; ++j) {
-      const int t = wv + NW * j;
-      const int nt = ALDS ? t / mt2n : (wv >> 2) + (NW / 4) * j;
-      const bool mine = ALDS ? t < mt2n * nt2n : (nt < nt2n && mt2 < mt2n);
-      un[j] = mine ? nt : -1;
-      um[j] = ALDS ? t - nt * mt2n : mt2;
-      nt2w += mine ? 1 : 0;
-#pragma unroll
-      for (int r = 0; r < 16; ++r) xc[j][r] = 0.f;
-    }
+    const int nt2w = dft_step_rega_tiles<ALDS, NW>(xc, un, um, wv, mt2, mt2n, nt2n);
     const int itn = it + DFT_GRID < iters ? it + DFT_GRID : it;
     {
       if (ALDS) {
@@ -647,61 +734,11 @@
     DFT_STAMP(3)
 
     const int XS = P * 8 * G + 16;
-#pragma unroll
-    for (int j = 0; j < 3; ++j) {
-      if (un[j] < 0) continue;
-      const int n2 = un[j] * 32 + l31;
-      const int img = dft_div(n2, pl.inv_v), v = n2 - img * V;
-#pragma unroll
-      for (int q = 0; q < 4; ++q) {
-        const int u0 = (um[j] * 32 + 8 * q + 4 * hw) >> 1;
-        if (img < G && u0 < P) {
-          const float sc = 1.0f / 4194304.0f;
-          f32x4 o;
-          o[0] = xc[j][4 * q] * sc;
-          o[1] = xc[j][4 * q + 1] * sc;
-          o[2] = xc[j][4 * q + 2] * sc;
-          o[3] = xc[j][4 * q + 3] * sc;
-          *reinterpret_cast<f32x4*>(ldsUb + (size_t)v * XS + (u0 >> 2) * (G * 32) + img * 32 + (u0 & 3) * 8) = o;
-        }
-      }
-    }
+    dft_fwd_stage<G>(xc, un, um, pl, ldsUb, P, V, XS, l31, hw);
     DFT_BARRIER();
     DFT_STAMP(4)
 
-    {
-      const int per_v = (P / 4) * (G * 2), npieces = V * per_v;
-      size_t qstride;
-      float* dstbase = X + dft_spectra_pair0(pr_, NBT, pl.NBINS / 4, Cpad, &qstride) + (size_t)c0_ * 8;
-      if (R2) {
-        constexpr int per_h = (DFT_R2_P / 8) * (G * 2);
-        for (int i = tl; i < V * per_h; i += THR) {
-          const int v = i / per_h, rem = i - v * per_h;
-          const int uq = rem / (2 * G), jj = rem - uq * (2 * G);
-          const unsigned char* src = ldsUb + (size_t)v * XS + uq * (G * 32) + jj * 16;
-          const f32x4 e = *reinterpret_cast<const f32x4*>(src);
-          const f32x4 o = *reinterpret_cast<const f32x4*>(src + (DFT_R2_P / 8) * (G * 32));
-          const f32x4 w = *reinterpret_cast<const f32x4*>(ldsTw + (4 * uq + 2 * (jj & 1)) * 8);
-          f32x4 t;
-          t[0] = w[0] * o[0] - w[1] * o[1];
-          t[1] = w[0] * o[1] + w[1] * o[0];
-          t[2] = w[2] * o[2] - w[3] * o[3];
-          t[3] = w[2] * o[3] + w[3] * o[2];
-          float* dst = dstbase + (size_t)(v * (P / 4) + uq) * qstride + jj * 4;
-          DFT_STREAM_STORE(reinterpret_cast<f32x4*>(dst), e + t);
-          DFT_STREAM_STORE(reinterpret_cast<f32x4*>(dst + (size_t)(DFT_R2_P / 8) * qstride), e - t);
-        }
-      } else
-      for (int i = tl; i < npieces; i += THR) {
-        const int v = dft_div(i, pl.inv_pq), rem = i - v * per_v;
-        const int uq = rem / (2 * G), jj = rem - uq * (2 * G);
-        const f32x4 val = *reinterpret_cast<const f32x4*>(ldsUb + (size_t)v * XS + uq * (G * 32) + jj * 16);
-        DFT_STREAM_STORE(reinterpret_cast<f32x4*>(dstbase + (size_t)(v * (P / 4) + uq) * qstride + jj * 4), val);
-      }
-      const int qpad0 = (P * V) / 4, qpad1 = pl.NBINS / 4;
-      for (int i = tl; i < (qpad1 - qpad0) * 2 * G; i += THR)
-        *reinterpret_cast<f32x4*>(dstbase + (size_t)(qpad0 + i / (2 * G)) * qstride + (i % (2 * G)) * 4) = f32x4{0.f, 0.f, 0.f, 0.f};
-    }
+    dft_fwd_store<R2, G, THR>(X, pl, ldsUb, ldsTw, pr_, c0_, NBT, Cpad, P, V, XS, tl);
     DFT_BARRIER();
     DFT_STAMP(5)
   }
@@ -710,6 +747,97 @@
 #undef DFT_FWD_POS
 #undef DFT_FWD_PREFETCH
 #undef DFT_FWD_PREFETCH_SLOTS
+}
+
+#define DFT_INV_ITEM(E)                                                                     \
+  const int img_ = (E) & (G - 1), rest_ = (E) >> (G == 8 ? 3 : 2);                          \
+  const int v_ = dft_div(rest_, pl.inv_kg), uo_ = rest_ - v_ * uoct;                        \
+  const bool two_ = 8 * uo_ + 4 < P;
+
+template <int G>
+DFT_DEV void dft_inv_scales(const float* smaxw, const DftPlan& pl, int P, int tl, int hw, float* simg, float* cinv) {
+#pragma unroll
+  for (int g = 0; g < G; ++g) {
+    float m = 0.f;
+#pragma unroll
+    for (int w = 0; w < DFT_WAVES; ++w) m = fmaxf(m, smaxw[w * G + g]);
+    int E = (int)((__builtin_bit_cast(unsigned, m) >> 23) & 0xffu) - 127;
+    if (!(m > 0.f) || E < -100) E = -100;
+    if (E > 100) E = 100;
+    const float s = __builtin_bit_cast(float, (unsigned)(13 - E + 127) << 23);
+    const float sinv = __builtin_bit_cast(float, (unsigned)(E - 13 + 127) << 23);
+    if (g == (tl & (G - 1))) *simg = s;
+    const float ci = sinv * __builtin_bit_cast(float, (unsigned)(pl.eT - 13 + 127) << 23) / (float)(P * pl.Q);
+    if (G == 4 || (g >> 2) == hw) cinv[g & 3] = ci;
+  }
+}
+
+template <int G, int NITEM>
+DFT_DEV void dft_inv_write_y(const f32x4 (*py)[4], float simg, const DftPlan& pl, u32x4* ldsU, int P, int V, int N2S, int uoct, int nitem,
+                             int tl) {
+#pragma unroll
+  for (int s = 0; s < NITEM; ++s) {
+    const int e = tl + s * DFT_THR;
+    if (e < nitem) {
+      DFT_INV_ITEM(e)
+      const int img = img_, v = v_, uo = uo_;
+      const bool two = two_;
+      float re[8], im[8];
+#pragma unroll
+      for (int k = 0; k < 4; ++k) {
+        const bool ok = k < 2 || two;
+        re[2 * k] = ok ? py[s][k][0] * simg : 0.f;
+        im[2 * k] = ok ? py[s][k][1] * simg : 0.f;
+        re[2 * k + 1] = ok ? py[s][k][2] * simg : 0.f;
+        im[2 * k + 1] = ok ? py[s][k][3] * simg : 0.f;
+      }
+      u32x2 h0, l0, h1, l1;
+      u32x4 t;
+      const size_t n = (size_t)img * V + v;
+      dft_split4(re[0], re[1], re[2], re[3], &h0, &l0);
+      dft_split4(re[4], re[5], re[6], re[7], &h1, &l1);
+      t[0] = h0[0], t[1] = h0[1], t[2] = h1[0], t[3] = h1[1];
+      ldsU[(size_t)((uo)*2 + 0) * N2S + n] = t;
+      t[0] = l0[0], t[1] = l0[1], t[2] = l1[0], t[3] = l1[1];
+      ldsU[(size_t)((uo)*2 + 1) * N2S + n] = t;
+      dft_split4(im[0], im[1], im[2], im[3], &h0, &l0);
+      dft_split4(im[4], im[5], im[6], im[7], &h1, &l1);
+      t[0] = h0[0], t[1] = h0[1], t[2] = h1[0], t[3] = h1[1];
+      ldsU[(size_t)((uoct + uo) * 2 + 0) * N2S + n] = t;
+      t[0] = l0[0], t[1] = l0[1], t[2] = l1[0], t[3] = l1[1];
+      ldsU[(size_t)((uoct + uo) * 2 + 1) * N2S + n] = t;
+    }
+  }
+}
+
+template <int G>
+DFT_DEV void dft_inv_write_t(const f32x16* ta, const int* an, const int* am, const DftPlan& pl, unsigned char* ldsUb, int V, int MB, int MBS,
+                             int KB, int tl, int l31, int hw) {
+  const float sc = __builtin_bit_cast(float, (unsigned)(127 - 14 - pl.eT) << 23);
+#pragma unroll
+  for (int j = 0; j < 3; ++j) {
+    if (an[j] < 0) continue;
+    const int n = an[j] * 32 + l31;
+    const int img = dft_div(n, pl.inv_v), v = n - img * V;
+    if (img >= G) continue;
+#pragma unroll
+    for (int q = 0; q < 4; ++q) {
+      const int h0 = (am[j] * 32 + 8 * q + 4 * hw) >> 1;
+      u32x2 hi, lo;
+      dft_split4(ta[j][4 * q] * sc, ta[j][4 * q + 1] * sc, ta[j][4 * q + 2] * sc, ta[j][4 * q + 3] * sc, &hi, &lo);
+      unsigned char* d0 = ldsUb + ((size_t)((v >> 2) * 2) * MBS + (size_t)h0 * G + img) * 16 + (v & 3) * 4;
+      *reinterpret_cast<unsigned*>(d0) = hi[0];
+      *reinterpret_cast<unsigned*>(d0 + (size_t)MBS * 16) = lo[0];
+      *reinterpret_cast<unsigned*>(d0 + G * 16) = hi[1];
+      *reinterpret_cast<unsigned*>(d0 + G * 16 + (size_t)MBS * 16) = lo[1];
+    }
+  }
+  for (int v = V; v < KB / 2; ++v)
+    for (int m = tl; m < MB; m += DFT_THR) {
+      unsigned char* d0 = ldsUb + ((size_t)((v >> 2) * 2) * MBS + m) * 16 + (v & 3) * 4;
+      *reinterpret_cast<unsigned*>(d0) = 0u;
+      *reinterpret_cast<unsigned*>(d0 + (size_t)MBS * 16) = 0u;
+    }
 }
 
 template <bool TILED, int KSA = 0, int G = DFT_G>
@@ -783,10 +911,6 @@
       py[s][3] = *reinterpret_cast<const f32x4*>(p1_ + 4);                                 \
     }                                                                                       \
   }
-#define DFT_INV_ITEM(E)                                                                     \
-  const int img_ = (E) & (G - 1), rest_ = (E) >> LG;                                        \
-  const int v_ = dft_div(rest_, pl.inv_kg), uo_ = rest_ - v_ * uoct;                        \
-  const bool two_ = 8 * uo_ + 4 < P;
 #define DFT_INV_MAXIMA(TID)                                                                 \
   {                                                                                         \
     float m = 0.f;                                                                          \
@@ -831,72 +955,14 @@
 
     DFT_STAMP(0)
     float simg = 1.f, cinv[4] = {0.f, 0.f, 0.f, 0.f};
-    {
-#pragma unroll
-      for (int g = 0; g < G; ++g) {
-        float m = 0.f;
-#pragma unroll
-        for (int w = 0; w < DFT_WAVES; ++w) m = fmaxf(m, smaxw[w * G + g]);
-        int E = (int)((__builtin_bit_cast(unsigned, m) >> 23) & 0xffu) - 127;
-        if (!(m > 0.f) || E < -100) E = -100;
-        if (E > 100) E = 100;
-        const float s = __builtin_bit_cast(float, (unsigned)(13 - E + 127) << 23);
-        const float sinv = __builtin_bit_cast(float, (unsigned)(E - 13 + 127) << 23);
-        if (g == (tl & (G - 1))) simg = s;
-        const float ci = sinv * __builtin_bit_cast(float, (unsigned)(pl.eT - 13 + 127) << 23) / (float)(P * pl.Q);
-        if (G == 4 || (g >> 2) == hw) cinv[g & 3] = ci;
-      }
-    }
-#pragma unroll
-    for (int s = 0; s < NITEM; ++s) {
-      const int e = tl + s * DFT_THR;
-      if (e < nitem) {
-        DFT_INV_ITEM(e)
-        const int img = img_, v = v_, uo = uo_;
-        const bool two = two_;
-        float re[8], im[8];
-#pragma unroll
-        for (int k = 0; k < 4; ++k) {
-          const bool ok = k < 2 || two;
-          re[2 * k] = ok ? py[s][k][0] * simg : 0.f;
-          im[2 * k] = ok ? py[s][k][1] * simg : 0.f;
-          re[2 * k + 1] = ok ? py[s][k][2] * simg : 0.f;
-          im[2 * k + 1] = ok ? py[s][k][3] * simg : 0.f;
-        }
-        u32x2 h0, l0, h1, l1;
-        u32x4 t;
-        const size_t n = (size_t)img * V + v;
-        dft_split4(re[0], re[1], re[2], re[3], &h0, &l0);
-        dft_split4(re[4], re[5], re[6], re[7], &h1, &l1);
-        t[0] = h0[0], t[1] = h0[1], t[2] = h1[0], t[3] = h1[1];
-        ldsU[(size_t)((uo)*2 + 0) * N2S + n] = t;
-        t[0] = l0[0], t[1] = l0[1], t[2] = l1[0], t[3] = l1[1];
-        ldsU[(size_t)((uo)*2 + 1) * N2S + n] = t;
-        dft_split4(im[0], im[1], im[2], im[3], &h0, &l0);
-        dft_split4(im[4], im[5], im[6], im[7], &h1, &l1);
-        t[0] = h0[0], t[1] = h0[1], t[2] = h1[0], t[3] = h1[1];
-        ldsU[(size_t)((uoct + uo) * 2 + 0) * N2S + n] = t;
-        t[0] = l0[0], t[1] = l0[1], t[2] = l1[0], t[3] = l1[1];
-        ldsU[(size_t)((uoct + uo) * 2 + 1) * N2S + n] = t;
-      }
-    }
+    dft_inv_scales<G>(smaxw, pl, P, tl, hw, &simg, cinv);
+    dft_inv_write_y<G, NITEM>(py, simg, pl, ldsU, P, V, N2S, uoct, nitem, tl);
     DFT_BARRIER();
     DFT_STAMP(1)
 
     f32x16 ta[3];
     int an[3], am[3];
-    int ntaw = 0;
-#pragma unroll
-    for (int j = 0; j < 3; ++j) {
-      const int t = wv + DFT_WAVES * j;
-      const int nt = ALDS ? t / mtAn : (wv >> 2) + 2 * j;
-      const bool mine = ALDS ? t < mtAn * ntAn : (nt < ntAn && mtA < mtAn);
-      an[j] = mine ? nt : -1;
-      am[j] = ALDS ? t - nt * mtAn : mtA;
-      ntaw += mine ? 1 : 0;
-#pragma unroll
-      for (int r = 0; r < 16; ++r) ta[j][r] = 0.f;
-    }
+    const int ntaw = dft_step_rega_tiles<ALDS, DFT_WAVES>(ta, an, am, wv, mtA, mtAn, ntAn);
     const int itn = it + DFT_GRID < iters ? it + DFT_GRID : it;
     {
       if (ALDS) {
@@ -913,50 +979,13 @@
     DFT_BARRIER();
     DFT_STAMP(2)
 
-    {
-      const float sc = __builtin_bit_cast(float, (unsigned)(127 - 14 - pl.eT) << 23);
-#pragma unroll
-      for (int j = 0; j < 3; ++j) {
-        if (an[j] < 0) continue;
-        const int n = an[j] * 32 + l31;
-        const int img = dft_div(n, pl.inv_v), v = n - img * V;
-        if (img >= G) continue;
-#pragma unroll
-        for (int q = 0; q < 4; ++q) {
-          const int h0 = (am[j] * 32 + 8 * q + 4 * hw) >> 1;
-          u32x2 hi, lo;
-          dft_split4(ta[j][4 * q] * sc, ta[j][4 * q + 1] * sc, ta[j][4 * q + 2] * sc, ta[j][4 * q + 3] * sc, &hi, &lo);
-          unsigned char* d0 = ldsUb + ((size_t)((v >> 2) * 2) * MBS + (size_t)h0 * G + img) * 16 + (v & 3) * 4;
-          *reinterpret_cast<unsigned*>(d0) = hi[0];
-          *reinterpret_cast<unsigned*>(d0 + (size_t)MBS * 16) = lo[0];
-          *reinterpret_cast<unsigned*>(d0 + G * 16) = hi[1];
-          *reinterpret_cast<unsigned*>(d0 + G * 16 + (size_t)MBS * 16) = lo[1];
-        }
-      }
-      for (int v = V; v < KB / 2; ++v)
-        for (int m = tl; m < MB; m += DFT_THR) {
-          unsigned char* d0 = ldsUb + ((size_t)((v >> 2) * 2) * MBS + m) * 16 + (v & 3) * 4;
-          *reinterpret_cast<unsigned*>(d0) = 0u;
-          *reinterpret_cast<unsigned*>(d0 + (size_t)MBS * 16) = 0u;
-        }
-    }
+    dft_inv_write_t<G>(ta, an, am, pl, ldsUb, V, MB, MBS, KB, tl, l31, hw);
     DFT_BARRIER();
     DFT_STAMP(3)
 
     f32x16 yc[3];
     int bm[3], bn[3];
-    int ntbw = 0;
-#pragma unroll
-    for (int j = 0; j < 3; ++j) {
-      const int t = wv + DFT_WAVES * j;
-      const bool mine = t < mtBn * ntBn;
-      bn[j] = mine ? t / mtBn : 0;
-      bm[j] = mine ? t - bn[j] * mtBn : -1;
-      ntbw += mine ? 1 : 0;
-#pragma unroll
-      for (int r = 0; r < 16; ++r) yc[j][r] = 0.f;
-    }
-    dft_product_lds_any<DFT_WAVES, DFT_PIPE_LDS ? 1 : 0>(yc, ntbw, 0, ksBn, ldsU, MBS, ldsG, NBo, wv, mtBn, l31, hw);
+    dft_step_lds<DFT_WAVES, DFT_PIPE_LDS ? 1 : 0>(yc, bm, bn, ksBn, ldsU, MBS, ldsG, NBo, wv, mtBn, ntBn, l31, hw);
     DFT_INV_MAXIMA(tl)
     DFT_STAMP(4)
 
@@ -1039,6 +1068,205 @@
   if (DFT_FLAG_SET(bad_flag) && DFT_BALLOT(bad) != 0ull) {
     if ((tid & 63) == 0) DFT_RAISE(bad_flag);
   }
+}
+
+template <int KS = 0>
+DFT_DEV void dft_inverse_forward_body(const float* Y,
+                                      const float* bp,
+                                      int MTP, float* X,
+                                      const u32x4* FqT, const u32x4* Fp2, const u32x4* E2, const u32x4* Gq, const DftPlan& pl,
+                                      int Cout, int Cpad, int NBT, int iters, DFT_FLAG bad_flag) {
+  constexpr int G = DFT_G, LG = 2, NW = DFT_WAVES, THR = DFT_THR;
+  constexpr bool R2 = KS == 8;
+  unsigned char* smem = DFT_LDS;
+  const int tid = DFT_TID, lane = tid & 63, l31 = lane & 31, hw = lane >> 5;
+  const int wv = DFT_UNIFORM(tid >> 6);
+  const int P = pl.P, V = pl.V, Pp = pl.Pp, Wk = pl.Wk, N1 = pl.N1, Mx = pl.Mx, N2 = pl.N2, MB = pl.MB, KB = pl.KB, H = pl.H, W = pl.W;
+  const int MxS = Mx + 1, N2S = N2 + 1, MBS = MB + 1;
+  const int OG = Cout / G;
+  const int NBc = dft_fused_gq_cols(W), nG = (KB / 8) * 2 * NBc, NQ = dft_round_up(pl.Q, 32), nF = (Wk / 8) * 2 * N1;
+  u32x4* ldsG = reinterpret_cast<u32x4*>(smem);
+  u32x4* ldsF = ldsG + nG;
+  unsigned char* ldsUb = smem + (size_t)(nG + nF) * 16;
+  u32x4* ldsU = reinterpret_cast<u32x4*>(ldsUb);
+  unsigned char* fixed = ldsUb + pl.lds_union;
+  float* smaxw = reinterpret_cast<float*>(fixed);
+  const unsigned char* ldsTw = fixed + DFT_R2_LDS_TW;
+  for (int i = tid; i < nG; i += THR) {
+    const int kh = i / NBc, n = i - kh * NBc;
+    ldsG[i] = Gq[(size_t)kh * NQ + n];
+  }
+  for (int i = tid; i < nF; i += THR) ldsF[i] = FqT[i];
+  if (R2 && tid < DFT_R2_TWU) reinterpret_cast<u32x4*>(fixed + DFT_R2_LDS_TW)[tid] = Fp2[DFT_R2_MATU + tid];
+
+  const int mtAn = pl.MA / 32, ntAn = N2 / 32, ksAn = 2 * Pp / 16;
+  const int mtBn = MB / 32, ntBn = pl.NBo / 32, ksBn = KB / 16;
+  const int mt1n = Mx / 32, nt1n = N1 / 32, nt2n = N2 / 32, mt2n = pl.M2 / 32, ks1n = Wk / 16, ks2n = 2 * Pp / 16;
+  const int mtA = wv & 3, mt2 = wv & 3;
+  const int MAfull = dft_round_up(2 * P, 32);
+  constexpr int KRA = KS ? KS : DFT_KREG, KR2 = R2 ? 4 : KRA;
+  half8 e2h[KRA], e2l[KRA];
+#define DFT_FUSED_LOAD_E2(L31, HW)                                                                          \
+  _Pragma("unroll") for (int ks = 0; ks < KRA; ++ks) {                                                      \
+    const int kc = ks < ksAn ? ks : 0, mc = mtA < mtAn ? mtA : 0;                                           \
+    e2h[ks] = dft_frag(E2 + ((size_t)((2 * kc + (HW)) * 2 + 0)) * MAfull + mc * 32 + (L31));                \
+    e2l[ks] = dft_frag(E2 + ((size_t)((2 * kc + (HW)) * 2 + 1)) * MAfull + mc * 32 + (L31));                \
+  }
+#define DFT_FUSED_LANDED_E2()                               \
+  _Pragma("unroll") for (int ks = 0; ks < KRA; ++ks) {      \
+    DFT_LANDED(e2h[ks]);                                    \
+    DFT_LANDED(e2l[ks]);                                    \
+  }
+  DFT_FUSED_LOAD_E2(l31, hw)
+  DFT_FUSED_LANDED_E2()
+
+  constexpr int NITEM = 3;
+  const int uoct = Pp / 8, nitem = G * V * uoct;
+  f32x4 py[NITEM][4];
+  bool bad = false;
+  const int first = (DFT_GRID & 7) == 0 ? (DFT_BID & 7) * (DFT_GRID >> 3) + (DFT_BID >> 3) : DFT_BID;
+  if (first < iters) {
+    DFT_INV_PREFETCH(first, tid)
+    DFT_INV_MAXIMA(tid)
+  }
+  DFT_BARRIER();
+
+  DFT_STAMP_BEGIN()
+  for (int it = first; it < iters; it += DFT_GRID) {
+    int tl = tid;
+#ifndef OS2D_HOST_EMU
+    asm volatile("" : "+v"(tl));
+#endif
+    const int lane = tl & 63, l31 = lane & 31, hw = lane >> 5;
+    const int pr = dft_div(it, pl.inv_og), og = it - pr * OG, o0 = og * G;
+
+    DFT_STAMP(0)
+    float simg = 1.f, cinv[4] = {0.f, 0.f, 0.f, 0.f};
+    dft_inv_scales<G>(smaxw, pl, P, tl, hw, &simg, cinv);
+    dft_inv_write_y<G, NITEM>(py, simg, pl, ldsU, P, V, N2S, uoct, nitem, tl);
+    DFT_BARRIER();
+    DFT_STAMP(1)
+
+    f32x16 ta[3];
+    int an[3], am[3];
+    const int ntaw = dft_step_rega_tiles<false, NW>(ta, an, am, wv, mtA, mtAn, ntAn);
+    dft_product_rega_any<KS>(ta, ntaw, e2h, e2l, ksAn, ldsU, N2S, wv >> 2, 2, l31, hw);
+    DFT_BARRIER();
+    DFT_STAMP(2)
+
+    dft_inv_write_t<G>(ta, an, am, pl, ldsUb, V, MB, MBS, KB, tl, l31, hw);
+    DFT_BARRIER();
+    DFT_STAMP(3)
+
+    f32x16 yc[3];
+    int bm[3], bn[3];
+    dft_step_lds<NW, DFT_PIPE_LDS ? 1 : 0>(yc, bm, bn, ksBn, ldsU, MBS, ldsG, NBc, wv, mtBn, ntBn, l31, hw);
+    DFT_BARRIER();
+    DFT_STAMP(4)
+
+    {
+      float bias[4], osc[4];
+#pragma unroll
+      for (int g = 0; g < 4; ++g) {
+        bias[g] = bp[o0 + g];
+        osc[g] = bp[2 * MTP + o0 + g];
+      }
+#pragma unroll
+      for (int j = 0; j < 3; ++j) {
+        if (bm[j] < 0) continue;
+        const int w = bn[j] * 32 + l31;
+#pragma unroll
+        for (int q = 0; q < 4; ++q) {
+          const int h = (bm[j] * 32 + 8 * q + 4 * hw) >> 2;
+          const bool inside = h < H && w < W;
+          float t[4];
+#pragma unroll
+          for (int g = 0; g < 4; ++g) {
+            const float pre = yc[j][4 * q + g] * cinv[g] + bias[g];
+            t[g] = fmaxf(pre, 0.f) * osc[g];
+            if (inside && (!(fabsf(t[g]) <= 65504.f) || pre != pre)) bad = true;
+          }
+          if (h < Pp && w < Wk) {
+            u32x2 hi = {0u, 0u}, lo = {0u, 0u};
+            if (inside) dft_split4(t[0], t[1], t[2], t[3], &hi, &lo);
+            const int r = R2 ? (h & 1) * 32 + (h >> 1) : h;
+            unsigned char* dst = ldsUb + ((size_t)((w >> 3) * 2) * MxS + r) * 16 + (w & 7) * 2;
+#pragma unroll
+            for (int g = 0; g < 4; ++g) {
+              *reinterpret_cast<unsigned short*>(dst + (size_t)g * Pp * 16) = (unsigned short)(hi[g >> 1] >> (16 * (g & 1)));
+              *reinterpret_cast<unsigned short*>(dst + ((size_t)g * Pp + MxS) * 16) = (unsigned short)(lo[g >> 1] >> (16 * (g & 1)));
+            }
+          }
+        }
+      }
+      const int hB = pl.MA / 2, nz = Pp > hB ? Pp - hB : 0;
+      for (int i = tl; i < G * nz * (Wk / 8) * 2; i += THR) {
+        const int kh = i / (G * nz), rem = i - kh * (G * nz), g = rem / nz, h = hB + rem - g * nz;
+        ldsU[(size_t)kh * MxS + g * Pp + (R2 ? (h & 1) * 32 + (h >> 1) : h)] = u32x4{0u, 0u, 0u, 0u};
+      }
+      for (int i = tl; i < (Mx - G * Pp) * (Wk / 8) * 2; i += THR) {
+        const int m = G * Pp + i % (Mx - G * Pp), kh = i / (Mx - G * Pp);
+        ldsU[(size_t)kh * MxS + m] = u32x4{0u, 0u, 0u, 0u};
+      }
+    }
+    DFT_BARRIER();
+    DFT_STAMP(5)
+
+    f32x16 acc[3];
+    int tm[3], tn[3];
+    dft_step_lds<NW, DFT_PIPE_LDS ? 2 : 0>(acc, tm, tn, ks1n, ldsU, MxS, ldsF, N1, wv, mt1n, nt1n, l31, hw);
+    DFT_BARRIER();
+    DFT_STAMP(6)
+
+    half8 fp2h[KR2], fp2l[KR2];
+#pragma unroll
+    for (int ks = 0; ks < KR2; ++ks) {
+      if (R2) {
+        fp2h[ks] = dft_frag(Fp2 + ((size_t)((2 * ks + hw) * 2 + 0)) * 64 + (mt2 & 1) * 32 + l31);
+        fp2l[ks] = dft_frag(Fp2 + ((size_t)((2 * ks + hw) * 2 + 1)) * 64 + (mt2 & 1) * 32 + l31);
+      } else {
+        const int kc = ks < ks2n ? ks : 0, mc = mt2 < mt2n ? mt2 : 0;
+        fp2h[ks] = dft_frag(Fp2 + ((size_t)((2 * kc + hw) * 2 + 0)) * pl.M2 + mc * 32 + l31);
+        fp2l[ks] = dft_frag(Fp2 + ((size_t)((2 * kc + hw) * 2 + 1)) * pl.M2 + mc * 32 + l31);
+      }
+    }
+    dft_fwd_write_r<R2, G>(acc, tm, tn, pl, ldsUb, V, Pp, N2S, l31, hw);
+    DFT_BARRIER();
+    DFT_STAMP(7)
+#pragma unroll
+    for (int ks = 0; ks < KR2; ++ks) {
+      DFT_LANDED(fp2h[ks]);
+      DFT_LANDED(fp2l[ks]);
+    }
+
+    f32x16 xc[3];
+    int un[3], um[3];
+    const int nt2w = dft_step_rega_tiles<false, NW>(xc, un, um, wv, mt2, mt2n, nt2n);
+    const int itn = it + DFT_GRID < iters ? it + DFT_GRID : it;
+    DFT_INV_PREFETCH_ITEMS(itn, tl, 0, NITEM)
+    if (R2) dft_product_rega_any<4>(xc, nt2w, fp2h, fp2l, 4, ldsU + (size_t)(mt2 >> 1) * 16 * N2S, N2S, wv >> 2, NW / 4, l31, hw);
+    else dft_product_rega_any<KS>(xc, nt2w, fp2h, fp2l, ks2n, ldsU, N2S, wv >> 2, NW / 4, l31, hw);
+    DFT_INV_MAXIMA(tl)
+    DFT_FUSED_LOAD_E2(l31, hw)
+    DFT_BARRIER();
+    DFT_STAMP(8)
+
+    const int XS = P * 8 * G + 16;
+    dft_fwd_stage<G>(xc, un, um, pl, ldsUb, P, V, XS, l31, hw);
+    DFT_BARRIER();
+    DFT_FUSED_LANDED_E2()
+    DFT_STAMP(9)
+
+    dft_fwd_store<R2, G, THR>(X, pl, ldsUb, ldsTw, pr, o0, NBT, Cpad, P, V, XS, tl);
+    DFT_BARRIER();
+    DFT_STAMP(10)
+  }
+  DFT_STAMP_END_FUSED()
+  if (DFT_FLAG_SET(bad_flag) && DFT_BALLOT(bad) != 0ull) {
+    if ((tid & 63) == 0) DFT_RAISE(bad_flag);
+  }
+#undef DFT_FUSED_LOAD_E2
+#undef DFT_FUSED_LANDED_E2
 #undef DFT_INV_MAXIMA
 #undef DFT_INV_ITEM
 #undef DFT_INV_PREFETCH
diff --git a/os2d_amd/csrc/dft_mfma.hip b/os2d_amd/csrc/dft_mfma.hip
--- a/os2d_amd/csrc/dft_mfma.hip
+++ b/os2d_amd/csrc/dft_mfma.hip
@@ -27,7 +27,7 @@
 #define DFT_RAISE(f) os2d_raise(f)
 #ifdef OS2D_DIAG_DFT_STAMPS
 __device__ unsigned long long os2d_dft_stamps[16];
-#define DFT_STAMP_BEGIN() unsigned long long st_acc_[6] = {0, 0, 0, 0, 0, 0}, st_n_ = 0, st_last_ = wall_clock64();
+#define DFT_STAMP_BEGIN() unsigned long long st_acc_[11] = {0, 0, 0, 0, 0, 0, 0, 0, 0, 0, 0}, st_n_ = 0, st_last_ = wall_clock64();
 #define DFT_STAMP(K)                                   \
   {                                                    \
     const unsigned long long t_ = wall_clock64();      \
@@ -40,6 +40,13 @@
     for (int k_ = 0; k_ < 6; ++k_) atomicAdd(&os2d_dft_stamps[(BASE) + k_], st_acc_[k_]);     \
     atomicAdd(&os2d_dft_stamps[(BASE) + 6], st_n_);                                           \
   }
+#define DFT_STAMP_END_FUSED()                                                                 \
+  if (threadIdx.x == 0) {                                                                     \
+    for (int k_ = 0; k_ < 6; ++k_) atomicAdd(&os2d_dft_stamps[8 + k_], st_acc_[k_]);          \
+    for (int k_ = 6; k_ < 11; ++k_) atomicAdd(&os2d_dft_stamps[k_ - 5], st_acc_[k_]);         \
+    atomicAdd(&os2d_dft_stamps[6], st_n_);                                                    \
+    atomicAdd(&os2d_dft_stamps[14], st_n_);                                                   \
+  }
 #endif
 #include "dft_mfma.h"
 
@@ -52,6 +59,14 @@
                                                                       float* __restrict__ X, const u32x4* __restrict__ FqT,
                                                                       const u32x4* __restrict__ Fp2, DftPlan pl, int C, int Cpad, int NBT,
                                                                       int iters) {
+  if constexpr (!TILED && !FAST && G == DFT_G && KS != 0) {
+    if (pl.fused) {
+      const u32x4* E2 = Fp2 + dft_units_fp2(pl.P, pl.Q);
+      const u32x4* Gq = E2 + dft_units_e2(pl.P, pl.Q);
+      dft_inverse_forward_body<KS>(corr, invn, C, X, FqT, Fp2, E2, Gq, pl, C, Cpad, NBT, iters, pl.fused_flag);
+      return;
+    }
+  }
   dft_forward_body<TILED, FAST, G, NW, KS>(corr, invn, X, FqT, Fp2, pl, C, Cpad, NBT, iters);
 }
 
@@ -197,7 +212,7 @@
   const u32x4* FqT = static_cast<const u32x4*>(matrices);
   const u32x4* Fp2 = FqT + dft_units_fqt(pl.P, pl.Q);
   auto kern = G == 8 ? dft_forward_pick<8, 8>(pl) : dft_forward_pick<4, 8>(pl);
-  if (int rc = os2d_set_dynamic_lds(kern, pl.lds_total, "dft_forward")) return rc;
+  if (int rc = os2d_set_dynamic_lds(kern, pl.lds_fused > pl.lds_total ? pl.lds_fused : pl.lds_total, "dft_forward")) return rc;
   hipLaunchKernelGGL(kern, dim3(dft_grid(iters)), dim3(DFT_THR), pl.lds_total, stream, corr, inv, X, FqT, Fp2, pl,
                      C, Cpad, NBT, iters);
   return os2d_launched("dft_forward");
@@ -225,6 +240,46 @@
   return os2d_launched("dft_inverse");
 }
 
+static bool dft_fused_ok(const DftPlan& pl) {
+  const int ks = 2 * pl.Pp / 16;
+  return pl.G == DFT_G && pl.T == 1 && pl.lds_fused != 0 && ks >= 5 && ks <= 8 && !(pl.Pp == 64 && !dft_radix2(pl.P));
+}
+
+bool os2d_dft_has_fused_plan(int H, int W) {
+  DftPlan pl;
+  return H >= 1 && W >= 1 && dft_plan_cached(H, W, &pl) && dft_fused_ok(pl);
+}
+
+int os2d_launch_dft_inverse_forward(const float* Y, const float* bp, int MTP, float* X, const void* matrices, int NB, int Cout, int Cpad,
+                                    int H, int W, Os2dRangeFlag status, hipStream_t stream) {
+  DftPlan pl;
+  if (!dft_plan_cached(H, W, &pl)) {
+    os2d_set_error("dft_inverse_forward: no transform plan for a %dx%d map", H, W);
+    return -3;
+  }
+  if (Cout % 8 || Cpad < Cout) {
+    os2d_set_error("dft_inverse_forward: Cout %d must be a multiple of 8 and the channel stride %d not smaller", Cout, Cpad);
+    return -1;
+  }
+  if (!dft_fused_ok(pl)) return OS2D_DFT_NO_FUSED_PLAN;
+  const int OG = Cout / DFT_G, NBT = NB, iters = NBT * OG;
+  pl.inv_og = dft_magic((unsigned)OG);
+  if (MTP != Cout) {
+    os2d_set_error("dft_inverse_forward: the bias table must have %d entries per row", Cout);
+    return -1;
+  }
+  const u32x4* FqT = static_cast<const u32x4*>(matrices);
+  const u32x4* Fp2 = FqT + dft_units_fqt(pl.P, pl.Q);
+  pl.fused = 1;
+  pl.fused_flag = status;
+  DftPlan any_width = pl;
+  any_width.fast = 0;
+  auto kern = dft_forward_pick<4, 8>(any_width);
+  if (int rc = os2d_set_dynamic_lds(kern, pl.lds_fused > pl.lds_total ? pl.lds_fused : pl.lds_total, "dft_inverse_forward")) return rc;
+  hipLaunchKernelGGL(kern, dim3(dft_grid(iters)), dim3(DFT_THR), pl.lds_fused, stream, Y, bp, X, FqT, Fp2, pl, Cout, Cpad, NBT, iters);
+  return os2d_launched("dft_inverse_forward");
+}
+
 extern "C" int os2d_debug_dft_stamps(unsigned long long* out16, int reset) {
 #ifdef OS2D_DIAG_DFT_STAMPS
   if (out16 && hipMemcpyFromSymbol(out16, HIP_SYMBOL(os2d_dft_stamps), 16 * sizeof(unsigned long long)) != hipSuccess) return -4;
diff --git a/os2d_amd/csrc/os2d_common.h b/os2d_amd/csrc/os2d_common.h
--- a/os2d_amd/csrc/os2d_common.h
+++ b/os2d_amd/csrc/os2d_common.h
@@ -127,6 +127,10 @@
 enum { OS2D_DFT_OUT_SHB = 0, OS2D_DFT_OUT_SHB_BORDERS = 1, OS2D_DFT_OUT_PLANES = 2 };
 int os2d_launch_dft_inverse(const float* Y, const float* bp, int MTP, void* out, const void* matrices, int NB, int Cout, int H, int W,
                             Os2dRangeFlag status, int form, hipStream_t stream);
+enum { OS2D_DFT_NO_FUSED_PLAN = 1 };
+bool os2d_dft_has_fused_plan(int H, int W);
+int os2d_launch_dft_inverse_forward(const float* Y, const float* bp, int MTP, float* X, const void* matrices, int NB, int Cout, int Cpad,
+                                    int H, int W, Os2dRangeFlag status, hipStream_t stream);
 int os2d_corr_groups(int C);
 int os2d_launch_split_fm(const float* fm, const float* sumsq, void* fs, int A, int C, int HW, void* clear, size_t clear_words,
                          Os2dRangeFlag status, hipStream_t stream);
```

Result: no change. 46490, median of 6 (+0.5%).
